# jzhangbs/MVSDF

Measured on AMD Instinct MI355X. Metric: traced rays/sec (fwd+bwd, 10 sphere iters, 4 src views), higher is better.
Workload: dtype f32x3

## Files before the change

include/mvsdf_hip.h:

```cpp
#ifndef MVSDF_HIP_H
#define MVSDF_HIP_H
#include <stddef.h>
#include <stdint.h>

#ifdef __cplusplus
extern "C" {
#endif

#define MVSDF_MAX_LAYERS 12

typedef struct {
    int n_layers;
    int K[MVSDF_MAX_LAYERS];
    int N[MVSDF_MAX_LAYERS];
    const float* wp[MVSDF_MAX_LAYERS];
    const float* bias[MVSDF_MAX_LAYERS];
    const float* w[MVSDF_MAX_LAYERS];
    int skip_layer;
    int multires;
    const void* wp16[MVSDF_MAX_LAYERS];
    int trace_dtype;
    unsigned skip_mask;
    const void* wx3[MVSDF_MAX_LAYERS];
} MvsdfNetDesc;

typedef struct {
    float r;
    float thr;
    float line_search_step;
    int line_step_iters;
    int st_iters;
    int n_steps;
    int n_secant;
    float dist_clip;
} MvsdfTraceParams;

enum {
    MVSDF_CNT_ROWS_SPHERE = 0,
    MVSDF_CNT_ROWS_SAMPLER = 1,
    MVSDF_CNT_ROWS_SECANT = 2,
    MVSDF_CNT_ROWS_MINSDF = 3,
    MVSDF_CNT_N_SECANT = 4,
    MVSDF_CNT_N_SAMPLER = 5,
    MVSDF_CNT_N_MINSDF = 6,
    MVSDF_CNT_N_SAMPLER_REST = 7,
    MVSDF_CNT_ROWS_SAMPLER_EVAL = 8,
    MVSDF_CNT_TAIL_NEXT = 9,
    MVSDF_CNT_TAIL_READY = 10,
    MVSDF_CNT_TAIL_WGS = 11,
    MVSDF_CNT_TAIL_ROWS = 12
};

int mvsdf_version(void);
int mvsdf_abi_struct_sizes(size_t* out);
const char* mvsdf_last_error(void);

size_t mvsdf_packed_floats(int N, int K);

int mvsdf_fold_pack(const float* v, const float* g, int N, int K, float* w, float* wp, float* wpT, void* stream);
int mvsdf_fold_pack_net(int n_layers, const float* const* v, const float* const* g, const int* N, const int* K, float* const* w,
                        float* const* wp, float* const* wpT, void* stream);
int mvsdf_fold_backward_net(int n_layers, const float* const* v, const float* const* g, const float* const* dW, const float* const* db,
                            const int* N, const int* K, float* const* dv, float* const* dg, float* const* dbias, int accumulate,
                            void* stream);
int mvsdf_fold_backward(const float* v, const float* g, const float* dW, int N, int K, float* dv, float* dg, void* stream);

size_t mvsdf_packed_bf16_bytes(int N, int K, int nsplit);
int mvsdf_pack_bf16w_net(int n_layers, const float* const* w, const int* N, const int* K, float* const* wp_rounded, void* stream);
int mvsdf_pack_bf16s_net(int n_layers, const float* const* w, const int* N, const int* K, void* const* wp16, void* stream);
int mvsdf_pack_bf16x3_net(int n_layers, const float* const* w, const int* N, const int* K, void* const* wp16, void* stream);
int mvsdf_pack_bf16x3t_net(int n_layers, const float* const* w, const int* N, const int* K, void* const* wx3t, void* stream);

int mvsdf_sdf_col0(const MvsdfNetDesc* net, const float* x, int n, float* y, int mt, void* stream);

int mvsdf_camera_rays(const float* uv, const float* pose, const float* intrinsics, int B, int P, float* ray_dirs, float* cam_loc,
                      void* stream);

int mvsdf_sphere_intersection(const float* cam_loc, const float* ray_dirs, int B, int P, float r, float* t, uint8_t* mask, void* stream);

size_t mvsdf_trace_workspace_bytes(int R);
size_t mvsdf_trace_workspace_bytes_n(int R, int n_steps);
int mvsdf_trace(const MvsdfNetDesc* net, const MvsdfTraceParams* tp, const float* cam_loc, const float* ray_dirs,
                const uint8_t* object_mask, int B, int P, int training, const float* intervals, const float* minsdf_steps,
                float* points, uint8_t* mask, float* dists, unsigned long long* counters, void* workspace,
                size_t workspace_bytes, int mt, int mt_samples, void* stream);
int mvsdf_trace_stage(int stage, const MvsdfNetDesc* net, const MvsdfTraceParams* tp, const float* cam_loc, const float* ray_dirs,
                      const uint8_t* object_mask, int B, int P, int training, const float* intervals, const float* minsdf_steps,
                      float* points, uint8_t* mask, float* dists, unsigned long long* counters, void* workspace,
                      size_t workspace_bytes, int mt, int mt_samples, void* stream);

size_t mvsdf_tracegen_state_bytes(int R);
int mvsdf_tracegen_init(const MvsdfTraceParams* tp, const float* cam_loc, const float* ray_dirs, const uint8_t* object_mask, int B, int P,
                        void* state, uint8_t* req, float* pts, unsigned long long* counters, void* stream);
int mvsdf_tracegen_step(const MvsdfTraceParams* tp, const float* cam_loc, const float* ray_dirs, int B, int P, void* state, const float* vals,
                        uint8_t* req, float* pts, unsigned long long* counters, void* stream);
int mvsdf_tracegen_finish(const MvsdfTraceParams* tp, const float* cam_loc, const float* ray_dirs, int B, int P, int training, const void* state,
                          float* points, uint8_t* mask, float* dists, unsigned long long* counters, void* workspace, size_t workspace_bytes,
                          void* stream);
int mvsdf_tracegen_rows(const MvsdfTraceParams* tp, int kind, const float* cam_loc, const float* ray_dirs, int B, int P, const float* zs, int n_list,
                        void* workspace, float* out_pts, void* stream);
int mvsdf_tracegen_reduce(const MvsdfTraceParams* tp, int kind, const float* cam_loc, const float* ray_dirs, int B, int P, int training,
                          const float* intervals, const float* minsdf_steps, const float* sv, float* points, uint8_t* mask, float* dists,
                          unsigned long long* counters, void* workspace, uint8_t* marks, void* stream);
int mvsdf_tracegen_secant(const MvsdfTraceParams* tp, int op, const float* cam_loc, const float* ray_dirs, int B, int P, int n_sec, const float* vals,
                          float* pts_out, float* points, float* dists, unsigned long long* counters, void* workspace, void* stream);

size_t mvsdf_sdf_ctx_floats(const MvsdfNetDesc* net, int M, int Mg);
int mvsdf_sdf_forward(const MvsdfNetDesc* net, const MvsdfNetDesc* netT, const float* x, int M, int Mg, float* y, float* nrm, float* ctx,
                      void* stream);
size_t mvsdf_sdf_bwd_ws_floats(const MvsdfNetDesc* net, int Mb);
int mvsdf_sdf_backward(const MvsdfNetDesc* net, const MvsdfNetDesc* netT, const float* x, int M, int Mg, int row0, int Mb, const float* dy,
                       const float* dn, const float* ctx, float* dW_cat, float* db_cat, float* dx, float* ws, void* stream);

int mvsdf_sdf_backward_pair(const MvsdfNetDesc* net, const MvsdfNetDesc* netT, int M, int Mg, int MbA, const float* dyA, const float* dnA, float* wsA,
                            int row0X, int MbX, const float* dyX, const float* dnX, float* wsX, float* dx, const float* ctx, void* stream);
int mvsdf_sdf_backward_finish(const MvsdfNetDesc* net, const MvsdfNetDesc* netT, int M, int Mg, int Mb, const float* dy, const float* ctx, float* ws,
                              int row0D, int MbD, const float* fbar, float* dW_cat, float* db_cat, void* stream);

size_t mvsdf_render_ctx_floats(const MvsdfNetDesc* net, int N);
size_t mvsdf_render_bwd_ws_floats(const MvsdfNetDesc* net, int N);
int mvsdf_render_forward(const MvsdfNetDesc* net, const float* points, const float* view, const float* normals, const float* feat,
                         int ldfeat, int N, int multires_view, float* rgb, float* ctx, void* stream);
int mvsdf_render_backward(const MvsdfNetDesc* net, const MvsdfNetDesc* netT, int N, int Nctx, const float* drgb, const float* ctx,
                          float* dW_cat, float* db_cat, float* din, float* ws, void* stream);

int mvsdf_feat_corr(const float* pts, int N, const int* view_start, int B, int V, int C, int H, int W, const float* feat,
                    const long long* feat_strides, const float* feat_src, const long long* src_strides, const float* cam,
                    const float* src_cams, const float* size, const float* center, float* loss_pp, float* dpts, void* stream);

int mvsdf_depth_carve(const float* pts, int pts_ld, int M, const float* depths, int B, int h, int w, const float* cams, const float* size,
                      const float* center, float out_thresh_perc, float far_thresh, float far_att, float near_thresh, float near_att, int use_invalid,
                      float* dist_r, float* weight, float* pts_world, void* stream);

int mvsdf_loss_terms(const float* rgb, const float* rgb_gt, const uint8_t* rgb_mask, int R, const float* grad_theta, int n_eik,
                     const float* eik_out, const float* dist_r, const float* dweight, int n_depth, const float* surf, int n_surf,
                     const long long* n_pos, const float* feat_pp, int n_feat, float w_rgb, float w_eik, float w_surf, float w_feat,
                     float w_depth, float smooth, int surf_on, int feat_on, const float* inv_counts, float* out, float* d_rgb, float* d_grad,
                     float* d_eik_out, float* d_surf, void* stream);

int mvsdf_partition_rays(const uint8_t* net_mask, const uint8_t* object_mask, const uint8_t* true_mask, const float* ray_dirs, int R,
                         long long* perm, long long* inv, long long* true_rows, long long* counts, float* view_sorted, void* stream);
int mvsdf_step_outputs(int R, int n_eik, int n_ds, int Nout, const long long* counts, const float* x_eval, const float* y_eval,
                       const float* n_eval, const long long* inv, const long long* true_rows, const float* rgb_sorted, int d_mask,
                       int e_mask, float* rgb_values, float* sdf_output, float* diff_pts, float* eik_out, float* points_hom, float* grad_theta,
                       float* surf, void* stream);
int mvsdf_step_backward_inputs(int stage, int n_eik, int n_ds, int N, int Nout, int n_true, const float* din, int din_ld, int din_feat0,
                               int din_nrm0, int use_geo, const float* d_diff, const float* dx, const float* view_sorted, const float* n_eval,
                               const long long* true_rows, const float* d_eo, const float* d_gth, const float* d_si, int d_mask, int e_mask,
                               float* dy, float* dn, void* stream);
int mvsdf_step_backward_fbar(int n_eik, int n_ds, int N, int Nout, const float* din, int din_ld, int use_geo, const float* d_diff, const float* dx,
                             const float* view_sorted, const float* n_eval, float* dy, float* fbar, void* stream);

int mvsdf_dsurf_select(const float* depths, const float* kinv, const float* einv, int N, int H, int W, const float* size, const float* center,
                       float bb, float jitter_rad, unsigned long long seed, int n, long long* idx, long long* counts, void* stream);
int mvsdf_dsurf_points(const float* depths, const float* kinv, const float* einv, int N, int H, int W, const float* size, const float* center,
                       float bb, float jitter_rad, unsigned long long seed, int n, const long long* idx_sorted, const long long* counts,
                       float* pts_on, float* pts_jit, void* stream);

size_t mvsdf_adam_ws_floats(void);
int mvsdf_adam_step(float* p, float* g, float* m, float* v, size_t n, float lr, double beta1, double beta2, float eps, int step, float max_norm,
                    float* norm_out, float* ws, void* stream);
int mvsdf_adam_step_scaled(float* p, float* g, float* m, float* v, size_t n, float lr, double beta1, double beta2, float eps, int step,
                           float max_norm, float grad_scale, float* norm_out, float* ws, void* stream);
int mvsdf_adam_step_fused(float* p, float* g, float* m, float* v, size_t n, float lr, double beta1, double beta2, float eps, int step,
                          float max_norm, float grad_scale, int zero_grad, float* norm_out, float* ws, void* stream);

int mvsdf_loss_prep(const uint8_t* net_mask, const uint8_t* obj_mask, const uint8_t* true_mask, int R, int B, uint8_t* hit, int* view_start,
                    long long* n_pos, void* stream);
int mvsdf_loss_scale(const float* const* g, float w_rgb, float w_eik, float w_surf, float w_feat, float w_depth, const float* d_rgb, float* g_rgb,
                     int n_rgb, const float* d_grad, float* g_grad, int n_grad, const float* d_eo, float* g_eo, int n_eo, const float* d_sf,
                     float* g_sf, int n_sf, float* coef_feat, void* stream);

int mvsdf_det_math(int op, const float* x, int n, float* y0, float* y1, void* stream);

#define MVSDF_STEP_MAX_LAYERS 24

typedef struct {
    int B, P;
    int n_eik;
    int n_ds;
    int n_sdf, n_render;
    int N[MVSDF_STEP_MAX_LAYERS];
    int K[MVSDF_STEP_MAX_LAYERS];
    unsigned skip_mask;
    int multires;
    int view_spec;
    int trace_dtype;
    int use_object_mask;
    MvsdfTraceParams tp;
    int mt, mt_samples;
} MvsdfStepDesc;

typedef struct {
    const float* v[MVSDF_STEP_MAX_LAYERS];
    const float* g[MVSDF_STEP_MAX_LAYERS];
    const float* b[MVSDF_STEP_MAX_LAYERS];
} MvsdfStepParams;

typedef struct {
    const float* uv; const float* pose; const float* intrinsics;
    const uint8_t* object_mask;
    const uint8_t* object_mask_true;
    const float* intervals;
    const float* minsdf_steps;
    const float* eik_points;
    const float* ds_on; const float* ds_jit;
    const long long* ds_counts;
    const float* host_stage;
} MvsdfStepInputs;

typedef struct {
    size_t fwd_bytes, bwd_bytes;
    size_t ray_dirs, cam_loc;
    size_t points, mask, dists, counters;
    size_t object_mask_out;
    size_t rgb_values, sdf_output, diff_pts, eik_out, points_hom, grad_theta, surf;
    size_t perm;
    size_t dflat;
    size_t dflat_floats;
} MvsdfStepLayout;

int mvsdf_step_create(const MvsdfStepDesc* desc, MvsdfStepLayout* layout, void** step);
void mvsdf_step_destroy(void* step);
#define MVSDF_STEP_UNHIT_DEFER 0
#define MVSDF_STEP_UNHIT_EAGER 1
int mvsdf_step_forward(void* step, const MvsdfStepParams* prm, const MvsdfStepInputs* in, int d_mask, int e_mask, int mode, void* fwd, void* stream);
int mvsdf_step_resolve_unhit(void* step, void* fwd, void* stream);
int mvsdf_step_can_defer_unhit(void* step);
int mvsdf_step_last_tracer_grid(void* step, int out[2]);
int mvsdf_step_wait_counts(void* step, long long counts[4]);
#define MVSDF_STEP_COUNT_RING 64
long long mvsdf_step_seq(void* step);
size_t mvsdf_step_counts_offset(void* step);
int mvsdf_step_wait_counts_seq(void* step, long long seq, long long counts[4]);
long long mvsdf_step_done_seq(void* step, long long counts[4]);
int mvsdf_step_can_defer(void* step);
int mvsdf_step_saved_offsets(void* step, size_t out[6]);
int mvsdf_step_backward(void* step, const MvsdfStepParams* prm, int N, int n_true, int d_mask, int e_mask, int use_geo, const float* d_diff,
                        const float* d_rgb, const float* d_gth, const float* d_eo, const float* d_si, const void* fwd, void* bwd,
                        float* const* dv, float* const* dg, float* const* db, int accumulate, void* stream);
int mvsdf_step_set_timing(void* step, int enable);
int mvsdf_step_trace_times(void* step, float ms[3]);
int mvsdf_step_times(void* step, float ms[6]);

typedef struct {
    int R, B;
    int N, n_grad, n_depth, n_surf;
    const uint8_t* net_mask; const uint8_t* obj_mask; const uint8_t* true_mask;
    const float* rgb; const float* rgb_gt;
    const float* grad_theta; const float* eik_out; const float* surf; const float* diff_pts;
    float* points_hom;
    int feat_on, surf_on;
    int V, C, H, W;
    const float* feat; long long feat_strides[4]; const float* feat_src; long long src_strides[5];
    const float* cam; const float* src_cams; const float* size; const float* center;
    const float* depths; int dB, dh, dw; const float* depth_cams;
    float out_thresh_perc, far_thresh, far_att, near_thresh, near_att;
    float w_rgb, w_eik, w_surf, w_feat, w_depth;
    int use_invalid;
    float smooth;
    const float* inv_counts;
    const long long* counts_dev;
    int n_eik, n_ds, d_mask, e_mask;
} MvsdfLossArgs;
typedef struct {
    size_t bytes, out, hit, view_start, n_pos, loss_pp, dpts, dist_r, weight, d_rgb, d_grad, d_eo, d_sf;
    size_t s_rgb, s_grad, s_eo, s_sf, s_diff;
} MvsdfLossLayout;
int mvsdf_loss_layout(const MvsdfLossArgs* a, MvsdfLossLayout* lo);
int mvsdf_loss_forward(const MvsdfLossArgs* a, void* blk, void* stream);
int mvsdf_loss_backward(const MvsdfLossArgs* a, const void* blk, const float* const* g, float* g_rgb, float* g_grad, float* g_eo, float* g_sf,
                        float* g_diff, void* stream);

size_t mvsdf_mc_workspace_bytes(int64_t nx, int64_t ny, int64_t nz);
int mvsdf_mc_count(const float* vol, const int64_t* shape, const int64_t* strides, float level, void* ws, size_t ws_bytes, void* stream);
int mvsdf_mc_emit(const float* vol, const int64_t* shape, const int64_t* strides, float level, const float* spacing, const float* origin, void* ws,
                  size_t ws_bytes, float* verts, float* normals, int32_t* faces, int64_t nv_cap, int64_t nf_cap, void* stream);
size_t mvsdf_mesh_cc_workspace_bytes(int64_t nv, int64_t nf);
int mvsdf_mesh_components(const float* verts, const int32_t* faces, int64_t nv, int64_t nf, void* ws, size_t ws_bytes, int32_t* vert_label,
                          int32_t* face_label, void* stream);
int mvsdf_mesh_select(const int32_t* vert_label, const int32_t* face_label, int64_t nv, int64_t nf, int32_t label, const float* verts, const float* normals,
                      const float* colors, const int32_t* faces, void* ws, size_t ws_bytes, float* out_verts, float* out_normals, float* out_colors,
                      int32_t* out_faces, int64_t nv_cap, int64_t nf_cap, void* stream);

size_t mvsdf_smc_workspace_bytes(int64_t n, int64_t block);
size_t mvsdf_smc_emit_workspace_bytes(int64_t n, int64_t block, int64_t nactive);
int mvsdf_smc_coarse_points(const float* axis, int64_t n, int64_t block, int64_t start, int64_t count, float* pts, void* stream);
int mvsdf_smc_seed(const float* coarse, int64_t n, int64_t block, float level, float tol, void* ws, size_t ws_bytes, void* stream);
int mvsdf_smc_brick_points(const float* axis, int64_t n, int64_t block, const void* ws, size_t ws_bytes, int64_t start, int64_t count, float* pts,
                           void* stream);
int mvsdf_smc_closure(const float* values, int64_t n, int64_t block, float level, int64_t slot0, int64_t count, void* ws, size_t ws_bytes, void* stream);
int mvsdf_smc_count(const float* values, int64_t n, int64_t block, float level, int64_t nactive, void* ws, size_t ws_bytes, void* ews, size_t ews_bytes,
                    void* stream);
int mvsdf_smc_emit(const float* values, int64_t n, int64_t block, float level, const float* spacing, const float* origin, int64_t nactive, void* ws,
                   size_t ws_bytes, void* ews, size_t ews_bytes, float* verts, float* normals, int32_t* faces, int64_t nv_cap, int64_t nf_cap, void* stream);

size_t mvsdf_mesh_cut_workspace_bytes(int64_t nv, int64_t nf);
int mvsdf_mesh_cut(const float* colors, const int32_t* faces, int64_t nv, int64_t nf, int32_t thresh, int32_t smooth, void* ws, size_t ws_bytes,
                   uint8_t* removed, void* stream);
int mvsdf_mesh_trim(const float* verts, const float* normals, const float* colors, const int32_t* faces, int64_t nv, int64_t nf, void* ws, size_t ws_bytes,
                    float* out_verts, float* out_normals, float* out_colors, int32_t* out_faces, int64_t nv_cap, int64_t nf_cap, void* stream);

size_t mvsdf_mesh_simplify_workspace_bytes(int64_t nv, int64_t nf);
int mvsdf_mesh_simplify(const float* verts, const float* normals, const float* colors, const int32_t* faces, int64_t nv, int64_t nf, double cell,
                        const double* origin, int32_t quadric, int32_t counts_only, void* ws, size_t ws_bytes, void* stream);
int mvsdf_mesh_simplify_emit(const int32_t* faces, int64_t nv, int64_t nf, void* ws, size_t ws_bytes, float* out_verts, float* out_normals,
                             float* out_colors, int32_t* out_faces, int64_t nv_cap, int64_t nf_cap, void* stream);

uint64_t mvsdf_chamfer_key(uint64_t seed, int64_t i);
size_t mvsdf_chamfer_sample_workspace_bytes(int64_t nv, int64_t nf);
int mvsdf_chamfer_sample_count(const float* verts, const int32_t* faces, int64_t nv, int64_t nf, double density, int64_t max_points, void* ws, size_t ws_bytes,
// ... 133 lines not shown
```

mvsdf_amd/_lib.py:

```python
import ctypes as C
import os
import struct

_HERE = os.path.dirname(os.path.abspath(__file__))
SO_PATH = os.environ.get('MVSDF_LIB') or os.path.join(_HERE, 'libmvsdf_hip.so')
MAX_LAYERS = 12
_lib = None


class NetDesc(C.Structure):
    _fields_ = [('n_layers', C.c_int), ('K', C.c_int * MAX_LAYERS), ('N', C.c_int * MAX_LAYERS),
                ('wp', C.c_void_p * MAX_LAYERS), ('bias', C.c_void_p * MAX_LAYERS), ('w', C.c_void_p * MAX_LAYERS),
                ('skip_layer', C.c_int), ('multires', C.c_int), ('wp16', C.c_void_p * MAX_LAYERS), ('trace_dtype', C.c_int), ('skip_mask', C.c_uint), ('wx3', C.c_void_p * MAX_LAYERS)]


class TraceParams(C.Structure):
    _fields_ = [('r', C.c_float), ('thr', C.c_float), ('line_search_step', C.c_float), ('line_step_iters', C.c_int),
                ('st_iters', C.c_int), ('n_steps', C.c_int), ('n_secant', C.c_int), ('dist_clip', C.c_float)]


class MvsdfError(RuntimeError):
    pass


def lib():
    global _lib
    if _lib is None:
        if not os.path.exists(SO_PATH):
            raise MvsdfError('libmvsdf_hip.so not found at %s -- run `python -c "import __graft_entry__ as g; g.build()"` '
                             '(hipcc --offload-arch=gfx950); there is no CPU/PyTorch fallback for the hot path' % SO_PATH)
        import torch
        L = C.CDLL(SO_PATH)
        L.mvsdf_last_error.restype = C.c_char_p
        L.mvsdf_packed_floats.restype = C.c_size_t
        L.mvsdf_packed_floats.argtypes = [C.c_int, C.c_int]
        L.mvsdf_trace_workspace_bytes.restype = C.c_size_t
        L.mvsdf_trace_workspace_bytes.argtypes = [C.c_int]
        L.mvsdf_trace_workspace_bytes_n.restype = C.c_size_t
        L.mvsdf_trace_workspace_bytes_n.argtypes = [C.c_int, C.c_int]
        for fn in ('mvsdf_sdf_ctx_floats', 'mvsdf_sdf_bwd_ws_floats', 'mvsdf_render_ctx_floats', 'mvsdf_render_bwd_ws_floats'):
            getattr(L, fn).restype = C.c_size_t
        L.mvsdf_adam_ws_floats.restype = C.c_size_t
        L.mvsdf_packed_bf16_bytes.restype = C.c_size_t
        L.mvsdf_packed_bf16_bytes.argtypes = [C.c_int, C.c_int, C.c_int]
        L.mvsdf_tracegen_state_bytes.restype = C.c_size_t
        L.mvsdf_adam_step.argtypes = [C.c_void_p] * 4 + [C.c_size_t] + [C.c_float, C.c_double, C.c_double, C.c_float] + [C.c_int, C.c_float, C.c_void_p, C.c_void_p, C.c_void_p]
        L.mvsdf_adam_step_scaled.argtypes = [C.c_void_p] * 4 + [C.c_size_t] + [C.c_float, C.c_double, C.c_double, C.c_float] + [C.c_int, C.c_float, C.c_float, C.c_void_p, C.c_void_p, C.c_void_p]
        L.mvsdf_adam_step_fused.argtypes = [C.c_void_p] * 4 + [C.c_size_t] + [C.c_float, C.c_double, C.c_double, C.c_float] + [C.c_int, C.c_float, C.c_float, C.c_int, C.c_void_p, C.c_void_p, C.c_void_p]
        L.mvsdf_loss_scale.argtypes = [C.c_void_p] + [C.c_float] * 5 + [C.c_void_p, C.c_void_p, C.c_int] * 4 + [C.c_void_p, C.c_void_p]
        i64, vp, f32 = C.c_int64, C.c_void_p, C.c_float
        L.mvsdf_mc_workspace_bytes.restype = C.c_size_t
        L.mvsdf_mc_workspace_bytes.argtypes = [i64] * 3
        L.mvsdf_mc_count.argtypes = [vp, vp, vp, f32, vp, C.c_size_t, vp]
        L.mvsdf_mc_emit.argtypes = [vp, vp, vp, f32, vp, vp, vp, C.c_size_t, vp, vp, vp, i64, i64, vp]
        L.mvsdf_mesh_cc_workspace_bytes.restype = C.c_size_t
        L.mvsdf_mesh_cc_workspace_bytes.argtypes = [i64, i64]
        L.mvsdf_mesh_components.argtypes = [vp, vp, i64, i64, vp, C.c_size_t, vp, vp, vp]
        L.mvsdf_mesh_select.argtypes = [vp, vp, i64, i64, C.c_int32] + [vp] * 5 + [C.c_size_t] + [vp] * 4 + [i64, i64, vp]
        L.mvsdf_smc_workspace_bytes.restype = C.c_size_t
        L.mvsdf_smc_workspace_bytes.argtypes = [i64, i64]
        L.mvsdf_smc_emit_workspace_bytes.restype = C.c_size_t
        L.mvsdf_smc_emit_workspace_bytes.argtypes = [i64, i64, i64]
        L.mvsdf_smc_coarse_points.argtypes = [vp, i64, i64, i64, i64, vp, vp]
        L.mvsdf_smc_seed.argtypes = [vp, i64, i64, f32, f32, vp, C.c_size_t, vp]
        L.mvsdf_smc_brick_points.argtypes = [vp, i64, i64, vp, C.c_size_t, i64, i64, vp, vp]
        L.mvsdf_smc_closure.argtypes = [vp, i64, i64, f32, i64, i64, vp, C.c_size_t, vp]
        L.mvsdf_smc_count.argtypes = [vp, i64, i64, f32, i64, vp, C.c_size_t, vp, C.c_size_t, vp]
        L.mvsdf_smc_emit.argtypes = [vp, i64, i64, f32, vp, vp, i64, vp, C.c_size_t, vp, C.c_size_t, vp, vp, vp, i64, i64, vp]
        L.mvsdf_mesh_cut_workspace_bytes.restype = C.c_size_t
        L.mvsdf_mesh_cut_workspace_bytes.argtypes = [i64, i64]
        L.mvsdf_mesh_cut.argtypes = [vp, vp, i64, i64, C.c_int32, C.c_int32, vp, C.c_size_t, vp, vp]
        L.mvsdf_mesh_trim.argtypes = [vp] * 4 + [i64, i64, vp, C.c_size_t] + [vp] * 4 + [i64, i64, vp]
        f64, u64, sz = C.c_double, C.c_uint64, C.c_size_t
        L.mvsdf_mesh_simplify_workspace_bytes.restype = sz
        L.mvsdf_mesh_simplify_workspace_bytes.argtypes = [i64, i64]
        L.mvsdf_mesh_simplify.argtypes = [vp] * 4 + [i64, i64, f64, vp, C.c_int32, C.c_int32, vp, sz, vp]
        L.mvsdf_mesh_simplify_emit.argtypes = [vp, i64, i64, vp, sz] + [vp] * 4 + [i64, i64, vp]
        L.mvsdf_chamfer_key.restype = u64
        L.mvsdf_chamfer_key.argtypes = [u64, i64]
        for fn in ('mvsdf_chamfer_sample_workspace_bytes', 'mvsdf_chamfer_mask_workspace_bytes', 'mvsdf_chamfer_nearest_workspace_bytes'):
            getattr(L, fn).restype = sz
            getattr(L, fn).argtypes = [i64, i64]
        L.mvsdf_chamfer_downsample_workspace_bytes.restype = sz
        L.mvsdf_chamfer_downsample_workspace_bytes.argtypes = [i64]
        L.mvsdf_chamfer_sample_count.argtypes = [vp, vp, i64, i64, f64, i64, vp, sz, vp]
        L.mvsdf_chamfer_sample_emit.argtypes = [vp, vp, i64, i64, f64, vp, sz, vp, i64, vp]
        L.mvsdf_chamfer_downsample.argtypes = [vp, i64, f64, u64, i64, vp, sz, vp, vp]
        L.mvsdf_chamfer_mask.argtypes = [vp, vp, i64, vp, i64, vp, f64, vp, vp, vp, vp, sz, vp, vp, vp, vp]
        L.mvsdf_chamfer_nearest.argtypes = [vp, i64, vp, i64, f64, vp, sz, vp, vp]
        i32 = C.c_int32
        L.mvsdf_fusion_workspace_bytes.restype = sz
        L.mvsdf_fusion_workspace_bytes.argtypes = [i64] * 4
        L.mvsdf_fusion_fuse.argtypes = [vp, vp, vp, i64, i64, i64, vp, vp, vp, i32, i32, f64, f64, vp, sz, vp, vp, vp, vp]
        L.mvsdf_fusion_emit.argtypes = [vp, i64, i64, i64, i64, vp, sz, vp, vp, vp, vp, i64, vp]
        L.mvsdf_tsdf_workspace_bytes.restype = sz
        L.mvsdf_tsdf_workspace_bytes.argtypes = [i64] * 4
        L.mvsdf_tsdf_integrate.argtypes = [vp, i64, i64, i64, vp, vp, i64, vp, f64, vp, f64, f64, i32, vp, sz, vp, vp, vp, vp]
        L.mvsdf_mcm_workspace_bytes.restype = sz
        L.mvsdf_mcm_workspace_bytes.argtypes = [i64] * 3
        L.mvsdf_mcm_count.argtypes = [vp, vp, vp, vp, f32, vp, sz, vp]
        L.mvsdf_mcm_emit.argtypes = [vp, vp, vp, vp, f32, vp, vp, vp, sz, vp, vp, vp, i64, i64, vp]
        for fn in ('mvsdf_cloud_clean_workspace_bytes', 'mvsdf_cloud_compact_workspace_bytes'):
            getattr(L, fn).restype = sz
            getattr(L, fn).argtypes = [i64]
        L.mvsdf_cloud_knn.argtypes = [vp, i64, i32, vp, sz, vp, vp]
        L.mvsdf_cloud_components.argtypes = [vp, i64, f64, vp, sz, vp, vp]
        L.mvsdf_cloud_clean.argtypes = [vp, i64, i32, f64, f64, f64, vp, sz, vp, vp, vp, vp]
        L.mvsdf_cloud_compact.argtypes = [vp] * 5 + [i64, vp, sz] + [vp] * 4 + [i64, vp]
        L.mvsdf_raster_workspace_bytes.restype = sz
        L.mvsdf_raster_workspace_bytes.argtypes = [i64] * 5
        L.mvsdf_raster_draw.argtypes = [vp, vp, i64, i64, vp, i64, i64, i64, f64, i64, i32, vp, sz, vp]
        L.mvsdf_raster_resolve.argtypes = [i64, i64, i64, vp, sz, vp, vp, vp]
        L.mvsdf_raster_visibility.argtypes = [vp, i64, vp, i64, i64, i64, f64, vp, vp, f64, vp, sz, vp, vp]
        L.mvsdf_raster_colors.argtypes = [vp, vp, i64, vp, vp, i64, i64, i64, f64, vp, vp, vp, f64, f64, i32, f32, f32, f32, vp, sz, vp, vp, vp]
        for fn in ('mvsdf_featext_raw_floats', 'mvsdf_featext_pack_bytes', 'mvsdf_featext_workspace_bytes', 'mvsdf_featext_layer_workspace_bytes'):
            getattr(L, fn).restype = sz
        L.mvsdf_featext_raw_floats.argtypes = []
        L.mvsdf_featext_pack_bytes.argtypes = []
        L.mvsdf_featext_pack.argtypes = [vp, vp, sz, vp]
        L.mvsdf_featext_workspace_bytes.argtypes = [i64] * 3
        L.mvsdf_featext_forward.argtypes = [vp, vp, i64, i64, i64, vp, sz, vp, vp, vp, C.c_int, C.c_int, vp]
        L.mvsdf_featext_layer_workspace_bytes.argtypes = [C.c_int] * 5
        L.mvsdf_featext_layer.argtypes = [C.c_int, vp, vp, C.c_int, C.c_int, C.c_int, vp, C.c_int, vp, C.c_int, i64, i64, i64, vp, C.c_int, vp, sz, vp, vp]
        for fn in ('mvsdf_stereo_workspace_bytes', 'mvsdf_stereo_volume_offset'):
            getattr(L, fn).restype = sz
            getattr(L, fn).argtypes = [i64] * 4
        L.mvsdf_stereo_normalize.argtypes = [vp, i64, i64, vp, vp, vp]
        L.mvsdf_stereo_patches.argtypes = [vp, i64, i64, i64, i32, vp, vp]
        L.mvsdf_stereo_sweep.argtypes = [vp, i64, i64, i64, i64, i64] + [vp] * 7 + [sz] + [vp] * 5
        L.mvsdf_stereo_sgm_workspace_bytes.restype = sz
        L.mvsdf_stereo_sgm_workspace_bytes.argtypes = [i64] * 3
        L.mvsdf_stereo_regularize.argtypes = [vp, i64, i64, i64, f64, f64, i32, vp, sz, vp, vp]
        L.mvsdf_stereo_sweep_sgm_workspace_bytes.restype = sz
        L.mvsdf_stereo_sweep_sgm_workspace_bytes.argtypes = [i64] * 4
        L.mvsdf_stereo_sweep_sgm.argtypes = [vp, i64, i64, i64, i64, i64] + [vp] * 6 + [f64, f64, i32, vp, sz] + [vp] * 5
        L.mvsdf_stereo_upsample.argtypes = [vp, vp] + [i64] * 5 + [vp, vp]
        L.mvsdf_stereo_band_workspace_bytes.restype = sz
        L.mvsdf_stereo_band_workspace_bytes.argtypes = [i64] * 5
        L.mvsdf_stereo_band.argtypes = [vp, i64, i64, i64, i64, i64] + [vp] * 6 + [i32, vp, sz] + [vp] * 5
        L.mvsdf_viewsel_bits_bytes.restype = sz
        L.mvsdf_viewsel_bits_bytes.argtypes = [i64, i64]
        L.mvsdf_viewsel_workspace_bytes.restype = sz
        L.mvsdf_viewsel_workspace_bytes.argtypes = [i64]
        L.mvsdf_viewsel_pack_dense.argtypes = [vp, i64, i64, vp, vp, vp]
        L.mvsdf_viewsel_pack_tracks.argtypes = [vp, vp, i64, i64, i64, vp, vp, vp]
        L.mvsdf_viewsel_scores.argtypes = [vp, vp, vp, i64, i64, f64, f64, f64, vp, sz, vp, vp, vp, vp]
        L.mvsdf_viewsel_depths.argtypes = [vp, vp, vp, i64, i64, i64, i64, vp, vp, vp]
        L.mvsdf_viewsel_weights_host.argtypes = [vp, vp, i64, f64, f64, f64, vp, vp]
        L.mvsdf_undistort_points.argtypes = [vp, i64, C.c_int, vp, vp, C.c_int, vp, vp, vp]
        L.mvsdf_undistort_images.argtypes = [vp, i64, i64, i64, i64, C.c_int, C.c_int, vp, vp, i64, i64, vp, vp, vp]
        L.mvsdf_undistort_points_host.argtypes = [vp, i64, C.c_int, vp, vp, C.c_int, vp, vp]
        L.mvsdf_undistort_images_host.argtypes = [vp, i64, i64, i64, i64, C.c_int, C.c_int, vp, vp, i64, i64, vp, vp]
        L.mvsdf_batch_args_bytes.restype = sz
        L.mvsdf_batch_args_bytes.argtypes = []
        L.mvsdf_batch_gather.argtypes = [vp, vp]
        for name in EXPORTS:
            getattr(L, name)
        _lib = L
    return _lib


EXPORTS = [
    'mvsdf_version', 'mvsdf_abi_struct_sizes', 'mvsdf_last_error', 'mvsdf_packed_floats', 'mvsdf_fold_pack', 'mvsdf_fold_backward', 'mvsdf_fold_pack_net', 'mvsdf_fold_backward_net', 'mvsdf_packed_bf16_bytes', 'mvsdf_pack_bf16w_net', 'mvsdf_pack_bf16s_net', 'mvsdf_pack_bf16x3_net', 'mvsdf_pack_bf16x3t_net',
    'mvsdf_sdf_col0', 'mvsdf_camera_rays', 'mvsdf_sphere_intersection', 'mvsdf_trace_workspace_bytes', 'mvsdf_trace_workspace_bytes_n', 'mvsdf_trace', 'mvsdf_trace_stage', 'mvsdf_det_math',
    'mvsdf_tracegen_state_bytes', 'mvsdf_tracegen_init', 'mvsdf_tracegen_step', 'mvsdf_tracegen_finish', 'mvsdf_tracegen_rows', 'mvsdf_tracegen_reduce',
    'mvsdf_tracegen_secant',
    'mvsdf_sdf_ctx_floats', 'mvsdf_sdf_forward', 'mvsdf_sdf_bwd_ws_floats', 'mvsdf_sdf_backward', 'mvsdf_sdf_backward_pair', 'mvsdf_sdf_backward_finish',
    'mvsdf_feat_corr', 'mvsdf_depth_carve', 'mvsdf_loss_terms', 'mvsdf_loss_prep', 'mvsdf_loss_scale', 'mvsdf_adam_ws_floats', 'mvsdf_adam_step', 'mvsdf_adam_step_scaled', 'mvsdf_adam_step_fused',
    'mvsdf_partition_rays', 'mvsdf_step_outputs', 'mvsdf_step_backward_inputs', 'mvsdf_step_backward_fbar', 'mvsdf_dsurf_select', 'mvsdf_dsurf_points',
    'mvsdf_render_ctx_floats', 'mvsdf_render_bwd_ws_floats', 'mvsdf_render_forward', 'mvsdf_render_backward',
    'mvsdf_step_create', 'mvsdf_step_destroy', 'mvsdf_step_forward', 'mvsdf_step_resolve_unhit', 'mvsdf_step_can_defer_unhit', 'mvsdf_step_last_tracer_grid', 'mvsdf_step_wait_counts', 'mvsdf_step_backward', 'mvsdf_step_set_timing', 'mvsdf_step_trace_times', 'mvsdf_step_times',
    'mvsdf_step_seq', 'mvsdf_step_counts_offset', 'mvsdf_step_wait_counts_seq', 'mvsdf_step_done_seq', 'mvsdf_step_can_defer', 'mvsdf_step_saved_offsets',
    'mvsdf_loss_layout', 'mvsdf_loss_forward', 'mvsdf_loss_backward',
    'mvsdf_mc_workspace_bytes', 'mvsdf_mc_count', 'mvsdf_mc_emit', 'mvsdf_mesh_cc_workspace_bytes', 'mvsdf_mesh_components', 'mvsdf_mesh_select',
    'mvsdf_smc_workspace_bytes', 'mvsdf_smc_emit_workspace_bytes', 'mvsdf_smc_coarse_points', 'mvsdf_smc_seed', 'mvsdf_smc_brick_points',
    'mvsdf_smc_closure', 'mvsdf_smc_count', 'mvsdf_smc_emit',
    'mvsdf_mesh_cut_workspace_bytes', 'mvsdf_mesh_cut', 'mvsdf_mesh_trim',
    'mvsdf_mesh_simplify_workspace_bytes', 'mvsdf_mesh_simplify', 'mvsdf_mesh_simplify_emit',
    'mvsdf_chamfer_key', 'mvsdf_chamfer_sample_workspace_bytes', 'mvsdf_chamfer_sample_count', 'mvsdf_chamfer_sample_emit',
    'mvsdf_chamfer_downsample_workspace_bytes', 'mvsdf_chamfer_downsample', 'mvsdf_chamfer_mask_workspace_bytes', 'mvsdf_chamfer_mask',
    'mvsdf_chamfer_nearest_workspace_bytes', 'mvsdf_chamfer_nearest',
    'mvsdf_fusion_workspace_bytes', 'mvsdf_fusion_fuse', 'mvsdf_fusion_emit',
    'mvsdf_tsdf_workspace_bytes', 'mvsdf_tsdf_integrate', 'mvsdf_mcm_workspace_bytes', 'mvsdf_mcm_count', 'mvsdf_mcm_emit',
    'mvsdf_cloud_clean_workspace_bytes', 'mvsdf_cloud_compact_workspace_bytes', 'mvsdf_cloud_knn', 'mvsdf_cloud_components', 'mvsdf_cloud_clean',
    'mvsdf_cloud_compact',
    'mvsdf_raster_workspace_bytes', 'mvsdf_raster_draw', 'mvsdf_raster_resolve', 'mvsdf_raster_visibility', 'mvsdf_raster_colors',
    'mvsdf_featext_raw_floats', 'mvsdf_featext_pack_bytes', 'mvsdf_featext_pack', 'mvsdf_featext_workspace_bytes', 'mvsdf_featext_forward',
    'mvsdf_featext_layer_workspace_bytes', 'mvsdf_featext_layer',
    'mvsdf_stereo_workspace_bytes', 'mvsdf_stereo_volume_offset', 'mvsdf_stereo_normalize', 'mvsdf_stereo_patches', 'mvsdf_stereo_sweep',
    'mvsdf_stereo_sgm_workspace_bytes', 'mvsdf_stereo_regularize', 'mvsdf_stereo_sweep_sgm_workspace_bytes', 'mvsdf_stereo_sweep_sgm',
    'mvsdf_stereo_upsample', 'mvsdf_stereo_band_workspace_bytes', 'mvsdf_stereo_band',
    'mvsdf_viewsel_bits_bytes', 'mvsdf_viewsel_workspace_bytes', 'mvsdf_viewsel_pack_dense', 'mvsdf_viewsel_pack_tracks', 'mvsdf_viewsel_scores',
    'mvsdf_viewsel_depths', 'mvsdf_viewsel_weights_host',
    'mvsdf_undistort_points', 'mvsdf_undistort_images', 'mvsdf_undistort_points_host', 'mvsdf_undistort_images_host',
    'mvsdf_batch_args_bytes', 'mvsdf_batch_gather',
]


def check(rc, what=''):
    if rc != 0:
        raise MvsdfError('%s failed (code %d): %s' % (what or 'mvsdf call', rc, lib().mvsdf_last_error().decode()))


def ptr(t):
    if t is None:
        return None
    assert t.is_contiguous(), 'tensor must be contiguous'
    return C.c_void_p(t.data_ptr())


def stream_of(t):
    import torch
    if t.is_cuda:
        return C.c_void_p(torch.cuda.current_stream(t.device).cuda_stream)
    return C.c_void_p(0)


def _vp(t):
    return None if t is None else t.data_ptr()


def _stream(t):
    import torch
    return torch.cuda.current_stream(t.device).cuda_stream


def _header(ws, n):
    import torch
    return [int(x) for x in ws[:8 * n].view(torch.int64).cpu()]


def f64_from_bits(bits):
    return struct.unpack('<d', struct.pack('<q', bits))[0]
```

mvsdf_amd/csrc/step_driver.hip:

```cpp
#include <hip/hip_runtime.h>
#include <stdint.h>
#include <stdlib.h>
#include <string.h>
#include <new>
#include "capi_util.h"
#include "step_internal.h"
#include <sched.h>
#include <time.h>

namespace {

inline size_t al256(size_t x) { return (x + 255) & ~(size_t)255; }

struct FwdOffsets {
    size_t w[MVSDF_STEP_MAX_LAYERS], wp[MVSDF_STEP_MAX_LAYERS], wpT[MVSDF_STEP_MAX_LAYERS], wp16[MVSDF_STEP_MAX_LAYERS];
    size_t wx3[MVSDF_STEP_MAX_LAYERS], wx3T[MVSDF_STEP_MAX_LAYERS];
    int chain_x3;
    size_t trace_ws, trace_ws_bytes;
    size_t inv, true_rows, true_rank, counts, view_sorted;
    size_t bias[MVSDF_STEP_MAX_LAYERS], steps;
    size_t x_eval, y_eval, n_eval, sdf_ctx, rgb_sorted, render_ctx;
};
struct BwdOffsets {
    size_t dy, dn, dy_x, dn_x, din, drgb_sorted, render_ws, wsA, wsX, dx, fbar;
};

struct Step {
    MvsdfStepDesc d;
    MvsdfStepLayout lay;
    FwdOffsets fo;
    BwdOffsets bo;
    int R, E, M, Nout, K0r, nl;
    size_t woff[MVSDF_STEP_MAX_LAYERS], boff[MVSDF_STEP_MAX_LAYERS];
    size_t seg[2][3];
    long long* counts_host;
    long long* counts_host_dev;
    int can_defer;
    hipEvent_t ev_counts;
    bool counts_pending;
    long long counts_seq;
    hipStream_t counts_stream;
    int timing;
    hipEvent_t ev_t[9];
    bool timed, timed_bwd;
    hipStream_t side;
    hipEvent_t ev_fork, ev_join;
    int split_rows;
    int can_lazy;
    int last_grid[2];
};

void make_descs(const Step& st, const MvsdfStepParams* prm, const char* fwd, MvsdfNetDesc* sdf, MvsdfNetDesc* sdfT, MvsdfNetDesc* rnd, MvsdfNetDesc* rndT) {
    const MvsdfStepDesc& d = st.d;
    auto fill = [&](MvsdfNetDesc* o, MvsdfNetDesc* oT, int l0, int n, bool is_sdf) {
        memset(o, 0, sizeof(*o));
        memset(oT, 0, sizeof(*oT));
        o->n_layers = oT->n_layers = n;
        for (int i = 0; i < n; ++i) {
            const int l = l0 + i;
            o->K[i] = d.K[l]; o->N[i] = d.N[l];
            oT->K[i] = d.N[l]; oT->N[i] = d.K[l];
            o->wp[i] = (const float*)(fwd + st.fo.wp[l]);
            oT->wp[i] = (const float*)(fwd + st.fo.wpT[l]);
            o->bias[i] = oT->bias[i] = prm->b[l];
            o->w[i] = oT->w[i] = (const float*)(fwd + st.fo.w[l]);
            if (is_sdf && d.trace_dtype != 0) o->wp16[i] = fwd + st.fo.wp16[l];
            if (is_sdf && st.fo.chain_x3) { o->wx3[i] = fwd + st.fo.wx3[l]; oT->wx3[i] = fwd + st.fo.wx3T[l]; }
        }
        if (is_sdf) {
            const unsigned m = d.skip_mask;
            const int single = (m && !(m & (m - 1))) ? __builtin_ctz(m) : -1;
            o->skip_layer = oT->skip_layer = m ? (single >= 0 ? single : __builtin_ctz(m)) : -1;
            o->skip_mask = (m && single < 0) ? m : 0;
            o->multires = oT->multires = d.multires;
            o->trace_dtype = (d.trace_dtype >= 1 && d.trace_dtype <= 5) ? d.trace_dtype : 0;
        } else {
            o->skip_layer = oT->skip_layer = -1;
        }
    };
    fill(sdf, sdfT, 0, d.n_sdf, true);
    fill(rnd, rndT, d.n_sdf, d.n_render, false);
}

__global__ void k_step_gather_x(const float* __restrict__ eik, int n_eik, const float* __restrict__ ds_on, const float* __restrict__ ds_jit, int n_ds,
                                const float* __restrict__ points, const long long* __restrict__ perm, int R, float* __restrict__ x_eval,
                                uint8_t* __restrict__ ones) {
    const int E = n_eik + 2 * n_ds, total = (E + R) * 3;
    for (int i = blockIdx.x * blockDim.x + threadIdx.x; i < total; i += gridDim.x * blockDim.x) {
        const int row = i / 3, c = i - 3 * row;
        float v;
        if (row < n_eik) v = eik[i];
        else if (row < n_eik + n_ds) v = ds_on[3 * (size_t)(row - n_eik) + c];
        else if (row < E) v = ds_jit[3 * (size_t)(row - n_eik - n_ds) + c];
        else v = points[3 * (size_t)perm[row - E] + c];
        x_eval[i] = v;
        if (ones && i < R) ones[i] = 1;
    }
}

__global__ void k_step_gather_drgb(const float* __restrict__ d_rgb, const long long* __restrict__ perm, int N, float* __restrict__ out) {
    const int i = blockIdx.x * blockDim.x + threadIdx.x;
    if (i >= 3 * N) return;
    const int row = i / 3, c = i - 3 * row;
    out[i] = d_rgb[3 * (size_t)perm[row] + c];
}

#define ST_TRY(expr) do { int rc_ = (expr); if (rc_) return rc_; } while (0)
#define ST_HIP(expr) do { hipError_t e_ = (expr); if (e_ != hipSuccess) return mv_check(e_, #expr); } while (0)

}

extern "C" {

int mvsdf_step_create(const MvsdfStepDesc* desc, MvsdfStepLayout* layout, void** out) {
    if (!desc || !layout || !out) return mv_fail(-1, "mvsdf_step_create: null argument");
    if (desc->trace_dtype == 1) return mv_fail(-2, "mvsdf_step_create: trace_dtype 1 (bf16 weights AND 8-bit activations) was removed in round 5: use 3 (bf16x2)");
    const MvsdfStepDesc& d = *desc;
    const int nl = d.n_sdf + d.n_render;
    if (d.B <= 0 || d.P <= 0 || d.n_eik < 0 || d.n_ds < 0 || d.n_sdf < 2 || d.n_render < 1 || d.n_sdf > MVSDF_MAX_LAYERS || d.n_render > MVSDF_MAX_LAYERS ||
        nl > MVSDF_STEP_MAX_LAYERS || (long long)d.B * d.P > (1ll << 24))
        return mv_fail(-1, "mvsdf_step_create: bad sizes");
    Step* st = new (std::nothrow) Step;
    if (!st) return mv_fail(-1, "mvsdf_step_create: out of host memory");
    memset(st, 0, sizeof(*st));
    st->d = d;
    st->R = d.B * d.P; st->E = d.n_eik + 2 * d.n_ds; st->M = st->R + st->E; st->nl = nl;
    st->Nout = d.N[d.n_sdf - 1]; st->K0r = d.K[d.n_sdf];
    st->split_rows = -1;
    const int R = st->R, M = st->M;
    MvsdfNetDesc sdf, sdfT, rnd, rndT;
    MvsdfStepParams fake;
    memset(&fake, 0, sizeof(fake));
    static const float dummy = 0.f;
    for (int l = 0; l < nl; ++l) fake.b[l] = &dummy;
    MvsdfStepLayout& L = st->lay;
    FwdOffsets& fo = st->fo;
    size_t p = 0;
    auto take = [&](size_t bytes) { const size_t o = p; p += al256(bytes ? bytes : 4); return o; };
    L.ray_dirs = take((size_t)R * 12); L.cam_loc = take((size_t)d.B * 12);
    L.points = take((size_t)R * 12); L.mask = take((size_t)R); L.dists = take((size_t)R * 4); L.counters = take(16 * 8);
    L.object_mask_out = take((size_t)R);
    fo.trace_ws_bytes = mvsdf_trace_workspace_bytes_n(R, d.tp.n_steps);
    fo.trace_ws = take(fo.trace_ws_bytes);
    fo.chain_x3 = mv_dev_switches().chain_x3;
    for (int l = 0; l < nl; ++l) {
        fo.w[l] = take((size_t)d.N[l] * d.K[l] * 4);
        fo.wp[l] = take(mvsdf_packed_floats(d.N[l], d.K[l]) * 4);
        fo.wpT[l] = take(mvsdf_packed_floats(d.K[l], d.N[l]) * 4);
        if (l < d.n_sdf && d.trace_dtype == 2) {
            fo.wp16[l] = take(mvsdf_packed_floats(d.N[l], d.K[l]) * 4);
        } else if (l < d.n_sdf && (d.trace_dtype == 3 || d.trace_dtype == 4)) {
            fo.wp16[l] = take(mvsdf_packed_bf16_bytes(d.N[l], d.K[l], 0));
        } else if (l < d.n_sdf && d.trace_dtype == 5) {
            fo.wp16[l] = take(3 * mvsdf_packed_bf16_bytes(d.N[l], d.K[l], 0));
        }
        if (l < d.n_sdf && fo.chain_x3) {
            fo.wx3[l] = d.trace_dtype == 5 ? fo.wp16[l] : take(3 * mvsdf_packed_bf16_bytes(d.N[l], d.K[l], 0));
            fo.wx3T[l] = take(3 * mvsdf_packed_bf16_bytes(d.K[l], d.N[l], 0));
        }
    }
    L.perm = take((size_t)R * 8); fo.inv = take((size_t)R * 8); fo.true_rows = take((size_t)R * 8); fo.true_rank = take((size_t)R * 4); fo.counts = take(4 * 8 + 4 * 4);
    fo.view_sorted = take((size_t)R * 12);
    for (int l = 0; l < d.n_sdf; ++l) fo.bias[l] = take((size_t)d.N[l] * 4);
    fo.steps = take((size_t)(d.tp.n_steps > 0 ? d.tp.n_steps : 0) * 4);
    fo.x_eval = take((size_t)M * 12); fo.y_eval = take((size_t)M * st->Nout * 4); fo.n_eval = take((size_t)M * 12);
    make_descs(*st, &fake, (const char*)nullptr, &sdf, &sdfT, &rnd, &rndT);
    for (int i = 0; i < d.n_sdf; ++i) { sdf.wp[i] = sdfT.wp[i] = &dummy; sdf.w[i] = &dummy; }
    for (int i = 0; i < d.n_render; ++i) { rnd.wp[i] = rndT.wp[i] = &dummy; }
    const size_t ctx_f = mvsdf_sdf_ctx_floats(&sdf, M, M), rctx_f = mvsdf_render_ctx_floats(&rnd, R);
    if (!ctx_f || !rctx_f) { delete st; return mv_fail(-2, "mvsdf_step_create: network descriptor rejected (layer dims / skip mask)"); }
    st->can_lazy = mv_chain_fwd_covers(&sdf);
    st->can_defer = (d.n_ds == 0 && mv_step_can_defer(&sdf, &sdfT, &rnd, &rndT)) ? 1 : 0;
    fo.sdf_ctx = take(ctx_f * 4);
    fo.rgb_sorted = take((size_t)R * 12);
    fo.render_ctx = take(rctx_f * 4);
    L.rgb_values = take((size_t)R * 12); L.sdf_output = take((size_t)R * 4); L.diff_pts = take((size_t)R * 12);
    L.eik_out = take((size_t)M * 4); L.points_hom = take((size_t)M * 16); L.grad_theta = take((size_t)M * 12);
    L.surf = take((size_t)(R + d.n_eik) * 4);
    L.fwd_bytes = p;
    BwdOffsets& bo = st->bo;
    p = 0;
    bo.dy = take((size_t)M * st->Nout * 4); bo.dn = take((size_t)M * 12);
    bo.dy_x = take((size_t)R * st->Nout * 4); bo.dn_x = take((size_t)R * 12);
    bo.din = take((size_t)R * st->K0r * 4); bo.drgb_sorted = take((size_t)R * 12);
    bo.render_ws = take(mvsdf_render_bwd_ws_floats(&rnd, R) * 4);
    bo.wsA = take(mvsdf_sdf_bwd_ws_floats(&sdf, M) * 4);
    bo.wsX = take(mvsdf_sdf_bwd_ws_floats(&sdf, R) * 4);
    bo.dx = take((size_t)R * 12); bo.fbar = take((size_t)R * 4);
    size_t off = 0;
    int lo = 0;
    const int cuts[2] = {d.n_sdf, nl};
    for (int net = 0; net < 2; ++net) {
        st->seg[net][0] = off;
        for (int l = lo; l < cuts[net]; ++l) { st->woff[l] = off; off += (size_t)d.N[l] * d.K[l]; }
        st->seg[net][1] = off;
        for (int l = lo; l < cuts[net]; ++l) { st->boff[l] = off; off += (size_t)d.N[l]; }
        st->seg[net][2] = off;
        lo = cuts[net];
    }
    L.dflat_floats = off;
    L.dflat = take(off * 4);
    L.bwd_bytes = p;
    *layout = L;
    *out = st;
    return 0;
}

void mvsdf_step_destroy(void* step) {
    Step* st = (Step*)step;
    if (!st) return;
    if (st->timing) for (int i = 0; i < 9; ++i) hipEventDestroy(st->ev_t[i]);
    if (st->counts_host) { hipEventDestroy(st->ev_counts); hipHostFree(st->counts_host); }
    if (st->side) { hipStreamSynchronize(st->side); hipEventDestroy(st->ev_fork); hipEventDestroy(st->ev_join); hipStreamDestroy(st->side); }
    delete st;
}

int mvsdf_step_set_timing(void* step, int enable) {
    Step* st = (Step*)step;
    if (!st) return mv_fail(-1, "mvsdf_step_set_timing: null step");
    if (enable && !st->timing) {
        for (int i = 0; i < 9; ++i) ST_HIP(hipEventCreate(&st->ev_t[i]));
        st->timing = 1;
    } else if (!enable && st->timing) {
        for (int i = 0; i < 9; ++i) hipEventDestroy(st->ev_t[i]);
        st->timing = 0;
    }
    st->timed = false; st->timed_bwd = false;
    return 0;
}

int mvsdf_step_trace_times(void* step, float ms[3]) {
    Step* st = (Step*)step;
    if (!st || !ms || !st->timing || !st->timed) return mv_fail(-1, "mvsdf_step_trace_times: timing is off or no forward has run");
    float a = 0.f, b = 0.f, c = 0.f;
    ST_HIP(hipEventElapsedTime(&a, st->ev_t[0], st->ev_t[1]));
    ST_HIP(hipEventElapsedTime(&b, st->ev_t[1], st->ev_t[2]));
    ST_HIP(hipEventElapsedTime(&c, st->ev_t[3], st->ev_t[4]));
    ms[0] = a; ms[1] = b; ms[2] = c;
    return 0;
}

int mvsdf_step_times(void* step, float ms[6]) {
    Step* st = (Step*)step;
    if (!st || !ms || !st->timing || !st->timed) return mv_fail(-1, "mvsdf_step_times: timing is off or no forward has run");
    if (int rc = mvsdf_step_trace_times(step, ms)) return rc;
    ST_HIP(hipEventElapsedTime(&ms[3], st->ev_t[4], st->ev_t[5]));
    ms[4] = 0.f;
    if (st->timed_bwd) ST_HIP(hipEventElapsedTime(&ms[4], st->ev_t[6], st->ev_t[7]));
    ST_HIP(hipEventElapsedTime(&ms[5], st->ev_t[8], st->ev_t[5]));
    return 0;
}

int mvsdf_step_forward(void* step, const MvsdfStepParams* prm, const MvsdfStepInputs* in, int d_mask, int e_mask, int mode, void* fwd_, void* stream) {
    Step* st = (Step*)step;
    if (!st || !prm || !in || !fwd_) return mv_fail(-1, "mvsdf_step_forward: null argument");
    if (mode != MVSDF_STEP_UNHIT_DEFER && mode != MVSDF_STEP_UNHIT_EAGER) return mv_fail(-1, "mvsdf_step_forward: mode must be MVSDF_STEP_UNHIT_DEFER or MVSDF_STEP_UNHIT_EAGER");
    const bool lazy = mode == MVSDF_STEP_UNHIT_DEFER;
    if (lazy && !st->can_lazy) return mv_fail(-3, "mvsdf_step_forward: MVSDF_STEP_UNHIT_DEFER is not available for this step (mvsdf_step_can_defer_unhit)");
    const MvsdfStepDesc& d = st->d;
    if (!in->uv || !in->pose || !in->intrinsics || !in->object_mask || !in->object_mask_true || !in->intervals || !in->minsdf_steps ||
        (d.n_eik > 0 && !in->eik_points) || (d.n_ds > 0 && (!in->ds_on || !in->ds_jit || !in->ds_counts)))
        return mv_fail(-1, "mvsdf_step_forward: missing input");
    hipStream_t s = (hipStream_t)stream;
    if (!st->counts_host) {
        ST_HIP(hipHostMalloc((void**)&st->counts_host, MVSDF_STEP_COUNT_RING * 8 * sizeof(long long), hipHostMallocMapped | hipHostMallocCoherent));
        memset(st->counts_host, 0, MVSDF_STEP_COUNT_RING * 8 * sizeof(long long));
        if (hipHostGetDevicePointer((void**)&st->counts_host_dev, st->counts_host, 0) != hipSuccess) { (void)hipGetLastError(); st->counts_host_dev = nullptr; }
        if (hipEventCreateWithFlags(&st->ev_counts, hipEventDisableTiming) != hipSuccess) {
            hipHostFree(st->counts_host); st->counts_host = nullptr;
            return mv_fail(-1, "mvsdf_step_forward: hipEventCreate failed");
        }
    }
    char* fwd = (char*)fwd_;
    const MvsdfStepLayout& L = st->lay;
    const FwdOffsets& fo = st->fo;
    const int R = st->R, E = st->E, M = st->M, nl = st->nl;
    if (st->timing) ST_HIP(hipEventRecord(st->ev_t[8], s));
    float* w[MVSDF_STEP_MAX_LAYERS]; float* wp[MVSDF_STEP_MAX_LAYERS]; float* wpT[MVSDF_STEP_MAX_LAYERS];
    for (int l = 0; l < nl; ++l) { w[l] = (float*)(fwd + fo.w[l]); wp[l] = (float*)(fwd + fo.wp[l]); wpT[l] = (float*)(fwd + fo.wpT[l]); }
    float* ray_dirs = (float*)(fwd + L.ray_dirs); float* cam_loc = (float*)(fwd + L.cam_loc);
    {
        void* wp16[MVSDF_STEP_MAX_LAYERS]; int nsplit[MVSDF_STEP_MAX_LAYERS];
        void* wx3[MVSDF_STEP_MAX_LAYERS]; void* wx3T[MVSDF_STEP_MAX_LAYERS];
        for (int l = 0; l < nl; ++l) {
            const bool bf = l < d.n_sdf && d.trace_dtype != 0;
            wp16[l] = bf ? (void*)(fwd + fo.wp16[l]) : nullptr;
            const bool x3 = l < d.n_sdf && fo.chain_x3;
            wx3[l] = (x3 && d.trace_dtype != 5) ? (void*)(fwd + fo.wx3[l]) : nullptr;
            wx3T[l] = x3 ? (void*)(fwd + fo.wx3T[l]) : nullptr;
            nsplit[l] = 0;
        }
        const float* stage_dev = nullptr;
        if (in->host_stage) {
            if (hipHostGetDevicePointer((void**)&stage_dev, (void*)in->host_stage, 0) != hipSuccess || !stage_dev) {
                (void)hipGetLastError();
                return mv_fail(-1, "mvsdf_step_forward: host_stage is not device-visible pinned memory");
            }
        }
        float* bias_copy[MVSDF_STEP_MAX_LAYERS];
        for (int l = 0; l < nl; ++l) bias_copy[l] = (lazy && l < d.n_sdf) ? (float*)(fwd + fo.bias[l]) : nullptr;
        float* steps_copy = lazy ? (float*)(fwd + fo.steps) : nullptr;
        if (lazy && !stage_dev) ST_HIP(hipMemcpyAsync(steps_copy, in->minsdf_steps, (size_t)d.tp.n_steps * 4, hipMemcpyDeviceToDevice, s));
        ST_TRY(mv_step_prologue(nl, prm->v, prm->g, d.N, d.K, w, wp, wpT, wp16, nsplit, d.trace_dtype == 2 ? 1 : (d.trace_dtype == 5 ? 2 : 0), wx3, wx3T, in->uv, in->pose, in->intrinsics, d.B, d.P, ray_dirs, cam_loc,
                                (uint8_t*)(fwd + L.object_mask_out), (unsigned long long*)(fwd + L.counters), stage_dev, (float*)in->minsdf_steps, d.tp.n_steps,
                                (float*)in->eik_points, 3 * d.n_eik, steps_copy, prm->b, bias_copy, stream));
    }
    MvsdfNetDesc sdf, sdfT, rnd, rndT;
    make_descs(*st, prm, fwd, &sdf, &sdfT, &rnd, &rndT);
    float* x_eval = (float*)(fwd + fo.x_eval); float* y_eval = (float*)(fwd + fo.y_eval); float* n_eval = (float*)(fwd + fo.n_eval);
    FwdGather g;
    g.eik = in->eik_points; g.on = in->ds_on; g.jit = in->ds_jit; g.pts = (float*)(fwd + L.points); g.perm = (long long*)(fwd + L.perm);
    g.n_eik = d.n_eik; g.n_ds = d.n_ds; g.x_out = x_eval;
    if (st->split_rows < 0) {
        const char* e = getenv("MVSDF_SPLIT_ROWS");
        st->split_rows = (e && *e) ? (atoi(e) != 0 && E >= 1) : mv_chain_split_pays(&sdf, E, M);
        if (st->split_rows) {
            int prio_least = 0, prio_greatest = 0;
            if (hipDeviceGetStreamPriorityRange(&prio_least, &prio_greatest) != hipSuccess) { (void)hipGetLastError(); prio_least = 0; }
            if (hipStreamCreateWithPriority(&st->side, hipStreamNonBlocking, prio_least) != hipSuccess) { (void)hipGetLastError(); st->side = nullptr; st->split_rows = 0; }
            else if (hipEventCreateWithFlags(&st->ev_fork, hipEventDisableTiming) != hipSuccess ||
                     hipEventCreateWithFlags(&st->ev_join, hipEventDisableTiming) != hipSuccess) {
                (void)hipGetLastError();
                if (st->ev_fork) { (void)hipEventDestroy(st->ev_fork); st->ev_fork = nullptr; }
                if (st->ev_join) { (void)hipEventDestroy(st->ev_join); st->ev_join = nullptr; }
                (void)hipStreamDestroy(st->side);
                st->side = nullptr; st->split_rows = 0;
            }
        }
    }
    bool split = st->split_rows == 1;
    struct SideGuard {
        hipStream_t side; bool armed;
        ~SideGuard() { if (armed && side) (void)hipStreamSynchronize(side); }
    } side_guard{st->side, false};
    if (split) ST_HIP(hipEventRecord(st->ev_fork, s));
    float* points = (float*)(fwd + L.points); uint8_t* mask = (uint8_t*)(fwd + L.mask); float* dists = (float*)(fwd + L.dists);
    unsigned long long* counters = (unsigned long long*)(fwd + L.counters);
    auto stage = [&](int which) {
        if (lazy && which != 3)
            return mv_trace_stage_notail(which, &sdf, &d.tp, cam_loc, ray_dirs, in->object_mask, d.B, d.P, 1, in->intervals, in->minsdf_steps, points, mask, dists,
                                         counters, fwd + fo.trace_ws, fo.trace_ws_bytes, d.mt, d.mt_samples, stream);
        return mvsdf_trace_stage(which, &sdf, &d.tp, cam_loc, ray_dirs, in->object_mask, d.B, d.P, 1, in->intervals, in->minsdf_steps, points, mask, dists,
                                 counters, fwd + fo.trace_ws, fo.trace_ws_bytes, d.mt, d.mt_samples, stream);
    };
    if (st->timing) ST_HIP(hipEventRecord(st->ev_t[0], s));
    if (lazy) ST_TRY(stage(1));
    else ST_TRY(mv_trace_stage1_prezeroed(&sdf, &d.tp, cam_loc, ray_dirs, in->object_mask, d.B, d.P, 1, in->intervals, in->minsdf_steps, points, mask, dists,
                                     counters, fwd + fo.trace_ws, fo.trace_ws_bytes, d.mt, d.mt_samples, stream));
    if (st->timing) ST_HIP(hipEventRecord(st->ev_t[1], s));
    if (split) {
        ST_HIP(hipStreamWaitEvent(st->side, st->ev_fork, 0));
        side_guard.armed = true;
        const int rcs = mv_sdf_forward_gather(&sdf, &sdfT, nullptr, &g, M, M, 0, E, y_eval, n_eval, (float*)(fwd + fo.sdf_ctx), st->side);
        if (rcs == 1) { split = false; side_guard.armed = false; }
        else if (rcs) return rcs;
        else ST_HIP(hipEventRecord(st->ev_join, st->side));
    }
    ST_TRY(stage(3));
    if (st->timing) ST_HIP(hipEventRecord(st->ev_t[2], s));
    long long* perm = (long long*)(fwd + L.perm); long long* inv = (long long*)(fwd + fo.inv); long long* true_rows = (long long*)(fwd + fo.true_rows);
    long long* counts = (long long*)(fwd + fo.counts); float* view_sorted = (float*)(fwd + fo.view_sorted);
    ST_TRY(mv_partition_rays_step(mask, d.use_object_mask ? in->object_mask : nullptr, in->object_mask_true, ray_dirs, R, perm, inv, true_rows, counts,
                                  view_sorted, (int*)(fwd + fo.true_rank), d.n_ds > 0 ? in->ds_counts : nullptr,
                                  st->counts_host_dev ? st->counts_host_dev + 8 * ((st->counts_seq + 1) % MVSDF_STEP_COUNT_RING) : nullptr, st->counts_seq + 1,
                                  (float*)(fwd + fo.counts + 32), d.n_eik, d.n_ds, d_mask, e_mask, stream));
    ++st->counts_seq;
    if (!st->counts_host_dev) {
        ST_HIP(hipMemcpyAsync(st->counts_host, counts, 4 * sizeof(long long), hipMemcpyDeviceToHost, s));
        ST_HIP(hipEventRecord(st->ev_counts, s));
    }
    st->counts_pending = true; st->counts_stream = s;
    if (st->timing) ST_HIP(hipEventRecord(st->ev_t[3], s));
    ST_TRY(stage(lazy ? 7 : 4));
    mv_trace_last_grid(st->last_grid);
    if (st->timing) { ST_HIP(hipEventRecord(st->ev_t[4], s)); st->timed = true; }
    {
        if (split) { ST_HIP(hipStreamWaitEvent(s, st->ev_join, 0)); side_guard.armed = false; }
        int rcf = mv_sdf_forward_gather_cnt(&sdf, &sdfT, nullptr, &g, M, M, split ? E : 0, M, lazy ? counts : nullptr, E, 1, y_eval, n_eval, (float*)(fwd + fo.sdf_ctx), stream);
        if (rcf == 1 && lazy) return mv_fail(-3, "mvsdf_step_forward: the fused forward chain refused a step it was said to cover");
        if (rcf == 1) {
            const int total = M * 3;
            hipLaunchKernelGGL(k_step_gather_x, dim3((total + 255) / 256), dim3(256), 0, s, in->eik_points, d.n_eik, in->ds_on, in->ds_jit, d.n_ds, points, perm,
                               R, x_eval, (uint8_t*)nullptr);
            ST_HIP(hipGetLastError());
            rcf = mvsdf_sdf_forward(&sdf, &sdfT, x_eval, M, M, y_eval, n_eval, (float*)(fwd + fo.sdf_ctx), stream);
        }
        if (rcf) return rcf;
    }
    float* rgb_sorted = (float*)(fwd + fo.rgb_sorted);
    ST_TRY(mvsdf_render_forward(&rnd, x_eval + 3 * (size_t)E, view_sorted, n_eval + 3 * (size_t)E, y_eval + (size_t)E * st->Nout + 2, st->Nout, R,
                                d.view_spec, rgb_sorted, (float*)(fwd + fo.render_ctx), stream));
    ST_TRY((lazy ? mv_step_outputs_hit : mvsdf_step_outputs)(R, d.n_eik, d.n_ds, st->Nout, counts, x_eval, y_eval, n_eval, inv, true_rows, rgb_sorted, d_mask, e_mask,
                              (float*)(fwd + L.rgb_values), (float*)(fwd + L.sdf_output), (float*)(fwd + L.diff_pts), (float*)(fwd + L.eik_out),
                              (float*)(fwd + L.points_hom), (float*)(fwd + L.grad_theta), (float*)(fwd + L.surf), stream));
    if (st->timing) ST_HIP(hipEventRecord(st->ev_t[5], s));
    return 0;
}

int mvsdf_step_resolve_unhit(void* step, void* fwd_, void* stream) {
    Step* st = (Step*)step;
    if (!st || !fwd_) return mv_fail(-1, "mvsdf_step_resolve_unhit: null argument");
    if (!st->can_lazy) return mv_fail(-3, "mvsdf_step_resolve_unhit: not available for this step (mvsdf_step_can_defer_unhit)");
    const MvsdfStepDesc& d = st->d;
    char* fwd = (char*)fwd_;
    const MvsdfStepLayout& L = st->lay;
    const FwdOffsets& fo = st->fo;
    const int R = st->R, E = st->E, M = st->M;
    MvsdfStepParams prm;
    memset(&prm, 0, sizeof(prm));
    for (int l = 0; l < d.n_sdf; ++l) prm.b[l] = (const float*)(fwd + fo.bias[l]);
    MvsdfNetDesc sdf, sdfT, rnd, rndT;
    make_descs(*st, &prm, fwd, &sdf, &sdfT, &rnd, &rndT);
    float* points = (float*)(fwd + L.points); uint8_t* mask = (uint8_t*)(fwd + L.mask); float* dists = (float*)(fwd + L.dists);
    const float* steps = (const float*)(fwd + fo.steps);
    ST_TRY(mv_trace_stage_notail(5, &sdf, &d.tp, (const float*)(fwd + L.cam_loc), (const float*)(fwd + L.ray_dirs), (const uint8_t*)(fwd + L.object_mask_out), d.B, d.P, 1,
                                 steps, steps, points, mask, dists, (unsigned long long*)(fwd + L.counters), fwd + fo.trace_ws, fo.trace_ws_bytes, d.mt, d.mt_samples, stream));
    FwdGather g;
    memset(&g, 0, sizeof(g));
    g.pts = points; g.perm = (long long*)(fwd + L.perm); g.n_eik = d.n_eik; g.n_ds = d.n_ds; g.x_out = (float*)(fwd + fo.x_eval);
    const long long* counts = (const long long*)(fwd + fo.counts);
    float* y_eval = (float*)(fwd + fo.y_eval);
    const int rcf = mv_sdf_forward_gather_cnt(&sdf, &sdfT, nullptr, &g, M, M, E, M, counts, E, 2, y_eval, (float*)(fwd + fo.n_eval), (float*)(fwd + fo.sdf_ctx), stream);
    if (rcf) return rcf == 1 ? mv_fail(-3, "mvsdf_step_resolve_unhit: the fused forward chain refused a step it was said to cover") : rcf;
    return mv_step_unhit_scatter(R, E, st->Nout, counts, y_eval, g.perm, (float*)(fwd + L.sdf_output), stream);
}
int mvsdf_step_can_defer_unhit(void* step) { Step* st = (Step*)step; return (st && st->can_lazy) ? 1 : 0; }
int mvsdf_step_last_tracer_grid(void* step, int out[2]) {
    Step* st = (Step*)step;
    if (!st || !out) return mv_fail(-1, "mvsdf_step_last_tracer_grid: null argument");
    out[0] = st->last_grid[0]; out[1] = st->last_grid[1];
    return 0;
}

static int step_wait_seq(Step* st, long long seq, long long counts[4]) {
    long long* slot = st->counts_host + 8 * (seq % MVSDF_STEP_COUNT_RING);
    for (unsigned long long it = 1;; ++it) {
        const long long have = __atomic_load_n(&slot[4], __ATOMIC_ACQUIRE);
        if (have == seq) break;
        if (have > seq) return mv_fail(-4, "mvsdf_step_wait_counts_seq: the record of that forward was overwritten (read the counts from its forward block)");
        if (it < 5000) { __builtin_ia32_pause(); continue; }
        struct timespec ts = {0, 20000};
// ... 194 lines not shown
```

mvsdf_amd/csrc/step_internal.h:

```cpp
#pragma once
#include <stdint.h>
#include "../../include/mvsdf_hip.h"
#include "diff_route.h"

struct FwdGather { const float* eik; const float* on; const float* jit; const float* pts; const long long* perm; int n_eik, n_ds; float* x_out; };

int mv_partition_rays_step(const uint8_t* net_mask, const uint8_t* object_mask, const uint8_t* true_mask, const float* ray_dirs, int R, long long* perm,
                           long long* inv, long long* true_rows, long long* counts, float* view_sorted, int* true_rank, const long long* extra_counts,
                           long long* counts_host, long long counts_seq, float* term_rows, int n_eik, int n_ds, int d_mask, int e_mask,
                           void* stream);
int mv_step_backward_assemble(int n_eik, int n_ds, int N, int Nout, int n_true, const float* din, int din_ld, int din_feat0, int din_nrm0, int use_geo,
                              const int* true_rank, const float* d_eo, const float* d_gth, const float* d_si, int d_mask, int e_mask, float* dy,
                              float* dn, float* dy_x, float* dn_x, const long long* cnt, void* stream);

int mv_sdf_backward_pair_cnt(const MvsdfNetDesc* d, const MvsdfNetDesc* dT, int M, int Mg, int MbA, const float* dyA, const float* dnA, float* wsA,
                             int row0X, int MbX, const float* dyX, const float* dnX, float* wsX, float* dx, const float* ctx, const long long* cnt, int n_hint,
                             void* stream);
int mv_step_can_defer(const MvsdfNetDesc* sdf, const MvsdfNetDesc* sdfT, const MvsdfNetDesc* rnd, const MvsdfNetDesc* rndT);

int mv_sdf_forward_gather(const MvsdfNetDesc* d, const MvsdfNetDesc* dT, const float* x, const void* gather, int M, int Mg, int r_begin, int r_end,
                          float* y, float* nrm, float* ctx, void* stream);
int mv_sdf_forward_gather_cnt(const MvsdfNetDesc* d, const MvsdfNetDesc* dT, const float* x, const void* gather, int M, int Mg, int r_begin, int r_end,
                              const long long* cnt, int cnt_base, int cnt_mode, float* y, float* nrm, float* ctx, void* stream);
int mv_step_outputs_hit(int R, int n_eik, int n_ds, int Nout, const long long* counts, const float* x_eval, const float* y_eval, const float* n_eval,
                        const long long* inv, const long long* true_rows, const float* rgb_sorted, int d_mask, int e_mask, float* rgb_values, float* sdf_output,
                        float* diff_pts, float* eik_out, float* points_hom, float* grad_theta, float* surf, void* stream);
int mv_step_unhit_scatter(int R, int E, int Nout, const long long* counts, const float* y_eval, const long long* perm, float* sdf_output, void* stream);
int mv_chain_fwd_covers(const MvsdfNetDesc* d);
int mv_chain_split_pays(const MvsdfNetDesc* d, int E, int M);

int mv_render_backward_chain(const MvsdfNetDesc* d, const MvsdfNetDesc* dT, int N, int Nctx, const float* drgb, const long long* drgb_rows, const float* ctx,
                             float* din, float* ws, const long long* cnt, void* stream);
int mv_sdf_backward_delta_fbar(const MvsdfNetDesc* d, int M, int Mg, int Mb, const float* ctx, float* ws, int row0D, int MbD, int Nout, const float* din,
                               int din_ld, int use_geo, const float* d_diff, const float* dx, const float* view_sorted, const float* n_eval, float* dy,
                               float* fbar, const long long* cnt, void* stream);
int mv_sdf_backward_delta(const MvsdfNetDesc* d, const MvsdfNetDesc* dT, int M, int Mg, int Mb, const float* ctx, float* ws, int row0D, int MbD,
                          const float* fbar, void* stream);
int mv_step_wgrad(const MvsdfNetDesc* sd, const MvsdfNetDesc* rd, int M, int Mg, int Mb, const float* dy, const float* ctx, float* wsA, int N, int Nctx,
                  const float* rctx, float* rws, float* dW_s, float* db_s, float* dW_r, float* db_r, const long long* cnt, int cnt_base, void* stream);

int mv_step_prologue(int n_layers, const float* const* v, const float* const* g, const int* N, const int* K, float* const* w, float* const* wp,
                     float* const* wpT, void* const* wp16, const int* nsplit, int wp16_mode, void* const* wx3, void* const* wx3T, const float* uv, const float* pose,
                     const float* intrinsics, int B, int P,
                     float* ray_dirs, float* cam_loc, uint8_t* ones, unsigned long long* counters, const float* stage_src, float* stage_a, int stage_na,
                     float* stage_b, int stage_nb, float* stage_a2, const float* const* bias, float* const* bias_copy,
                     void* stream);
const MvDevSwitches& mv_dev_switches();
extern "C" int mv_trace_stage1_prezeroed(const MvsdfNetDesc* desc, const MvsdfTraceParams* tp, const float* cam_loc, const float* ray_dirs, const uint8_t* object_mask,
                              int B, int P, int training, const float* intervals, const float* minsdf_steps, float* points, uint8_t* mask, float* dists,
                              unsigned long long* counters, void* workspace, size_t workspace_bytes, int mt, int mt_samples, void* stream);
extern "C" int mv_trace_stage_notail(int stage, const MvsdfNetDesc* desc, const MvsdfTraceParams* tp, const float* cam_loc, const float* ray_dirs, const uint8_t* object_mask,
                              int B, int P, int training, const float* intervals, const float* minsdf_steps, float* points, uint8_t* mask, float* dists,
                              unsigned long long* counters, void* workspace, size_t workspace_bytes, int mt, int mt_samples, void* stream);
void mv_trace_last_grid(int out[2]);
```

mvsdf_amd/csrc/trace.hip:

```cpp
#include <stdlib.h>
#include <type_traits>
#include "tile_engine.h"
#include "tile_engine_bf16.h"
#include "tile_engine_bf16s.h"
#include "trace_params.h"
#include "capi_util.h"

struct RayCommon {
    float c[3], d[3];
};

__device__ __forceinline__ float mv_clamp(float v, float lo, float hi) { return v < lo ? lo : (v > hi ? hi : v); }

__device__ __forceinline__ bool mv_sphere_isect(const float* c, const float* d, float r, float& t0, float& t1) {
    const float dot = fmaf(d[2], c[2], fmaf(d[1], c[1], d[0] * c[0]));
    const float nrm = sqrtf(c[0] * c[0] + c[1] * c[1] + c[2] * c[2]);
    const float under = dot * dot - (nrm * nrm - r * r);
    const bool hit = under > 0.0f;
    float a = 0.0f, b = 0.0f;
    if (hit) {
        const float s = sqrtf(under);
        a = s * -1.0f - dot;
        b = s * 1.0f - dot;
    }
    t0 = a < 0.0f ? 0.0f : a;
    t1 = b < 0.0f ? 0.0f : b;
    return hit;
}

template <int MT, int NTW, int NW, class NET, bool XR = false>
__device__ __forceinline__ void mv_eval_dispatch(const NET& net, int ntiles, float* act, float* pe, const float* pts, float* out, int tid) {
    if constexpr (std::is_same<NET, MvNet>::value) {
        if (MT >= 4 && ntiles == 4) mv_sdf_eval_col0<(MT >= 4 ? 4 : MT), NTW, NW>(net, act, pe, pts, out, tid);
        else if (MT >= 3 && ntiles == 3) mv_sdf_eval_col0<(MT >= 3 ? 3 : MT), NTW, NW>(net, act, pe, pts, out, tid);
        else if (MT >= 2 && ntiles == 2) mv_sdf_eval_col0<(MT >= 2 ? 2 : MT), NTW, NW>(net, act, pe, pts, out, tid);
        else if constexpr (XR) mv_sdf_eval_col0<1, NTW, NW, true>(net, act, pe, pts, out, tid);
        else mv_sdf_eval_col0<1, NTW, NW>(net, act, pe, pts, out, tid);
    } else {
        if (MT >= 4 && ntiles == 4) mv_sdf_eval_col0<(MT >= 4 ? 4 : MT), NTW, NW, false>(net, act, pe, pts, out, tid);
        else if (MT >= 3 && ntiles == 3) mv_sdf_eval_col0<(MT >= 3 ? 3 : MT), NTW, NW, false>(net, act, pe, pts, out, tid);
        else if (MT >= 2 && ntiles == 2) {
            if constexpr (XR && MT == 2 && NTW < 4 && mv_bs_pp<NET>::v) mv_sdf_eval_col0_pp<2, NTW, NW, (XR && NTW < 4)>(net, act, pe, pts, out, tid);
            else mv_sdf_eval_col0<(MT >= 2 ? 2 : MT), NTW, NW, (XR && NTW < 4)>(net, act, pe, pts, out, tid);
        }
        else if constexpr (mv_bs_pp<NET>::v) mv_sdf_eval_col0_pp<1, NTW, NW, (XR && NTW < 4)>(net, act, pe, pts, out, tid);
        else mv_sdf_eval_col0<1, NTW, NW, (XR && NTW < 4)>(net, act, pe, pts, out, tid);
    }
}

struct TraceLds {
    float* act; float* pe; float* pts; float* sdfv; float* sv; int* misc;
};
template <class NET> __host__ __device__ constexpr int mv_act_rows(int rows, bool sphere = false) {
    return !mv_bs_pp<NET>::v ? rows : (rows < 32 ? 32 : ((sphere && rows == 32) ? 64 : rows));
}
template <class NET, bool SPHERE = false>
__device__ __forceinline__ TraceLds mv_carve(float* base, int rows, int S, int d0, int sv_floats) {
    TraceLds l;
    l.act = base;
    l.pe = l.act + mv_act_rows<NET>(rows, SPHERE) * S;
    l.pts = l.pe + ((rows * d0 + 3) & ~3);
    l.sdfv = l.pts + rows * 4;
    l.sv = l.sdfv + rows;
    l.misc = (int*)(l.sv + sv_floats);
    return l;
}

struct TailCtx {
    const float* steps;
    float* sv;
    int unit_rows;
    int enable, spin;
    int stop_left;
    unsigned* probe;
};
#define MV_SPHERE_FINALIZE \
    if (tid == 0 && nrows_total) atomicAdd(&counters[MV_CNT_ROWS_SPHERE], nrows_total); \
    if (valid) { \
        bool net_mask = acc_s < acc_e; \
        const bool sampler = unf_s; \
        float dist = acc_s; \
        bool listed = false; \
        float zmin = acc_s, zmax = acc_e; \
        int kind = 0; \
        if (sampler) { listed = true; kind = MV_ITEM_SAMPLER | (om ? MV_ITEM_OM : 0); } \
        else if (training) { \
            const bool in_mask = !net_mask && om; \
            const bool out_mask = !om; \
            if (in_mask || out_mask) { \
                if (!isect) { \
                    const float dot = (d[0] * c[0] + d[1] * c[1]) + d[2] * c[2]; \
                    dist = -dot; \
                } else { \
                    listed = true; kind = MV_ITEM_MINSDF; \
                    zmin = (net_mask && out_mask) ? acc_s : t0; \
                    zmax = t1; \
                } \
            } \
        } \
        o_mask[gid] = net_mask ? 1 : 0; \
        o_dists[gid] = dist; \
        o_points[3 * (size_t)gid + 0] = c[0] + dist * d[0]; \
        o_points[3 * (size_t)gid + 1] = c[1] + dist * d[1]; \
        o_points[3 * (size_t)gid + 2] = c[2] + dist * d[2]; \
        if (listed) { \
            const bool smp = kind & MV_ITEM_SAMPLER; \
            w_zmin[gid] = zmin; \
            w_zmax[gid] = zmax; \
            const unsigned long long idx = atomicAdd(&counters[smp ? MV_CNT_N_SAMPLER : MV_CNT_N_MINSDF], 1ull); \
            (smp ? w_list : w_list_min)[idx] = gid | (kind << 28); \
            if (!smp) n_pub = 1; \
        } \
    }

template <int MT, int NTW, int NW, class NET>
__global__ __launch_bounds__(64 * NW) void k_sphere_trace(NET net, MvTraceParams tp, const float* __restrict__ cam_loc,
                                                            const float* __restrict__ dirs, const uint8_t* __restrict__ object_mask,
                                                            int R, int P, int training, float* __restrict__ o_points,
                                                            uint8_t* __restrict__ o_mask, float* __restrict__ o_dists,
                                                            float* __restrict__ w_zmin, float* __restrict__ w_zmax, int* __restrict__ w_list,
                                                            int* __restrict__ w_list_min, unsigned long long* __restrict__ counters, TailCtx tail) {
    extern __shared__ __attribute__((aligned(16))) float smem[];
    constexpr int ROWS = 16 * MT, NR = 8 * MT;
    const long long clk0 = tail.probe ? (long long)wall_clock64() : 0;
    unsigned n_rounds = 0;
    const int tid = threadIdx.x, lane = tid & 63, w = __builtin_amdgcn_readfirstlane(tid >> 6);
    TraceLds lds = mv_carve<NET, (NTW < 4)>(smem, ROWS, net.S, 3 + 6 * net.multires, 0);
    int* s_n = lds.misc;

    const int gid = blockIdx.x * NR + tid;
    const bool valid = (tid < NR) && (gid < R);
    float c[3] = {0, 0, 0}, d[3] = {0, 0, 0};
    float t0 = 0.f, t1 = 0.f;
    bool isect = false, om = false;
    if (valid) {
        const int b = gid / P;
        for (int i = 0; i < 3; ++i) { c[i] = cam_loc[3 * b + i]; d[i] = dirs[3 * (size_t)gid + i]; }
        isect = mv_sphere_isect(c, d, tp.r, t0, t1);
        om = object_mask[gid] != 0;
    }
    bool unf_s = isect, unf_e = isect;
    float acc_s = isect ? t0 : 0.f, acc_e = isect ? t1 : 0.f;
    float next_s = 0.f, next_e = 0.f, curr_s = 0.f, curr_e = 0.f;
    int iters = 0, k = 0, phase = isect ? 0 : 3;
    bool req_s = isect, req_e = isect;
    float ts = acc_s, te = acc_e;
    unsigned long long nrows_total = 0;

    bool hard_s = false, hard_e = false, bo_s = false, bo_e = false;
    const float lss1 = 1.0f - tp.line_search_step;
    bool helping = false;
    int n_pub = 0;
    int h_chunk = 0, h_left = 0, h_items = 0, h_nr = 0;
    long long h_svi = 0;
    unsigned h_units = 0;
    long long clk1 = 0;
    for (;;) {
        int row_s = 0, row_e = 0;
        int sr_s[3] = {-1, -1, -1}, sr_e[3] = {-1, -1, -1};
        int lvl0 = 0;
        if (!helping && w == 0) {
            const unsigned long long ms = __ballot(req_s), me = __ballot(req_e);
            const unsigned long long lt = (1ull << lane) - 1ull;
            const int ns = __popcll(ms), ne = __popcll(me), n = ns + ne;
            row_s = __popcll(ms & lt);
            row_e = ns + __popcll(me & lt);
            if (req_s) { float* p = lds.pts + row_s * 3; p[0] = c[0] + ts * d[0]; p[1] = c[1] + ts * d[1]; p[2] = c[2] + ts * d[2]; }
            if (req_e) { float* p = lds.pts + row_e * 3; p[0] = c[0] + te * d[0]; p[1] = c[1] + te * d[1]; p[2] = c[2] + te * d[2]; }
            int base = n, left = ((n + 15) & ~15) - n;
            lvl0 = (phase == 2) ? k + 1 : 0;
            const bool can = (phase == 1 || phase == 2);
            if (left > 0 && tp.line_step_iters > 0) {
#pragma unroll
                for (int pass = 0; pass < 2; ++pass) {
#pragma unroll
                    for (int dd = 0; dd < 3; ++dd) {
                        const bool lv_ok = can && (lvl0 + dd + 1 <= tp.line_step_iters);
                        const bool cs = lv_ok && req_s && (pass == 0 ? hard_s : !hard_s);
                        const bool ce = lv_ok && req_e && (pass == 0 ? hard_e : !hard_e);
                        const unsigned long long bs = __ballot(cs), be = __ballot(ce);
                        int cnt = __popcll(bs), take = cnt < left ? cnt : left;
                        if (cs && __popcll(bs & lt) < take) sr_s[dd] = base + __popcll(bs & lt);
                        base += take; left -= take;
                        cnt = __popcll(be); take = cnt < left ? cnt : left;
                        if (ce && __popcll(be & lt) < take) sr_e[dd] = base + __popcll(be & lt);
                        base += take; left -= take;
                    }
                }
                float z = ts;
#pragma unroll
                for (int dd = 0; dd < 3; ++dd) {
                    z = z - (lss1 / (float)(1 << (lvl0 + dd))) * curr_s;
                    if (sr_s[dd] >= 0) { float* p = lds.pts + sr_s[dd] * 3; p[0] = c[0] + z * d[0]; p[1] = c[1] + z * d[1]; p[2] = c[2] + z * d[2]; }
                }
                z = te;
#pragma unroll
                for (int dd = 0; dd < 3; ++dd) {
                    z = z + (lss1 / (float)(1 << (lvl0 + dd))) * curr_e;
                    if (sr_e[dd] >= 0) { float* p = lds.pts + sr_e[dd] * 3; p[0] = c[0] + z * d[0]; p[1] = c[1] + z * d[1]; p[2] = c[2] + z * d[2]; }
                }
            }
            if (lane == 0) { s_n[0] = base; s_n[1] = n; }
        }
        int n = 0;
        if (!helping) {
            __syncthreads();
            n = s_n[0];
            if (n == 0) {
                MV_SPHERE_FINALIZE
                if (!tail.enable) break;
                const int pub = (w == 0) ? __popcll(__ballot(n_pub != 0)) : 0;
                __syncthreads();
                if (tid == 0) {
                    __hip_atomic_fetch_add(&counters[MV_CNT_TAIL_READY], (unsigned long long)pub, __ATOMIC_RELEASE, __HIP_MEMORY_SCOPE_AGENT);
                    __hip_atomic_fetch_add(&counters[MV_CNT_TAIL_WGS], 1ull, __ATOMIC_RELAXED, __HIP_MEMORY_SCOPE_AGENT);
                }
                clk1 = tail.probe ? (long long)wall_clock64() : 0;
                helping = true;
            } else {
                ++n_rounds;
                if (tid == 0) nrows_total += (unsigned long long)s_n[1];
            }
        }
        if (helping) {
            if (h_left == 0) {
                if (tid == 0) {
                    long long take = -1;
                    int n_items = 0;
                    for (int tries = 0; tries < 64; ++tries) {
                        if (__hip_atomic_load(&counters[MV_CNT_TAIL_WGS], __ATOMIC_RELAXED, __HIP_MEMORY_SCOPE_AGENT) + (unsigned long long)tail.stop_left >= (unsigned long long)gridDim.x) break;
                        const long long head = (long long)__hip_atomic_load(&counters[MV_CNT_TAIL_NEXT], __ATOMIC_RELAXED, __HIP_MEMORY_SCOPE_AGENT);
                        const unsigned long long res0 = __hip_atomic_load(&counters[MV_CNT_N_MINSDF], __ATOMIC_RELAXED, __HIP_MEMORY_SCOPE_AGENT);
                        asm volatile("" ::: "memory");
                        const unsigned long long rdy = __hip_atomic_load(&counters[MV_CNT_TAIL_READY], __ATOMIC_RELAXED, __HIP_MEMORY_SCOPE_AGENT);
                        asm volatile("" ::: "memory");
                        const unsigned long long res = __hip_atomic_load(&counters[MV_CNT_N_MINSDF], __ATOMIC_RELAXED, __HIP_MEMORY_SCOPE_AGENT);
                        long long rows = (long long)res * tp.n_steps;
                        if (res0 == res && rdy == res && head + ((long long)gridDim.x + 1) * ROWS <= rows) {
                            take = (long long)__hip_atomic_fetch_add(&counters[MV_CNT_TAIL_NEXT], (unsigned long long)ROWS, __ATOMIC_RELAXED, __HIP_MEMORY_SCOPE_AGENT);
                            n_items = (int)res;
                            while (take + ROWS > rows) {
                                const unsigned long long wgs = __hip_atomic_load(&counters[MV_CNT_TAIL_WGS], __ATOMIC_RELAXED, __HIP_MEMORY_SCOPE_AGENT);
                                asm volatile("" ::: "memory");
                                const unsigned long long a0 = __hip_atomic_load(&counters[MV_CNT_N_MINSDF], __ATOMIC_RELAXED, __HIP_MEMORY_SCOPE_AGENT);
                                asm volatile("" ::: "memory");
                                const unsigned long long r1 = __hip_atomic_load(&counters[MV_CNT_TAIL_READY], __ATOMIC_RELAXED, __HIP_MEMORY_SCOPE_AGENT);
                                asm volatile("" ::: "memory");
                                const unsigned long long a1 = __hip_atomic_load(&counters[MV_CNT_N_MINSDF], __ATOMIC_RELAXED, __HIP_MEMORY_SCOPE_AGENT);
                                if (a0 == a1 && r1 == a1) {
                                    rows = (long long)a1 * tp.n_steps;
                                    n_items = (int)a1;
                                    if (wgs >= (unsigned long long)gridDim.x) break;
                                }
                                __builtin_amdgcn_s_sleep(127);
                            }
                            if (take >= rows) take = -1;
                            break;
                        }
                        if (!tail.spin) break;
                        __builtin_amdgcn_s_sleep(127); __builtin_amdgcn_s_sleep(127); __builtin_amdgcn_s_sleep(127); __builtin_amdgcn_s_sleep(127);
                    }
                    s_n[0] = (int)take; s_n[1] = n_items;
                }
                __syncthreads();
                const int take = s_n[0];
                if (take < 0) break;
                h_items = s_n[1];
                h_left = 1;
                h_chunk = take;
                ++h_units;
            }
            {
                const long long total = (long long)h_items * tp.n_steps, q0 = (long long)h_chunk;
                h_nr = (int)min((long long)ROWS, total - q0);
                if (tid < ROWS) {
                    float* p = lds.pts + tid * 3;
                    if (tid < h_nr) {
                        const long long q = q0 + tid;
                        const int it = (int)(q / tp.n_steps), i = (int)(q - (long long)it * tp.n_steps);
                        const int g2 = __hip_atomic_load(&w_list_min[it], __ATOMIC_RELAXED, __HIP_MEMORY_SCOPE_AGENT) & 0x0fffffff;
                        const float* cc = cam_loc + 3 * (g2 / P);
                        const float* dd = dirs + 3 * (size_t)g2;
                        const float zmin = __hip_atomic_load(&w_zmin[g2], __ATOMIC_RELAXED, __HIP_MEMORY_SCOPE_AGENT);
                        const float zmax = __hip_atomic_load(&w_zmax[g2], __ATOMIC_RELAXED, __HIP_MEMORY_SCOPE_AGENT);
                        const float z = tail.steps[i] * (zmax - zmin) + zmin;
                        p[0] = cc[0] + z * dd[0]; p[1] = cc[1] + z * dd[1]; p[2] = cc[2] + z * dd[2];
                        h_svi = (long long)it * tp.n_steps + i;
                    } else { p[0] = 0.f; p[1] = 0.f; p[2] = 0.f; }
                }
                n = h_nr;
                --h_left;
            }
            __syncthreads();
        }
        mv_eval_dispatch<MT, NTW, NW, NET, (MT == 1 || (MT <= 2 && !std::is_same<NET, MvNet>::value))>(net, (n + 15) >> 4, lds.act, lds.pe, lds.pts, lds.sdfv, tid);
        if (helping) {
            if (tid < h_nr) tail.sv[h_svi] = lds.sdfv[tid];
            __syncthreads();
            continue;
        }
        if (w == 0) {
            int used = 0;
            if (phase != 3) {
                const float vs = req_s ? mv_clamp(lds.sdfv[row_s], -tp.dist_clip, tp.dist_clip) : 0.f;
                const float ve = req_e ? mv_clamp(lds.sdfv[row_e], -tp.dist_clip, tp.dist_clip) : 0.f;
                const bool had_s = req_s, had_e = req_e;
                bool end_iter = false;
                if (phase == 0) { next_s = vs; next_e = ve; }
                else {
                    if (phase == 1) { next_s = vs; next_e = ve; k = 0; bo_s = false; bo_e = false; }
                    else { if (req_s) next_s = vs; if (req_e) next_e = ve; k++; }
                    for (;;) {
                        const bool np_s = next_s < 0.f, np_e = next_e < 0.f;
                        if (!(k < tp.line_step_iters && (np_s || np_e))) { end_iter = true; break; }
                        const float coef = lss1 / (float)(1 << k);
                        if (np_s) { acc_s -= coef * curr_s; ts = acc_s; bo_s = true; }
                        if (np_e) { acc_e += coef * curr_e; te = acc_e; bo_e = true; }
                        const int dd = k - lvl0;
                        const int rs = (np_s && had_s && dd >= 0 && dd < 3) ? (dd == 0 ? sr_s[0] : (dd == 1 ? sr_s[1] : sr_s[2])) : -1;
                        const int re = (np_e && had_e && dd >= 0 && dd < 3) ? (dd == 0 ? sr_e[0] : (dd == 1 ? sr_e[1] : sr_e[2])) : -1;
                        if (rs >= 0) { next_s = mv_clamp(lds.sdfv[rs], -tp.dist_clip, tp.dist_clip); used++; }
                        if (re >= 0) { next_e = mv_clamp(lds.sdfv[re], -tp.dist_clip, tp.dist_clip); used++; }
                        req_s = np_s && rs < 0; req_e = np_e && re < 0;
                        if (req_s || req_e) { phase = 2; break; }
                        k++;
                    }
                    if (end_iter) {
                        unf_s = unf_s && (acc_s < acc_e);
                        unf_e = unf_e && (acc_s < acc_e);
                        hard_s = bo_s; hard_e = bo_e;
                    }
                }
                if (phase == 0 || end_iter) {
                    curr_s = unf_s ? next_s : 0.f;
                    curr_e = unf_e ? next_e : 0.f;
                    if (curr_s <= tp.thr) curr_s = 0.f;
                    if (curr_e <= tp.thr) curr_e = 0.f;
                    unf_s = unf_s && (curr_s > tp.thr);
                    unf_e = unf_e && (curr_e > tp.thr);
                    if ((!unf_s && !unf_e) || iters == tp.st_iters) {
                        phase = 3; req_s = false; req_e = false;
                    } else {
                        iters++;
                        acc_s = acc_s + curr_s;
                        acc_e = acc_e - curr_e;
                        req_s = unf_s; req_e = unf_e; ts = acc_s; te = acc_e;
                        phase = 1;
                    }
                }
            }
            for (int o = 32; o > 0; o >>= 1) used += __shfl_xor(used, o);
            if (lane == 0) nrows_total += (unsigned long long)used;
        }
    }

    if (tail.enable) {
        if (tid == 0 && h_units) atomicAdd(&counters[MV_CNT_TAIL_ROWS], (unsigned long long)h_units * (unsigned long long)ROWS);
        if (tail.probe && tid == 0) {
            unsigned* pr = tail.probe + 4 * blockIdx.x;
            pr[0] = n_rounds; pr[1] = h_units; pr[2] = (unsigned)(clk1 - clk0); pr[3] = (unsigned)((long long)wall_clock64() - clk1);
        }
    }
}

struct SampleCtx {
    const float* cam_loc; const float* dirs; int R, P, training;
    const float* intervals; const float* steps;
    float* o_points; uint8_t* o_mask; float* o_dists;
    const float* w_zmin; const float* w_zmax;
    float* sec_state;
    int* sec_list;
    float* sv;
    int* list_rest; int* src_rest;
    int n_first;
    unsigned long long* counters;
};

struct RowSeg { const int* list; const int* src; int cnt_index, i0, ni, blocks; int unit_rows; };

template <int MT, int NTW, int NW, class NET>
__device__ void mv_eval_rows(const NET& net, const MvTraceParams& tp, const SampleCtx& c, const RowSeg& sg, long long q0, float* smem, int n_list) {
    constexpr int ROWS = 16 * MT;
    const int tid = threadIdx.x;
    const int n_steps = tp.n_steps, ni = sg.ni;
    const long long total = (long long)n_list * ni;
    if (q0 >= total) return;
    const int nr = (int)min((long long)ROWS, total - q0);
    TraceLds lds = mv_carve<NET>(smem, ROWS, net.S, 3 + 6 * net.multires, 0);
    long long svi = 0;
    if (tid < ROWS) {
        float* p = lds.pts + tid * 3;
        if (tid < nr) {
            const long long q = q0 + tid;
            const int it = (int)(q / ni), i = sg.i0 + (int)(q - (long long)it * ni);
            const int e = sg.list[it];
            const int gid = e & 0x0fffffff;
            const bool samp = (e >> 28) & MV_ITEM_SAMPLER;
            const float* cc = c.cam_loc + 3 * (gid / c.P);
            const float* d = c.dirs + 3 * (size_t)gid;
            const float zmin = c.w_zmin[gid], zmax = c.w_zmax[gid];
            const float z = samp ? (zmin + c.intervals[i] * (zmax - zmin))
                                 : (c.steps[i] * (zmax - zmin) + zmin);
            p[0] = cc[0] + z * d[0]; p[1] = cc[1] + z * d[1]; p[2] = cc[2] + z * d[2];
            svi = (long long)(sg.src ? sg.src[it] : it) * n_steps + i;
        } else { p[0] = 0.f; p[1] = 0.f; p[2] = 0.f; }
    }
    __syncthreads();
    mv_eval_dispatch<MT, NTW, NW>(net, (nr + 15) >> 4, lds.act, lds.pe, lds.pts, lds.sdfv, tid);
    if (tid < nr) c.sv[svi] = lds.sdfv[tid];
}

__device__ __forceinline__ int mv_first_where(const float* __restrict__ sv, int n, int lane, int what) {
    for (int base = 0; base < n; base += 64) {
        const int i = base + lane;
        const float v = i < n ? sv[i] : 1.0f;
        const unsigned long long m = __ballot(what == 0 ? (v < 0.f) : (!(v > 0.f) && !(v < 0.f)));
        if (m) return base + __builtin_ctzll(m);
    }
    return -1;
}
__device__ __forceinline__ int mv_first_argmin(const float* __restrict__ sv, int n, int lane) {
    float bv = INFINITY; int bi = 0x7fffffff;
    for (int i = lane; i < n; i += 64) { const float v = sv[i]; if (v < bv) { bv = v; bi = i; } }
    for (int o = 32; o > 0; o >>= 1) {
        const float ov = __shfl_xor(bv, o); const int oi = __shfl_xor(bi, o);
        if (ov < bv || (ov == bv && oi < bi)) { bv = ov; bi = oi; }
    }
    return bi == 0x7fffffff ? 0 : bi;
}

#define MV_RED_WAVES 16
__global__ __launch_bounds__(64 * MV_RED_WAVES) void k_reduce_items(MvTraceParams tp, SampleCtx c, const int* __restrict__ list, const int* __restrict__ src,
                                                                  int cnt_index, int mode) {
    __shared__ int s_cat[MV_RED_WAVES];
    __shared__ unsigned long long s_base[2];
    const int n_list = (int)c.counters[cnt_index];
    const int lane = threadIdx.x & 63, w = threadIdx.x >> 6;
    const int it = blockIdx.x * MV_RED_WAVES + w;
// ... 99 lines not shown
    if (r0 >= n_list) return;
    const int n = min(ROWS, n_list - r0);
    TraceLds lds = mv_carve<NET, (SPHERE && NTW < 4)>(smem, ROWS, net.S, 3 + 6 * net.multires, 0);
    const bool mine = tid < n;
    int gid = 0;
    float cc[3] = {0, 0, 0}, d[3] = {0, 0, 0}, z_low = 0, z_high = 0, sdf_low = 0, sdf_high = 1, z_pred = 0;
    if (mine) {
        gid = c.sec_list[r0 + tid];
        const int b = gid / c.P;
        for (int i = 0; i < 3; ++i) { cc[i] = c.cam_loc[3 * b + i]; d[i] = c.dirs[3 * (size_t)gid + i]; }
        z_low = c.sec_state[gid]; z_high = c.sec_state[(size_t)c.R + gid];
        sdf_low = c.sec_state[2 * (size_t)c.R + gid]; sdf_high = c.sec_state[3 * (size_t)c.R + gid];
        z_pred = -sdf_low * (z_high - z_low) / (sdf_high - sdf_low) + z_low;
    }
    for (int it = 0; it < tp.n_secant; ++it) {
        if (tid < ROWS) { float* p = lds.pts + tid * 3; p[0] = cc[0] + z_pred * d[0]; p[1] = cc[1] + z_pred * d[1]; p[2] = cc[2] + z_pred * d[2]; }
        __syncthreads();
        mv_eval_dispatch<MT, NTW, NW, NET, SPHERE>(net, (n + 15) >> 4, lds.act, lds.pe, lds.pts, lds.sdfv, tid);
        if (mine) {
            const float sm = lds.sdfv[tid];
            if (sm > 0.f) { z_low = z_pred; sdf_low = sm; }
            if (sm < 0.f) { z_high = z_pred; sdf_high = sm; }
            z_pred = -sdf_low * (z_high - z_low) / (sdf_high - sdf_low) + z_low;
        }
    }
    if (mine) {
        c.o_dists[gid] = z_pred;
        c.o_points[3 * (size_t)gid + 0] = cc[0] + z_pred * d[0];
        c.o_points[3 * (size_t)gid + 1] = cc[1] + z_pred * d[1];
        c.o_points[3 * (size_t)gid + 2] = cc[2] + z_pred * d[2];
    }
    if (tid == 0) atomicAdd(&c.counters[MV_CNT_ROWS_SECANT], (unsigned long long)n * (unsigned long long)tp.n_secant);
}

template <class NET> struct mv_net_wt { static constexpr int v = 1; };
template <int NS, int WT> struct mv_net_wt<MvNetBs<NS, WT>> { static constexpr int v = WT; };
template <int MT, int NTW, int NW, class NET>
__global__ __launch_bounds__(64 * NW, (mv_net_wt<NET>::v == 3 && NTW == 2 && MT <= 2 && NW == 8) ? 4 : NW / 4) void k_ray_samples(NET net, MvTraceParams tp, SampleCtx c, RowSeg s0, RowSeg s1, int sec_blocks) {
    extern __shared__ __attribute__((aligned(16))) float smem[];
    int b = blockIdx.x;
    if (b < sec_blocks) {
        mv_secant_rays<(MT > 1 ? 1 : MT), NTW, NW, NET>(net, tp, c, (int)c.counters[MV_CNT_N_SECANT], b, smem);
        return;
    }
    b -= sec_blocks;
    const bool first = b < s0.blocks;
    if (!first && b - s0.blocks >= s1.blocks) return;
    const RowSeg sg = first ? s0 : s1;
    long long q0 = (long long)(first ? b : b - s0.blocks) * (16 * MT);
    const int n_list = (int)c.counters[sg.cnt_index];
    if (sg.unit_rows > 0) {
        if (q0 >= (long long)n_list * sg.ni + 16 * MT) return;
        __shared__ long long s_q0;
        if (threadIdx.x == 0) s_q0 = (long long)atomicAdd(&c.counters[MV_CNT_TAIL_NEXT], (unsigned long long)(16 * MT));
        __syncthreads();
        q0 = s_q0;
    }
    mv_eval_rows<MT, NTW, NW, NET>(net, tp, c, sg, q0, smem, n_list);
}
template <int MT, int NTW, int NW, class NET>
__global__ __launch_bounds__(64 * NW) void k_secant_chains(NET net, MvTraceParams tp, SampleCtx c) {
    extern __shared__ __attribute__((aligned(16))) float smem[];
    mv_secant_rays<MT, NTW, NW, NET, true>(net, tp, c, (int)c.counters[MV_CNT_N_SECANT], blockIdx.x, smem);
}
const MvTraceSwitches& mv_trace_switches() {
    static const MvTraceSwitches sw = mv_trace_switches_from_env([](const char* name) -> const char* { return getenv(name); }, mv_dev_env);
    return sw;
}
static unsigned* g_tail_probe = nullptr;
extern "C" void mv_trace_set_tail_probe(unsigned* buf) { g_tail_probe = buf; }
static int mv_cu_count() {
    static int n = 0;
    if (n == 0) {
        int dev = 0, v = 0;
        if (hipGetDevice(&dev) != hipSuccess || hipDeviceGetAttribute(&v, hipDeviceAttributeMultiprocessorCount, dev) != hipSuccess || v <= 0) { (void)hipGetLastError(); v = 1; }
        n = v;
    }
    return n;
}

struct TraceCall {
    int engine, R, P, training;
    bool tail, no_tail;
    const MvTraceParams* tp;
    const float *cam_loc, *dirs, *intervals, *steps;
    const uint8_t* om;
    float *points, *dists;
    uint8_t* mask;
    void* ws; unsigned long long* counters; hipStream_t stream;
};

static thread_local int g_last_grid[2] = {0, 0};
void mv_trace_last_grid(int out[2]) { out[0] = g_last_grid[0]; out[1] = g_last_grid[1]; }

template <int MT, int NTW, int NW, class NET>
static hipError_t launch_stage1(const NET& net, const TraceCall& t) {
    const MvTraceWs w = mv_trace_ws(t.R, t.tp->n_steps);
    TailCtx tail = {};
    if (t.tail) tail = {t.steps, mv_ws_at<float>(t.ws, w.sv_min), 16 * MT, 1, 1, mv_tail_stop_left(t.R, MT, mv_trace_switches()), g_tail_probe};
    const size_t lds1 = mv_trace_lds_bytes(net.S, net.multires, MT, mv_act_rows<NET>(16 * MT, NTW < 4));
    static size_t set1 = 0;
    if (lds1 > set1) {
        hipError_t e = hipFuncSetAttribute((const void*)k_sphere_trace<MT, NTW, NW, NET>, hipFuncAttributeMaxDynamicSharedMemorySize, (int)lds1);
        if (e != hipSuccess) return e;
        set1 = lds1;
    }
    hipLaunchKernelGGL((k_sphere_trace<MT, NTW, NW, NET>), dim3(mv_sphere_grid(t.R, MT)), dim3(64 * NW), lds1, t.stream, net, *t.tp, t.cam_loc, t.dirs, t.om, t.R, t.P,
                       t.training, t.points, t.mask, t.dists, mv_ws_at<float>(t.ws, w.w_zmin), mv_ws_at<float>(t.ws, w.w_zmax), mv_ws_at<int>(t.ws, w.w_list),
                       mv_ws_at<int>(t.ws, w.w_list_min), t.counters, tail);
    return hipGetLastError();
}

template <int MT, int NTW, int NW, class NET>
static hipError_t launch_stage2(const NET& net, const TraceCall& t, int part) {
    const MvTraceParams& tp = *t.tp;
    const MvTraceWs w = mv_trace_ws(t.R, tp.n_steps);
    const size_t lds2 = mv_trace_lds_bytes(net.S, net.multires, MT, mv_act_rows<NET>(16 * MT));
    static size_t set2 = 0;
    if (lds2 > set2) {
        hipError_t e = hipFuncSetAttribute((const void*)k_ray_samples<MT, NTW, NW, NET>, hipFuncAttributeMaxDynamicSharedMemorySize, (int)lds2);
        if (e != hipSuccess) return e;
        set2 = lds2;
    }
    const int n = tp.n_steps, nf = mv_first_window(n, mv_trace_switches());
    const MvSampleGrids g = mv_sample_grids(t.R, n, nf, MT, t.training, t.tail, MV_RED_WAVES);
    int *w_list = mv_ws_at<int>(t.ws, w.w_list), *w_list_min = mv_ws_at<int>(t.ws, w.w_list_min);
    SampleCtx c;
    c.cam_loc = t.cam_loc; c.dirs = t.dirs; c.R = t.R; c.P = t.P; c.training = t.training; c.intervals = t.intervals; c.steps = t.steps;
    c.o_points = t.points; c.o_mask = t.mask; c.o_dists = t.dists; c.w_zmin = mv_ws_at<float>(t.ws, w.w_zmin); c.w_zmax = mv_ws_at<float>(t.ws, w.w_zmax);
    c.sec_state = mv_ws_at<float>(t.ws, w.sec_state); c.sec_list = mv_ws_at<int>(t.ws, w.sec_list); c.sv = mv_ws_at<float>(t.ws, w.sv); c.counters = t.counters;
    c.list_rest = mv_ws_at<int>(t.ws, w.list_rest); c.src_rest = mv_ws_at<int>(t.ws, w.src_rest); c.n_first = nf;
    const RowSeg none = {nullptr, nullptr, 0, 0, 1, 0, 0};
    const dim3 wg(64 * NW), red_wg(64 * MV_RED_WAVES);
    if (part == 1) {
        const RowSeg first = {w_list, nullptr, (int)MV_CNT_N_SAMPLER, 0, nf, g.first, 0};
        hipLaunchKernelGGL((k_ray_samples<MT, NTW, NW, NET>), dim3(g.first), wg, lds2, t.stream, net, tp, c, first, none, 0);
        hipLaunchKernelGGL(k_reduce_items, dim3(g.red), red_wg, 0, t.stream, tp, c, w_list, (const int*)nullptr, (int)MV_CNT_N_SAMPLER, 0);
        if (nf < n) {
            const RowSeg rest = {c.list_rest, c.src_rest, (int)MV_CNT_N_SAMPLER_REST, nf, n - nf, g.rest, 0};
            hipLaunchKernelGGL((k_ray_samples<MT, NTW, NW, NET>), dim3(g.rest), wg, lds2, t.stream, net, tp, c, rest, none, 0);
            hipLaunchKernelGGL(k_reduce_items, dim3(g.red), red_wg, 0, t.stream, tp, c, c.list_rest, c.src_rest, (int)MV_CNT_N_SAMPLER_REST, 1);
        }
    } else if (part == 8) {
        hipLaunchKernelGGL((k_ray_samples<MT, NTW, NW, NET>), dim3(g.sec), wg, lds2, t.stream, net, tp, c, none, none, g.sec);
        g_last_grid[0] = g.sec; g_last_grid[1] = 0;
    } else if (part == 2 || t.training) {
        if (part == 4 || t.tail) c.sv = mv_ws_at<float>(t.ws, w.sv_min);
        const int sec = part == 2 ? g.sec : 0;
        const RowSeg minsdf = {w_list_min, nullptr, (int)MV_CNT_N_MINSDF, 0, n, g.minsdf, t.tail ? 1 : 0};
        hipLaunchKernelGGL((k_ray_samples<MT, NTW, NW, NET>), dim3(sec + g.minsdf), wg, lds2, t.stream, net, tp, c, minsdf, none, sec);
        g_last_grid[0] = sec; g_last_grid[1] = g.minsdf;
        if (t.training) hipLaunchKernelGGL(k_reduce_items, dim3(g.red), red_wg, 0, t.stream, tp, c, w_list_min, (const int*)nullptr, (int)MV_CNT_N_MINSDF, 2);
    }
    return hipGetLastError();
}

template <int MT, int NTW, int NW, class NET>
static hipError_t launch_secant(const NET& net, const TraceCall& t) {
    const MvTraceParams& tp = *t.tp;
    const MvTraceWs w = mv_trace_ws(t.R, tp.n_steps);
    const size_t lds = mv_trace_lds_bytes(net.S, net.multires, MT, mv_act_rows<NET>(16 * MT, NTW < 4));
    static size_t set = 0;
    if (lds > set) {
        hipError_t e = hipFuncSetAttribute((const void*)k_secant_chains<MT, NTW, NW, NET>, hipFuncAttributeMaxDynamicSharedMemorySize, (int)lds);
        if (e != hipSuccess) return e;
        set = lds;
    }
    SampleCtx c = {};
    c.cam_loc = t.cam_loc; c.dirs = t.dirs; c.R = t.R; c.P = t.P; c.training = t.training; c.intervals = t.intervals; c.steps = t.steps;
    c.o_points = t.points; c.o_mask = t.mask; c.o_dists = t.dists; c.w_zmin = mv_ws_at<float>(t.ws, w.w_zmin); c.w_zmax = mv_ws_at<float>(t.ws, w.w_zmax);
    c.sec_state = mv_ws_at<float>(t.ws, w.sec_state); c.sec_list = mv_ws_at<int>(t.ws, w.sec_list); c.sv = mv_ws_at<float>(t.ws, w.sv); c.counters = t.counters;
    c.list_rest = mv_ws_at<int>(t.ws, w.list_rest); c.src_rest = mv_ws_at<int>(t.ws, w.src_rest); c.n_first = tp.n_steps;
    const int sec = (t.R + 16 * MT - 1) / (16 * MT);
    hipLaunchKernelGGL((k_secant_chains<MT, NTW, NW, NET>), dim3(sec), dim3(64 * NW), lds, t.stream, net, tp, c);
    g_last_grid[0] = sec; g_last_grid[1] = 0;
    return hipGetLastError();
}

#define MV_S1(ON_, MT_, NTW_, NW_) case mv_inst_key(MT_, NTW_, NW_): if constexpr (ON_) return launch_stage1<MT_, NTW_, NW_>(net, t); break
#define MV_S2(ON_, MT_, NTW_, NW_) case mv_inst_key(MT_, NTW_, NW_): if constexpr (ON_) return launch_stage2<MT_, NTW_, NW_>(net, t, part); break
template <class NET>
static hipError_t mv_launch_inst(const MvInst& r, const NET& net, const TraceCall& t, int part) {
    constexpr bool f32 = std::is_same<NET, MvNet>::value, nw16 = MV_SPHERE_NW16 != 0 && mv_net_wt<NET>::v == 3;
    if (r.rc) return hipErrorInvalidValue;
    if (part == 16) {
        if (r.nw == 16) { if constexpr (nw16) { if (r.mt == 1 && r.ntw == 1) return launch_secant<1, 1, 16>(net, t); } return hipErrorInvalidValue; }
        part = 8;
    }
    if (part == 0) switch (mv_inst_key(r.mt, r.ntw, r.nw)) {
        MV_S1(nw16, 1, 1, 16); MV_S1(!nw16, 1, 2, 8); MV_S1(true, 2, 2, 8); MV_S1(true, 4, 2, 8); MV_S1(true, 1, 4, 8); MV_S1(true, 2, 4, 8);
        MV_S1(f32, 1, 4, 4); MV_S1(f32, 2, 4, 4); MV_S1(f32, 4, 4, 4);
    } else switch (mv_inst_key(r.mt, r.ntw, r.nw)) {
        MV_S2(true, 1, 2, 8); MV_S2(true, 2, 2, 8); MV_S2(true, 4, 2, 8); MV_S2(true, 1, 4, 8); MV_S2(true, 2, 4, 8);
        MV_S2(f32, 1, 4, 4); MV_S2(f32, 2, 4, 4); MV_S2(f32, 4, 4, 4);
    }
    return hipErrorInvalidValue;
}
#undef MV_S1
#undef MV_S2

template <class NET>
static hipError_t mv_trace_launch(int stages, const NET& net, TraceCall t, int mt, int mt_samples) {
    const MvTraceSwitches& sw = mv_trace_switches();
    const int maxnt = mv_hidden_nt(net);
    const MvInst s1 = mv_route_sphere(t.engine, maxnt, mt);
    if (s1.rc) return hipErrorInvalidValue;
    t.tail = !t.no_tail && mv_tail_on(t.engine, t.training, t.steps != nullptr, t.R, s1.mt, mv_cu_count(), sw);
    hipError_t e = (stages & 1) ? mv_launch_inst(s1, net, t, 0) : hipSuccess;
    for (int part = 1; part <= 16 && e == hipSuccess; part <<= 1)
        if ((stages >> 1) & part)
            e = mv_launch_inst(part == 16 ? mv_route_secant(t.engine, maxnt, mt_samples, t.R, sw) : mv_route_samples(t.engine, maxnt, mt_samples, t.R, part, sw), net, t, part);
    return e;
}

struct GenRay {
    float acc_s, acc_e, next_s, next_e, curr_s, curr_e, t0, t1, ts, te;
    int iters, k, phase, flags, pad0, pad1;
};

__device__ __forceinline__ void mv_gen_emit(const GenRay& g, const float* c, const float* d, uint8_t* req, float* pts) {
    const bool rs = g.flags & 4, re = g.flags & 8;
    req[0] = rs ? 1 : 0; req[1] = re ? 1 : 0;
    pts[0] = c[0] + g.ts * d[0]; pts[1] = c[1] + g.ts * d[1]; pts[2] = c[2] + g.ts * d[2];
    pts[3] = c[0] + g.te * d[0]; pts[4] = c[1] + g.te * d[1]; pts[5] = c[2] + g.te * d[2];
}

__global__ void k_gen_init(MvTraceParams tp, const float* __restrict__ cam_loc, const float* __restrict__ dirs, const uint8_t* __restrict__ om,
                           int R, int P, GenRay* __restrict__ state, uint8_t* __restrict__ req, float* __restrict__ pts) {
    const int gid = blockIdx.x * blockDim.x + threadIdx.x;
    if (gid >= R) return;
    float c[3], d[3];
    for (int i = 0; i < 3; ++i) { c[i] = cam_loc[3 * (gid / P) + i]; d[i] = dirs[3 * (size_t)gid + i]; }
    GenRay g;
    const bool isect = mv_sphere_isect(c, d, tp.r, g.t0, g.t1);
    g.acc_s = isect ? g.t0 : 0.f; g.acc_e = isect ? g.t1 : 0.f;
    g.next_s = g.next_e = g.curr_s = g.curr_e = 0.f;
    g.ts = g.acc_s; g.te = g.acc_e;
    g.iters = 0; g.k = 0; g.phase = isect ? 0 : 3;
    g.flags = (isect ? (1 | 2 | 4 | 8 | 16) : 0) | (om[gid] ? 32 : 0);
    g.pad0 = g.pad1 = 0;
    state[gid] = g;
    mv_gen_emit(g, c, d, req + 2 * (size_t)gid, pts + 6 * (size_t)gid);
}

__global__ void k_gen_step(MvTraceParams tp, const float* __restrict__ cam_loc, const float* __restrict__ dirs, int R, int P,
                           GenRay* __restrict__ state, const float* __restrict__ vals, uint8_t* __restrict__ req, float* __restrict__ pts,
                           unsigned long long* __restrict__ counters) {
    const int gid = blockIdx.x * blockDim.x + threadIdx.x;
    int nreq = 0;
    if (gid < R) {
        GenRay g = state[gid];
        if (g.phase != 3) {
            bool unf_s = g.flags & 1, unf_e = g.flags & 2;
            const bool req_s = g.flags & 4, req_e = g.flags & 8;
            nreq = (req_s ? 1 : 0) + (req_e ? 1 : 0);
            const float vs = req_s ? mv_clamp(vals[2 * (size_t)gid], -tp.dist_clip, tp.dist_clip) : 0.f;
            const float ve = req_e ? mv_clamp(vals[2 * (size_t)gid + 1], -tp.dist_clip, tp.dist_clip) : 0.f;
            bool nreq_s = false, nreq_e = false, end_iter = false;
            if (g.phase == 0) { g.next_s = vs; g.next_e = ve; }
            else if (g.phase == 1) { g.next_s = vs; g.next_e = ve; g.k = 0; }
            else { if (req_s) g.next_s = vs; if (req_e) g.next_e = ve; g.k++; }
            if (g.phase != 0) {
                const bool np_s = g.next_s < 0.f, np_e = g.next_e < 0.f;
                if (g.k < tp.line_step_iters && (np_s || np_e)) {
                    const float coef = (1.0f - tp.line_search_step) / (float)(1 << g.k);
                    nreq_s = np_s; nreq_e = np_e;
                    if (np_s) { g.acc_s -= coef * g.curr_s; g.ts = g.acc_s; }
                    if (np_e) { g.acc_e += coef * g.curr_e; g.te = g.acc_e; }
                    g.phase = 2;
                } else {
                    end_iter = true;
                    unf_s = unf_s && (g.acc_s < g.acc_e);
                    unf_e = unf_e && (g.acc_s < g.acc_e);
                }
            }
            if (g.phase == 0 || end_iter) {
                g.curr_s = unf_s ? g.next_s : 0.f;
                g.curr_e = unf_e ? g.next_e : 0.f;
                if (g.curr_s <= tp.thr) g.curr_s = 0.f;
                if (g.curr_e <= tp.thr) g.curr_e = 0.f;
                unf_s = unf_s && (g.curr_s > tp.thr);
                unf_e = unf_e && (g.curr_e > tp.thr);
                if ((!unf_s && !unf_e) || g.iters == tp.st_iters) {
                    g.phase = 3; nreq_s = false; nreq_e = false;
                } else {
                    g.iters++;
                    g.acc_s = g.acc_s + g.curr_s;
                    g.acc_e = g.acc_e - g.curr_e;
                    nreq_s = unf_s; nreq_e = unf_e; g.ts = g.acc_s; g.te = g.acc_e;
                    g.phase = 1;
                }
            }
            g.flags = (g.flags & (16 | 32)) | (unf_s ? 1 : 0) | (unf_e ? 2 : 0) | (nreq_s ? 4 : 0) | (nreq_e ? 8 : 0);
            state[gid] = g;
// ... 53 lines not shown
    __shared__ int base[2];
    const int tid = threadIdx.x, lane = tid & 63, w = tid >> 6;
    if (tid < 2) base[tid] = 0;
    __syncthreads();
    for (int r0 = 0; r0 < R; r0 += 1024) {
        const int gid = r0 + tid;
        const int e = gid < R ? scratch[gid] : -1;
        const bool smp = e >= 0 && ((e >> 28) & MV_ITEM_SAMPLER), mn = e >= 0 && ((e >> 28) & MV_ITEM_MINSDF);
        const unsigned long long bs = __ballot(smp), bm = __ballot(mn), lt = (1ull << lane) - 1ull;
        if (lane == 0) { wsum[0][w] = __popcll(bs); wsum[1][w] = __popcll(bm); }
        __syncthreads();
        int os = base[0], omn = base[1];
        for (int j = 0; j < w; ++j) { os += wsum[0][j]; omn += wsum[1][j]; }
        if (smp) w_list[os + __popcll(bs & lt)] = e;
        if (mn) w_list_min[omn + __popcll(bm & lt)] = e;
        __syncthreads();
        if (tid == 0) { for (int j = 0; j < 16; ++j) { base[0] += wsum[0][j]; base[1] += wsum[1][j]; } }
        __syncthreads();
    }
    if (tid == 0) { counters[MV_CNT_N_SAMPLER] = (unsigned long long)base[0]; counters[MV_CNT_N_MINSDF] = (unsigned long long)base[1]; }
}

__global__ void k_gen_rows(int n_list, int n_steps, const int* __restrict__ list, const float* __restrict__ cam_loc, const float* __restrict__ dirs,
                           int P, const float* __restrict__ zs , int is_sampler, const float* __restrict__ w_zmin,
                           const float* __restrict__ w_zmax, float* __restrict__ out) {
    const long long q = (long long)blockIdx.x * blockDim.x + threadIdx.x;
    if (q >= (long long)n_list * n_steps) return;
    const int it = (int)(q / n_steps), i = (int)(q - (long long)it * n_steps);
    const int gid = list[it] & 0x0fffffff;
    const float* cc = cam_loc + 3 * (gid / P);
    const float* d = dirs + 3 * (size_t)gid;
    const float zmin = w_zmin[gid], zmax = w_zmax[gid];
    const float z = is_sampler ? (zmin + zs[i] * (zmax - zmin)) : (zs[i] * (zmax - zmin) + zmin);
    out[3 * q + 0] = cc[0] + z * d[0]; out[3 * q + 1] = cc[1] + z * d[1]; out[3 * q + 2] = cc[2] + z * d[2];
}

__global__ void k_gen_secant(int op, int n_sec, int R, int P, const int* __restrict__ sec_list, float* __restrict__ sec_state,
                             const float* __restrict__ cam_loc, const float* __restrict__ dirs, const float* __restrict__ vals,
                             float* __restrict__ pts_out, float* __restrict__ o_points, float* __restrict__ o_dists) {
    const int i = blockIdx.x * blockDim.x + threadIdx.x;
    if (i >= n_sec) return;
    const int gid = sec_list[i];
    float z_low = sec_state[gid], z_high = sec_state[(size_t)R + gid], sdf_low = sec_state[2 * (size_t)R + gid], sdf_high = sec_state[3 * (size_t)R + gid];
    float z_pred = -sdf_low * (z_high - z_low) / (sdf_high - sdf_low) + z_low;
    const float* cc = cam_loc + 3 * (gid / P);
    const float* d = dirs + 3 * (size_t)gid;
    if (op == 1) {
        const float sm = vals[i];
        if (sm > 0.f) { sec_state[gid] = z_pred; sec_state[2 * (size_t)R + gid] = sm; }
        if (sm < 0.f) { sec_state[(size_t)R + gid] = z_pred; sec_state[3 * (size_t)R + gid] = sm; }
        return;
    }
    float* o = op == 0 ? pts_out + 3 * (size_t)i : o_points + 3 * (size_t)gid;
    o[0] = cc[0] + z_pred * d[0]; o[1] = cc[1] + z_pred * d[1]; o[2] = cc[2] + z_pred * d[2];
    if (op == 2) o_dists[gid] = z_pred;
}

__global__ __launch_bounds__(1024) void k_gen_sort_list(int* __restrict__ list, const unsigned long long* __restrict__ counters, int cnt_index,
                                                        uint8_t* __restrict__ marks, int R) {
    __shared__ int wsum[16];
    __shared__ int base;
    const int n = (int)counters[cnt_index], tid = threadIdx.x, lane = tid & 63, w = tid >> 6;
    for (int i = tid; i < n; i += 1024) marks[list[i]] = 1;
    if (tid == 0) base = 0;
    __syncthreads();
    for (int r0 = 0; r0 < R; r0 += 1024) {
        const int gid = r0 + tid;
        const bool m = gid < R && marks[gid];
        const unsigned long long b = __ballot(m), lt = (1ull << lane) - 1ull;
        if (lane == 0) wsum[w] = __popcll(b);
        __syncthreads();
        int o = base;
        for (int j = 0; j < w; ++j) o += wsum[j];
        if (m) list[o + __popcll(b & lt)] = gid;
        __syncthreads();
        if (tid == 0) for (int j = 0; j < 16; ++j) base += wsum[j];
        __syncthreads();
    }
}

extern "C" {

size_t mvsdf_trace_workspace_bytes_n(int R, int n_steps) { return mv_trace_ws(R, n_steps).total; }
size_t mvsdf_trace_workspace_bytes(int R) { return mvsdf_trace_workspace_bytes_n(R, 128); }

static int trace_impl(int stages, const MvsdfNetDesc* desc, const MvsdfTraceParams* tp, const float* cam_loc, const float* ray_dirs,
                      const uint8_t* object_mask, int B, int P, int training, const float* intervals, const float* minsdf_steps,
                      float* points, uint8_t* mask, float* dists, unsigned long long* counters, void* workspace,
                      size_t workspace_bytes, int mt, int mt_samples, void* stream) {
    const MvEngineClass ec = mv_trace_engine(desc ? desc->trace_dtype : 0, false);
    if (ec.rc) return mv_fail(ec.rc, ec.why);
    return mv_with_trace_net(desc, ec.engine, [&](const auto& net) {
        if (!tp || !cam_loc || !ray_dirs || !object_mask || !intervals || !points || !mask || !dists || !counters || !workspace)
            return mv_fail(-1, "mvsdf_trace: null argument");
        if (B <= 0 || P <= 0 || (long long)B * P >= (1 << 28)) return mv_fail(-1, "mvsdf_trace: B*P out of range");
        if (training && !minsdf_steps) return mv_fail(-1, "mvsdf_trace: training needs minsdf_steps");
        if (tp->n_steps < 2 || tp->n_steps > 1024 || tp->line_step_iters < 0 || tp->line_step_iters > 30)
            return mv_fail(-1, "mvsdf_trace: tracer parameters out of range");
        const int R = B * P;
        if (workspace_bytes < mvsdf_trace_workspace_bytes_n(R, tp->n_steps)) return mv_fail(-1, "mvsdf_trace: workspace too small");
        hipStream_t s = (hipStream_t)stream;
        hipError_t e = hipSuccess;
        if ((stages & 1) && !(stages & 0x100)) e = hipMemsetAsync(counters, 0, 16 * sizeof(unsigned long long), s);
        if (e != hipSuccess) return mv_check(e, "mvsdf_trace: memset");
        const TraceCall t = {ec.engine, R, P, training, false, (stages & 0x200) != 0, tp, cam_loc, ray_dirs, intervals, minsdf_steps ? minsdf_steps : intervals, object_mask,
                             points, dists, mask, workspace, counters, s};
        return mv_check(mv_trace_launch(stages, net, t, mt, mt_samples), "mvsdf_trace");
    });
}

int mvsdf_trace(const MvsdfNetDesc* desc, const MvsdfTraceParams* tp, const float* cam_loc, const float* ray_dirs,
                const uint8_t* object_mask, int B, int P, int training, const float* intervals, const float* minsdf_steps,
                float* points, uint8_t* mask, float* dists, unsigned long long* counters, void* workspace,
                size_t workspace_bytes, int mt, int mt_samples, void* stream) {
    return trace_impl(7, desc, tp, cam_loc, ray_dirs, object_mask, B, P, training, intervals, minsdf_steps, points, mask, dists, counters,
                      workspace, workspace_bytes, mt, mt_samples, stream);
}

int mvsdf_trace_stage(int stage, const MvsdfNetDesc* desc, const MvsdfTraceParams* tp, const float* cam_loc, const float* ray_dirs,
                      const uint8_t* object_mask, int B, int P, int training, const float* intervals, const float* minsdf_steps,
                      float* points, uint8_t* mask, float* dists, unsigned long long* counters, void* workspace,
                      size_t workspace_bytes, int mt, int mt_samples, void* stream) {
    if (stage < 1 || stage > 7) return mv_fail(-1, "mvsdf_trace_stage: stage must be 1..7");
    static const int bits[8] = {0, 1, 6, 2, 4, 8, 16, 32};
    return trace_impl(bits[stage], desc, tp, cam_loc, ray_dirs, object_mask, B, P, training, intervals, minsdf_steps, points, mask, dists, counters,
                      workspace, workspace_bytes, mt, mt_samples, stream);
}

int mv_trace_stage1_prezeroed(const MvsdfNetDesc* desc, const MvsdfTraceParams* tp, const float* cam_loc, const float* ray_dirs, const uint8_t* object_mask,
                              int B, int P, int training, const float* intervals, const float* minsdf_steps, float* points, uint8_t* mask, float* dists,
                              unsigned long long* counters, void* workspace, size_t workspace_bytes, int mt, int mt_samples, void* stream) {
    return trace_impl(1 | 0x100, desc, tp, cam_loc, ray_dirs, object_mask, B, P, training, intervals, minsdf_steps, points, mask, dists, counters,
                      workspace, workspace_bytes, mt, mt_samples, stream);
}
int mv_trace_stage_notail(int stage, const MvsdfNetDesc* desc, const MvsdfTraceParams* tp, const float* cam_loc, const float* ray_dirs, const uint8_t* object_mask,
                          int B, int P, int training, const float* intervals, const float* minsdf_steps, float* points, uint8_t* mask, float* dists,
                          unsigned long long* counters, void* workspace, size_t workspace_bytes, int mt, int mt_samples, void* stream) {
    static const int bits[8] = {0, 1 | 0x100, 0, 0, 0, 8, 16, 32};
    if (stage < 1 || stage > 7 || !bits[stage]) return mv_fail(-1, "mv_trace_stage_notail: stage must be 1, 5, 6 or 7");
    return trace_impl(bits[stage] | 0x200, desc, tp, cam_loc, ray_dirs, object_mask, B, P, training, intervals, minsdf_steps, points, mask, dists, counters,
                      workspace, workspace_bytes, mt, mt_samples, stream);
}

size_t mvsdf_tracegen_state_bytes(int R) { return (size_t)(R > 0 ? R : 0) * sizeof(GenRay); }

static int tracegen_check(const MvsdfTraceParams* tp, int B, int P) {
    if (!tp || B <= 0 || P <= 0 || (long long)B * P >= (1 << 28)) return mv_fail(-1, "mvsdf_tracegen: bad sizes");
    if (tp->n_steps < 2 || tp->n_steps > 1024 || tp->line_step_iters < 0 || tp->line_step_iters > 30) return mv_fail(-1, "mvsdf_tracegen: tracer parameters out of range");
    return 0;
}

int mvsdf_tracegen_init(const MvsdfTraceParams* tp, const float* cam_loc, const float* ray_dirs, const uint8_t* object_mask, int B, int P,
                        void* state, uint8_t* req, float* pts, unsigned long long* counters, void* stream) {
    int rc = tracegen_check(tp, B, P);
    if (rc) return rc;
    if (!cam_loc || !ray_dirs || !object_mask || !state || !req || !pts || !counters) return mv_fail(-1, "mvsdf_tracegen_init: null argument");
    const int R = B * P;
    hipStream_t s = (hipStream_t)stream;
    hipError_t e = hipMemsetAsync(counters, 0, 16 * sizeof(unsigned long long), s);
    if (e != hipSuccess) return mv_check(e, "mvsdf_tracegen_init: memset");
    hipLaunchKernelGGL(k_gen_init, dim3((R + 255) / 256), dim3(256), 0, s, *tp, cam_loc, ray_dirs, object_mask, R, P, (GenRay*)state, req, pts);
    return mv_check(hipGetLastError(), "mvsdf_tracegen_init");
}

int mvsdf_tracegen_step(const MvsdfTraceParams* tp, const float* cam_loc, const float* ray_dirs, int B, int P, void* state, const float* vals,
                        uint8_t* req, float* pts, unsigned long long* counters, void* stream) {
    int rc = tracegen_check(tp, B, P);
    if (rc) return rc;
    if (!cam_loc || !ray_dirs || !state || !vals || !req || !pts || !counters) return mv_fail(-1, "mvsdf_tracegen_step: null argument");
    const int R = B * P;
    hipLaunchKernelGGL(k_gen_step, dim3((R + 255) / 256), dim3(256), 0, (hipStream_t)stream, *tp, cam_loc, ray_dirs, R, P, (GenRay*)state, vals, req, pts, counters);
    return mv_check(hipGetLastError(), "mvsdf_tracegen_step");
}

int mvsdf_tracegen_finish(const MvsdfTraceParams* tp, const float* cam_loc, const float* ray_dirs, int B, int P, int training, const void* state,
                          float* points, uint8_t* mask, float* dists, unsigned long long* counters, void* workspace, size_t workspace_bytes,
                          void* stream) {
    int rc = tracegen_check(tp, B, P);
    if (rc) return rc;
    const int R = B * P;
    if (!cam_loc || !ray_dirs || !state || !points || !mask || !dists || !counters || !workspace) return mv_fail(-1, "mvsdf_tracegen_finish: null argument");
    if (workspace_bytes < mvsdf_trace_workspace_bytes_n(R, tp->n_steps)) return mv_fail(-1, "mvsdf_tracegen_finish: workspace too small");
    const MvTraceWs w = mv_trace_ws(R, tp->n_steps);
    hipStream_t s = (hipStream_t)stream;
    int* scratch = mv_ws_at<int>(workspace, w.sec_list);
    int* w_list_min = mv_ws_at<int>(workspace, w.w_list_min);
    hipLaunchKernelGGL(k_gen_finish, dim3((R + 255) / 256), dim3(256), 0, s, *tp, cam_loc, ray_dirs, R, P, training, (const GenRay*)state, points, mask,
                       dists, mv_ws_at<float>(workspace, w.w_zmin), mv_ws_at<float>(workspace, w.w_zmax), scratch, w_list_min, counters);
    hipLaunchKernelGGL(k_gen_lists, dim3(1), dim3(1024), 0, s, R, mv_ws_at<int>(workspace, w.w_list), w_list_min, scratch, counters);
    return mv_check(hipGetLastError(), "mvsdf_tracegen_finish");
}

int mvsdf_tracegen_rows(const MvsdfTraceParams* tp, int kind, const float* cam_loc, const float* ray_dirs, int B, int P, const float* zs, int n_list,
                        void* workspace, float* out_pts, void* stream) {
    int rc = tracegen_check(tp, B, P);
    if (rc) return rc;
    if (!cam_loc || !ray_dirs || !zs || !workspace || !out_pts || n_list <= 0 || n_list > B * P || kind < 0 || kind > 1)
        return mv_fail(-1, "mvsdf_tracegen_rows: bad arguments");
    const MvTraceWs w = mv_trace_ws(B * P, tp->n_steps);
    const long long total = (long long)n_list * tp->n_steps;
    hipLaunchKernelGGL(k_gen_rows, dim3((unsigned)((total + 255) / 256)), dim3(256), 0, (hipStream_t)stream, n_list, tp->n_steps,
                       mv_ws_at<int>(workspace, kind == 0 ? w.w_list : w.w_list_min), cam_loc, ray_dirs, P, zs, kind == 0 ? 1 : 0,
                       mv_ws_at<float>(workspace, w.w_zmin), mv_ws_at<float>(workspace, w.w_zmax), out_pts);
    return mv_check(hipGetLastError(), "mvsdf_tracegen_rows");
}

int mvsdf_tracegen_reduce(const MvsdfTraceParams* tp, int kind, const float* cam_loc, const float* ray_dirs, int B, int P, int training,
                          const float* intervals, const float* minsdf_steps, const float* sv, float* points, uint8_t* mask, float* dists,
                          unsigned long long* counters, void* workspace, uint8_t* marks, void* stream) {
    int rc = tracegen_check(tp, B, P);
    if (rc) return rc;
    const int R = B * P;
    if (!cam_loc || !ray_dirs || !intervals || !sv || !points || !mask || !dists || !counters || !workspace || kind < 0 || kind > 1 || (kind == 0 && !marks))
        return mv_fail(-1, "mvsdf_tracegen_reduce: bad arguments");
    const MvTraceWs w = mv_trace_ws(R, tp->n_steps);
    int* w_list = mv_ws_at<int>(workspace, w.w_list);
    int* w_list_min = mv_ws_at<int>(workspace, w.w_list_min);
    SampleCtx c;
    c.cam_loc = cam_loc; c.dirs = ray_dirs; c.R = R; c.P = P; c.training = training; c.intervals = intervals;
    c.steps = minsdf_steps ? minsdf_steps : intervals;
    c.o_points = points; c.o_mask = mask; c.o_dists = dists; c.w_zmin = mv_ws_at<float>(workspace, w.w_zmin); c.w_zmax = mv_ws_at<float>(workspace, w.w_zmax);
    c.sec_state = mv_ws_at<float>(workspace, w.sec_state); c.sec_list = mv_ws_at<int>(workspace, w.sec_list); c.sv = (float*)sv; c.counters = counters;
    c.list_rest = mv_ws_at<int>(workspace, w.list_rest); c.src_rest = mv_ws_at<int>(workspace, w.src_rest); c.n_first = tp->n_steps;
    hipStream_t s = (hipStream_t)stream;
// ... 28 lines not shown
```

mvsdf_amd/csrc/trace_params.h:

```cpp
#pragma once
#include "../../include/mvsdf_hip.h"
typedef MvsdfTraceParams MvTraceParams;
#define MV_CNT_ROWS_SPHERE MVSDF_CNT_ROWS_SPHERE
#define MV_CNT_ROWS_SAMPLER MVSDF_CNT_ROWS_SAMPLER
#define MV_CNT_ROWS_SECANT MVSDF_CNT_ROWS_SECANT
#define MV_CNT_ROWS_MINSDF MVSDF_CNT_ROWS_MINSDF
#define MV_CNT_N_SECANT MVSDF_CNT_N_SECANT
#define MV_CNT_N_SAMPLER MVSDF_CNT_N_SAMPLER
#define MV_CNT_N_MINSDF MVSDF_CNT_N_MINSDF
#define MV_CNT_N_SAMPLER_REST MVSDF_CNT_N_SAMPLER_REST
#define MV_CNT_ROWS_SAMPLER_EVAL MVSDF_CNT_ROWS_SAMPLER_EVAL
#define MV_CNT_TAIL_NEXT MVSDF_CNT_TAIL_NEXT
#define MV_CNT_TAIL_READY MVSDF_CNT_TAIL_READY
#define MV_CNT_TAIL_WGS MVSDF_CNT_TAIL_WGS
#define MV_CNT_TAIL_ROWS MVSDF_CNT_TAIL_ROWS
#define MV_ITEM_SAMPLER 1
#define MV_ITEM_MINSDF 2
#define MV_ITEM_OM 4
```

mvsdf_amd/csrc/trace_route.h:

```cpp
#pragma once
#include <stddef.h>
#include <stdlib.h>

struct MvTraceSwitches {
    int tail = 1;
    int tail_stop = -1;
    int nfirst = 12;
    int mt_first = 0;
    int bf_carry = 0;
};
inline MvTraceSwitches mv_trace_switches_from_env(const char* (*product_env)(const char*), const char* (*dev_env)(const char*)) {
    MvTraceSwitches v;
    const char* e;
    if ((e = product_env("MVSDF_TAIL"))) v.tail = atoi(e);
    if ((e = dev_env("MVSDF_TAIL_STOP"))) v.tail_stop = atoi(e);
    if ((e = dev_env("MVSDF_NFIRST"))) v.nfirst = atoi(e);
    if (v.nfirst < 2) v.nfirst = 2;
    if ((e = dev_env("MVSDF_MT_FIRST"))) v.mt_first = atoi(e);
    if ((e = dev_env("MVSDF_BF_CARRY"))) v.bf_carry = atoi(e) != 0;
    return v;
}

enum MvTraceEngine {
    MV_ENG_F32 = 0,
// ... 9 lines not shown
        case 1: return {-2, 0, col0 ? "mvsdf_sdf_col0: " MV_DTYPE1_GONE : "mvsdf_trace: " MV_DTYPE1_GONE};
        case 3: return {0, MV_ENG_BS2, nullptr};
        case 4: return {0, MV_ENG_BS3, nullptr};
        case 5: return {0, MV_ENG_X3, nullptr};
        default: return {0, MV_ENG_F32, nullptr};
    }
}

struct MvInst { int rc, mt, ntw, nw, xr; const char* why; };
inline MvInst mv_inst_refuse(int rc, const char* why) { return {rc, 0, 0, 0, 0, why}; }
constexpr int mv_inst_key(int mt, int ntw, int nw) { return (mt * 100 + ntw) * 100 + nw * 2; }
inline MvInst mv_inst_ladder(int engine, int maxnt, int mt) {
    if (maxnt > 16) return {0, mt >= 2 ? 2 : 1, 4, 8, 0, nullptr};
    const int m = mt >= 4 ? 4 : (mt >= 2 ? 2 : 1);
    return (engine != MV_ENG_F32 || maxnt >= 16) ? MvInst{0, m, 2, 8, 0, nullptr} : MvInst{0, m, 4, 4, 0, nullptr};
}
#ifndef MV_SPHERE_NW16
#define MV_SPHERE_NW16 1
#endif
inline MvInst mv_route_sphere(int engine, int maxnt, int mt) {
    if (maxnt > 32) return mv_inst_refuse(1, "network too wide");
    const MvInst r = mv_inst_ladder(engine, maxnt, mt);
    if (MV_SPHERE_NW16 != 0 && engine == MV_ENG_X3 && r.mt == 1 && r.ntw == 2) return {0, 1, 1, 16, 0, nullptr};
    return r;
}
inline MvInst mv_route_samples(int engine, int maxnt, int mt_samples, int R, int part, const MvTraceSwitches& sw) {
    if (maxnt > 32) return mv_inst_refuse(1, "network too wide");
    int mt = mt_samples;
    if (part == 1) mt = sw.mt_first > 0 ? sw.mt_first : (engine == MV_ENG_X3 ? (mt_samples > 2 ? 2 : mt_samples) : (R <= 4096 ? 1 : mt_samples));
    return mv_inst_ladder(engine, maxnt, mt);
}
#ifndef MV_SECANT_NW16
#define MV_SECANT_NW16 1
#endif
inline MvInst mv_route_secant(int engine, int maxnt, int mt_samples, int R, const MvTraceSwitches& sw) {
    const MvInst s = mv_route_sphere(engine, maxnt, 1);
    if (MV_SECANT_NW16 != 0 && s.rc == 0 && s.mt == 1 && s.ntw == 1 && s.nw == 16) return s;
    return mv_route_samples(engine, maxnt, mt_samples, R, 8, sw);
}
inline MvInst mv_route_col0(int engine, int maxnt, int mt, const MvTraceSwitches& sw) {
    if (engine != MV_ENG_F32) {
        if (maxnt > 32) return mv_inst_refuse(-1, "mvsdf_sdf_col0: network too wide");
        MvInst r = mv_inst_ladder(engine, maxnt, mt);
        r.xr = sw.bf_carry != 0;
        return r;
    }
    if (mt != 1 && mt != 2 && mt != 4 && mt != 49) return mv_inst_refuse(-1, "mvsdf_sdf_col0: mt must be 1, 2, 4 (row tiles per workgroup) or 49 (the sphere tracer's carried-ring engine)");
    if (mt != 49) return mv_inst_ladder(engine, maxnt, mt);
    if (maxnt > 16) return mv_inst_refuse(-1, "mvsdf_sdf_col0: mt = 49 needs a hidden width <= 256");
    return {0, 1, 2, 8, 1, nullptr};
}

inline int mv_sphere_grid(int R, int mt1) { return (R + 8 * mt1 - 1) / (8 * mt1); }
inline bool mv_tail_on(int engine, int training, bool steps_given, int R, int mt1, int cus, const MvTraceSwitches& sw) {
    const int need = engine == MV_ENG_F32 ? 1 : ((engine == MV_ENG_X3 && R > 2048) ? 1 : 2);
    return training && steps_given && sw.tail >= need && mv_sphere_grid(R, mt1) <= cus;
}
inline int mv_tail_stop_left(int R, int mt1, const MvTraceSwitches& sw) { return sw.tail_stop >= 0 ? sw.tail_stop : mv_sphere_grid(R, mt1) / 4; }
inline int mv_first_window(int n_steps, const MvTraceSwitches& sw) { return sw.nfirst < n_steps ? sw.nfirst : n_steps; }
struct MvSampleGrids { int first, rest, minsdf, sec, red; };
inline int mv_row_blocks(int R, int per_item, int mt) { return (int)(((long long)R * per_item + 16 * mt - 1) / (16 * mt)); }
inline MvSampleGrids mv_sample_grids(int R, int n_steps, int nf, int mt, int training, bool tail, int red_waves) {
    return {mv_row_blocks(R, nf, mt), nf < n_steps ? mv_row_blocks(R, n_steps - nf, mt) : 0, training ? mv_row_blocks(R, n_steps, mt) + (tail ? 1 : 0) : 0,
            (R + 15) / 16, (R + red_waves - 1) / red_waves};
}
inline size_t mv_tile_lds_floats(int S, int multires, int mt, int act_rows) { return (size_t)act_rows * S + ((16 * mt * (3 + 6 * multires) + 3) & ~3) + 16 * mt * 4 + 16 * mt; }
inline size_t mv_trace_lds_bytes(int S, int multires, int mt, int act_rows) { return mv_tile_lds_floats(S, multires, mt, act_rows) * 4 + 32; }
inline size_t mv_col0_lds_bytes(int S, int multires, int mt) { return mv_tile_lds_floats(S, multires, mt, 16 * mt) * 4; }

struct MvTraceWs {
    size_t w_zmin, w_zmax;
    size_t sec_state;
    size_t w_list, w_list_min;
    size_t sec_list;
    size_t sv;
    size_t list_rest, src_rest;
    size_t sv_min;
    size_t total;
};
inline MvTraceWs mv_trace_ws(int R, int n_steps) {
    const size_t r = 4 * (size_t)(R > 0 ? R : 0), n = n_steps > 0 ? n_steps : 0;
    return {0, r, 2 * r, 6 * r, 7 * r, 8 * r, 9 * r, (9 + n) * r, (10 + n) * r, (11 + n) * r, (11 + 2 * n) * r + 256};
}
template <class T> inline T* mv_ws_at(void* ws, size_t offset) { return (T*)((char*)ws + offset); }
```

mvsdf_amd/model/implicit_differentiable_renderer.py:

```python
import importlib
import os
import weakref

import numpy as np
import torch
import torch.nn as nn

from .. import functional as Fn
from .. import native_step as NS
from ..utils.general import PinnedUniform
from .. import ops
from ..utils import rend_util
from . import conf as _default_conf
from .ray_tracing import NativeSDF, RayTracing
from .sample_network import SampleNetwork

conf = _default_conf
if os.environ.get('IDR_USE_ENV', '0') == '1' and os.environ.get('IDR_CONF', '') != '':
    print('override conf: ', os.environ.get('IDR_CONF'))
    conf = importlib.import_module(os.environ.get('IDR_CONF'))

DEFAULT_TRACE_DTYPE = 'f32x3'


# ... 208 lines not shown

    def __ior__(self, other):
        self._need()
        return super().__ior__(other)

    def __copy__(self):
        return self.copy()

    def __deepcopy__(self, memo):
        import copy as _copy
        return _copy.deepcopy(self.copy(), memo)

    def __reduce__(self):
        return (dict, (self.copy(),))


class PendingOutputs(LazyOutputs):
    _LAZY = ('diff_surf_pts', 'rgb_values', 'grad_theta', 'eikonal_points_hom', 'eikonal_output', 'surf_indicator_output')

    def __init__(self, data, fill, rec, late=None):
        super().__init__(data, fill, late)
        self._mv_rec = rec

    def _materialize(self):
        if self._pending is not None:
            self._pending(self)
            self._pending = None

    def pending_rec(self):
        return self._mv_rec if self._pending is not None else None

    def raw(self, k):
        if self._late is not None and k in self._LATE:
            self._need(k)
        return dict.__getitem__(self, k)


class StepOutputs(LazyOutputs):
    _LAZY = ()

    def __init__(self, data, late):
        super().__init__(data, None, late)


class _StepStats(dict):

    def __init__(self, rec, **kw):
        super().__init__(**kw)
        self._rec = rec

    def __getitem__(self, k):
        if k == 'N' and not dict.__contains__(self, 'N'):
            dict.__setitem__(self, 'N', self._rec.resolve()[0])
        return dict.__getitem__(self, k)

    def get(self, k, default=None):
        return self[k] if (k == 'N' or k in self) else default


class IDRNetwork(nn.Module):
    HOST_STAGE = True
    DEFERRED_STEP = os.environ.get('MVSDF_DEFERRED_STEP', '1') != '0'

    def __init__(self, conf):
        super().__init__()
        self.feature_vector_size = conf.get_int('feature_vector_size')
        self.implicit_network = ImplicitNetwork(self.feature_vector_size, **conf.get_config('implicit_network'))
        self.rendering_network = RenderingNetwork(self.feature_vector_size, **conf.get_config('rendering_network'))
        self.ray_tracer = RayTracing(**conf.get_config('ray_tracer'))
        self.sample_network = SampleNetwork()
        self.object_bounding_sphere = conf.get_float('ray_tracer.object_bounding_sphere')
        self.last_stats = {}
        self.set_trace_dtype(DEFAULT_TRACE_DTYPE)
        self._counts_host = None
        self._counts_event = None
        self._draw = PinnedUniform()
        self._fold_cache = {}
        self._lazy_prev = None
        self.lazy_unused_outputs = False
        self.native_step = os.environ.get('MVSDF_NATIVE_STEP', '1') != '0'
        self.host_stage = type(self).HOST_STAGE
        self.deferred_step = type(self).DEFERRED_STEP
        self.eager_unhit_rows = os.environ.get('MVSDF_EAGER_UNHIT', '0') not in ('', '0')
        self._steps = {}
        self._ones = None

    def set_trace_dtype(self, dtype):
        if dtype not in ops.TRACE_DTYPES:
            raise ValueError('IDRNetwork.set_trace_dtype(%r): expected one of %s' % (dtype, ', '.join(sorted(ops.TRACE_DTYPES))))
        self.trace_dtype = dtype
        self.implicit_network.trace_dtype = dtype
        return self

    def _dsurf_samples(self, input, n_dsurf_points, bb):
        depths, depth_cams = input['depths'], input['depth_cams']
        depths_pack = depths.reshape(-1, depths.shape[-2], depths.shape[-1])
        cams_pack = depth_cams.reshape(-1, 2, 4, 4)
        seed = int(torch.randint(0, 2 ** 62, (1,)).item())
        jitter_rad = 0.1
        on, jit, counts, _ = ops.dsurf_samples(depths_pack, cams_pack, input['size'][:1], input['center'][:1], bb, jitter_rad, seed, n_dsurf_points)
        return on, jit, counts

    def forward(self, input, train_progress=None):
        intrinsics, uv, pose = input['intrinsics'], input['uv'], input['pose']
        object_mask_true = input['object_mask'].reshape(-1)
        prev = self._lazy_prev() if self._lazy_prev is not None else None
        if prev is not None:
            prev._expire()
        self._lazy_prev = None
        if self.training:
            self._check_point_groups(train_progress)
        if self.training and self.native_step and not self.lazy_unused_outputs and self.ray_tracer.events is None and not ops._MINSDF_SIDE_STREAM:
            out = self._forward_native(input, train_progress, object_mask_true)
            if out is not None:
                return out
        object_mask = object_mask_true if conf.use_mask else torch.ones_like(object_mask_true)

        ray_dirs, cam_loc = rend_util.get_camera_params(uv, pose, intrinsics)
        batch_size, num_pixels, _ = ray_dirs.shape
        R = batch_size * num_pixels
        dev = ray_dirs.device

        flat = None
        if self.training:
            flat, plan, (net, rnet) = Fn.fold_networks_flat([self.implicit_network.fold_spec(), self.rendering_network.fold_spec()], self._fold_cache)
            ws = bs = rws = rbs = None
        else:
            (net, ws, bs), (rnet, rws, rbs) = Fn.fold_networks([self.implicit_network.fold_spec(), self.rendering_network.fold_spec()])
        ops.pack_trace_net(net, self.trace_dtype)
        n_dsurf_points, dsurf = 0, None
        if self.training:
            assert train_progress is not None
            if any([conf.d_use_dsurf_on(train_progress), conf.d_use_dsurf_jitter(train_progress),
                    conf.eik_use_dsurf_on(train_progress), conf.eik_use_dsurf_jitter(train_progress)]):
                n_dsurf_points = R // 2
                dsurf = self._dsurf_samples(input, n_dsurf_points, self.object_bounding_sphere)
        sync = {}

        def on_mask(net_mask):
            sync['part'] = ops.partition_rays(net_mask, object_mask if conf.use_mask else None, object_mask_true, ray_dirs)
            if self._counts_host is None:
                self._counts_host = torch.empty(4, dtype=torch.int64).pin_memory()
                self._counts_event = torch.cuda.Event()
            if dsurf is None:
                self._counts_host[:2].copy_(sync['part'][3], non_blocking=True)
            else:
                self._counts_host.copy_(torch.cat([sync['part'][3], dsurf[2]]), non_blocking=True)
            self._counts_event.record()

        deferred = [] if (self.training and self.lazy_unused_outputs) else None
        with torch.no_grad():
            points, network_object_mask, dists = self.ray_tracer(sdf=NativeSDF(net), cam_loc=cam_loc, object_mask=object_mask,
                                                                 ray_directions=ray_dirs, mask_ready=on_mask if self.training else None,
                                                                 defer_minsdf=deferred)
        ray_dirs = ray_dirs.reshape(-1, 3)

        if self.training:
            perm, inv, true_rows, _, view_sorted = sync['part']
        else:
            surface_mask = network_object_mask
            perm = torch.sort((~surface_mask).to(torch.int8), stable=True).indices
            n_hit_dev = surface_mask.sum()
            inv = torch.empty_like(perm)
            inv[perm] = torch.arange(R, device=dev)
        pts_sorted = points[perm]

# ... 89 lines not shown
        key = (B, P, n_ds, str(dev), self.trace_dtype, mt, mt_samples, tpv, bool(conf.use_mask))
        st = self._steps.get(key)
        if st is None:
            vs, gs, bs, skips, multires = inet.fold_spec()
            rvs, rgs, rbs, _, _ = rnet.fold_spec()
            if len(vs) + len(rvs) > NS.STEP_MAX_LAYERS or max(v.shape[0] for v in vs[:-1]) > 512:
                self._steps[key] = False
                return None
            d = NS.StepDesc()
            d.B, d.P, d.n_eik, d.n_ds = B, P, R // 2, n_ds
            d.n_sdf, d.n_render = len(vs), len(rvs)
            for l, v in enumerate(list(vs) + list(rvs)):
                d.N[l], d.K[l] = v.shape
            skips = skips if isinstance(skips, (tuple, list)) else ((skips,) if skips >= 0 else ())
            d.skip_mask = sum(1 << int(sk) for sk in skips)
            d.multires, d.view_spec = multires, rnet.view_spec
            d.trace_dtype = ops.TRACE_DTYPES[self.trace_dtype]
            d.use_object_mask = 1 if conf.use_mask else 0
            d.tp = NS.TraceParams(*tpv)
            d.mt, d.mt_samples = mt, mt_samples
            st = self._steps[key] = NS.NativeStep(d, dev)
        return st or None

    def _forward_native(self, input, train_progress, object_mask_true):
        assert train_progress is not None
        uv, pose, intrinsics = input['uv'], input['pose'], input['intrinsics']
        dev = uv.device
        if not (uv.is_cuda and uv.dtype == torch.float32 and pose.dtype == torch.float32 and intrinsics.dtype == torch.float32 and pose.shape[1:] == (4, 4)):
            return None
        B, P = uv.shape[0], uv.shape[1]
        R = B * P
        use_ds = any([conf.d_use_dsurf_on(train_progress), conf.d_use_dsurf_jitter(train_progress),
                      conf.eik_use_dsurf_on(train_progress), conf.eik_use_dsurf_jitter(train_progress)])
        n_ds = R // 2 if use_ds else 0
        st = self._native_step_for(B, P, n_ds, dev)
        if st is None:
            return None
        rt = self.ray_tracer
        vs, gs, bs, params, live = self._step_params()
        dsurf = self._dsurf_samples(input, n_ds, self.object_bounding_sphere) if use_ds else None
        bb = self.object_bounding_sphere
        n_eik = R // 2
        stage_slot = None
        if isinstance(self._draw, PinnedUniform) and isinstance(rt._draw, PinnedUniform):
            if self.host_stage:
                minsdf_steps, eik, stage, stage_slot = self._draw.pair_staged((rt.n_steps,), 0.0, 1.0, (n_eik, 3), -bb, bb, dev)
            else:
                (minsdf_steps, eik), stage = self._draw.pair((rt.n_steps,), 0.0, 1.0, (n_eik, 3), -bb, bb, dev), None
        else:
            minsdf_steps = rt._draw((rt.n_steps,), 0.0, 1.0, dev)
            eik = self._draw((n_eik, 3), -bb, bb, dev)
            minsdf_steps, eik = minsdf_steps.float().contiguous(), eik.float().contiguous()
            stage = None
        true_u8 = object_mask_true if object_mask_true.dtype == torch.uint8 else (
            object_mask_true.view(torch.uint8) if object_mask_true.dtype == torch.bool else object_mask_true.to(torch.uint8))
        if not true_u8.is_contiguous():
            true_u8 = true_u8.contiguous()
        if conf.use_mask:
            om_u8 = true_u8
        else:
            if self._ones is None or self._ones.numel() != R or self._ones.device != dev:
                self._ones = torch.ones(R, dtype=torch.uint8, device=dev)
            om_u8 = self._ones
        iv = rt.intervals(dev)
        i = st.inputs
        uv_c, pose_c, intr_c = (uv if uv.is_contiguous() else uv.contiguous()), (pose if pose.is_contiguous() else pose.contiguous()), (
            intrinsics if intrinsics.is_contiguous() else intrinsics.contiguous())
        keep = (uv_c, pose_c, intr_c, true_u8, om_u8, iv, minsdf_steps, eik, dsurf)
        i.uv, i.pose, i.intrinsics = uv_c.data_ptr(), pose_c.data_ptr(), intr_c.data_ptr()
        i.object_mask, i.object_mask_true = om_u8.data_ptr(), true_u8.data_ptr()
        i.intervals, i.minsdf_steps, i.eik_points = iv.data_ptr(), minsdf_steps.data_ptr(), eik.data_ptr()
        i.host_stage = stage.data_ptr() if stage is not None else None
        if dsurf is not None:
            i.ds_on, i.ds_jit, i.ds_counts = dsurf[0].data_ptr(), dsurf[1].data_ptr(), dsurf[2].data_ptr()
        else:
            i.ds_on = i.ds_jit = i.ds_counts = None
        rec = NS.StepRecord()
        rec.step, rec.vs, rec.gs, rec.bs, rec.params, rec.live = st, vs, gs, bs, params, live
        rec.prm = st.params(vs, gs, bs)
        rec.d_mask, rec.e_mask = self._group_masks(train_progress, n_eik, n_ds)
        rec.use_geo = not bool(train_progress < conf.phase[0] or conf.disable_rgb_grad)
        rec.inputs_keep = keep
        rec.eager_unhit = bool(self.eager_unhit_rows) or not st.can_defer_unhit
        NS.enqueue_forward(rec)
        if stage_slot is not None:
            stage_slot[2] = (st, rec.seq)
        L, f = st.layout, rec.fwd
        counters = f.b(L.counters, (128,)).view(torch.int64)
        rt.last_counters = counters
        d_ = self.__dict__
        d_['_last_step'] = st
        d_['_last_rec'] = weakref.ref(rec)
        eager = {
            'points': f.f(L.points, (R, 3)),
            'diff_surf_pts': None,
            'rgb_values': None,
            'sdf_output': f.f(L.sdf_output, (R, 1)),
            'network_object_mask': f.b(L.mask, (R,)).view(torch.bool),
            'object_mask': object_mask_true if conf.use_mask else f.b(L.object_mask_out, (R,)).view(torch.bool),
            'object_mask_true': object_mask_true,
            'grad_theta': None,
            'eikonal_points_hom': None,
            'eikonal_output': None,
            'surf_indicator_output': None,
        }

        def materialize(target):
            diff_pts, rgb_values, grad_theta, eik_out, surf = NS.run_step(rec)
            if dsurf is not None and min(int(rec.counts[2]), int(rec.counts[3])) < n_ds:
                raise ValueError("Cannot take a larger sample than population when 'replace=False'")
            nd, _ = rec.keep
            dict.update(target, {'diff_surf_pts': diff_pts, 'rgb_values': rgb_values, 'grad_theta': grad_theta,
                                 'eikonal_points_hom': f.f(L.points_hom, (1, nd, 4, 1)), 'eikonal_output': eik_out, 'surf_indicator_output': surf})

        late = rec.resolve_unhit if rec.unhit_pending else None
        if self.deferred_step and st.can_defer and dsurf is None and torch.is_grad_enabled():
            out = PendingOutputs(eager, materialize, rec, late)
            d_['last_stats'] = _StepStats(rec, R=R, E=st.E, counters=counters)
            return out
        materialize(eager)
        d_['last_stats'] = {'R': R, 'N': rec.N, 'E': st.E, 'counters': counters}
        return StepOutputs(eager, late) if late is not None else eager

    def _step_params(self):
        c = getattr(self, '_param_cache', None)
        inet, rnet = self.implicit_network, self.rendering_network
        if c is not None:
            lins, objs = c[0], c[1]
            if all(m._parameters.get(n) is o for (m, n), o in zip(lins, objs)):
                return c[2]
        vs, gs, bs, _, _ = inet.fold_spec()
        rvs, rgs, rbs, _, _ = rnet.fold_spec()
        vs, gs, bs = list(vs) + list(rvs), list(gs) + list(rgs), list(bs) + list(rbs)
        lins, objs = [], []
        mods = inet._lins() + [getattr(rnet, 'lin' + str(l)) for l in range(rnet.num_layers - 1)]
        for m in mods:
            for n, o in m._parameters.items():
                lins.append((m, n)); objs.append(o)
        params = tuple(vs) + tuple(gs) + tuple(bs)
        res = (vs, gs, bs, params, [p for p in params if p is not None])
        self._param_cache = (lins, objs, res)
        return res

    @staticmethod
    def _check_point_groups(train_progress):
        for term, flags in (('depth', ('d_use_rt_surf', 'd_use_eik', 'd_use_dsurf_on', 'd_use_dsurf_jitter')),
                            ('eikonal', ('eik_use_rt_surf', 'eik_use_eik', 'eik_use_dsurf_on', 'eik_use_dsurf_jitter'))):
            if not any(getattr(conf, f)(train_progress) for f in flags):
                raise ValueError('IDRNetwork.forward: every point group of the %s term is switched off at train_progress %g (conf.%s): '
                                 'the reference fails here (torch.cat of an empty list, idr.py:258-286)' % (term, train_progress, ' / '.join(flags)))

    def _group_masks(self, train_progress, n_eik, n_ds):
        d_flags = (conf.d_use_rt_surf, conf.d_use_eik, conf.d_use_dsurf_on, conf.d_use_dsurf_jitter)
        e_flags = (conf.eik_use_rt_surf, conf.eik_use_eik, conf.eik_use_dsurf_on, conf.eik_use_dsurf_jitter)
        has = (True, n_eik > 0, n_ds > 0, n_ds > 0)
        return (sum(1 << g for g in range(4) if has[g] and d_flags[g](train_progress)),
                sum(1 << g for g in range(4) if has[g] and e_flags[g](train_progress)))

    def _rgb_from_shared(self, shared, ws, bs, points, view_dirs, N, train_progress, row0=0, folded=None):
        defer = self.training and points.requires_grad and points.grad_fn is not None
        y2, normals = Fn.sdf_reuse(shared, ws, bs, points, N, defer_dw=defer, row0=row0)
        feature_vectors = y2[:, 2:]
        if (train_progress is not None and train_progress < conf.phase[0]) or conf.disable_rgb_grad:
            points, normals, view_dirs = [a.detach() for a in (points, normals, view_dirs)]
        return self.rendering_network(points, normals, view_dirs, feature_vectors, folded=folded)

# ... 9 lines not shown
```

mvsdf_amd/native_step.py:

```python
import ctypes as C
import operator

import torch

from ._lib import TraceParams, check, lib

STEP_MAX_LAYERS = 24
_DATA_PTR = torch.Tensor.data_ptr
_VERSION_OF = operator.attrgetter('_version')


class StepDesc(C.Structure):
    _fields_ = [('B', C.c_int), ('P', C.c_int), ('n_eik', C.c_int), ('n_ds', C.c_int), ('n_sdf', C.c_int), ('n_render', C.c_int),
                ('N', C.c_int * STEP_MAX_LAYERS), ('K', C.c_int * STEP_MAX_LAYERS), ('skip_mask', C.c_uint), ('multires', C.c_int),
                ('view_spec', C.c_int), ('trace_dtype', C.c_int), ('use_object_mask', C.c_int), ('tp', TraceParams), ('mt', C.c_int),
                ('mt_samples', C.c_int)]


class StepParams(C.Structure):
    _fields_ = [('v', C.c_void_p * STEP_MAX_LAYERS), ('g', C.c_void_p * STEP_MAX_LAYERS), ('b', C.c_void_p * STEP_MAX_LAYERS)]


class StepInputs(C.Structure):
    _fields_ = [(n, C.c_void_p) for n in ('uv', 'pose', 'intrinsics', 'object_mask', 'object_mask_true', 'intervals', 'minsdf_steps', 'eik_points',
                                          'ds_on', 'ds_jit', 'ds_counts', 'host_stage')]


class StepLayout(C.Structure):
    _fields_ = [(n, C.c_size_t) for n in ('fwd_bytes', 'bwd_bytes', 'ray_dirs', 'cam_loc', 'points', 'mask', 'dists', 'counters', 'object_mask_out',
                                          'rgb_values', 'sdf_output', 'diff_pts', 'eik_out', 'points_hom', 'grad_theta', 'surf', 'perm', 'dflat',
                                          'dflat_floats')]


class LossArgs(C.Structure):
    _fields_ = [('R', C.c_int), ('B', C.c_int), ('N', C.c_int), ('n_grad', C.c_int), ('n_depth', C.c_int), ('n_surf', C.c_int),
                ('net_mask', C.c_void_p), ('obj_mask', C.c_void_p), ('true_mask', C.c_void_p), ('rgb', C.c_void_p), ('rgb_gt', C.c_void_p),
                ('grad_theta', C.c_void_p), ('eik_out', C.c_void_p), ('surf', C.c_void_p), ('diff_pts', C.c_void_p), ('points_hom', C.c_void_p),
                ('feat_on', C.c_int), ('surf_on', C.c_int), ('V', C.c_int), ('C', C.c_int), ('H', C.c_int), ('W', C.c_int),
                ('feat', C.c_void_p), ('feat_strides', C.c_longlong * 4), ('feat_src', C.c_void_p), ('src_strides', C.c_longlong * 5),
                ('cam', C.c_void_p), ('src_cams', C.c_void_p), ('size', C.c_void_p), ('center', C.c_void_p),
                ('depths', C.c_void_p), ('dB', C.c_int), ('dh', C.c_int), ('dw', C.c_int), ('depth_cams', C.c_void_p),
                ('out_thresh_perc', C.c_float), ('far_thresh', C.c_float), ('far_att', C.c_float), ('near_thresh', C.c_float), ('near_att', C.c_float),
                ('w_rgb', C.c_float), ('w_eik', C.c_float), ('w_surf', C.c_float), ('w_feat', C.c_float), ('w_depth', C.c_float),
                ('use_invalid', C.c_int), ('smooth', C.c_float), ('inv_counts', C.c_void_p),
                ('counts_dev', C.c_void_p), ('n_eik', C.c_int), ('n_ds', C.c_int), ('d_mask', C.c_int), ('e_mask', C.c_int)]


class LossLayout(C.Structure):
    _fields_ = [(n, C.c_size_t) for n in ('bytes', 'out', 'hit', 'view_start', 'n_pos', 'loss_pp', 'dpts', 'dist_r', 'weight', 'd_rgb', 'd_grad',
                                          'd_eo', 'd_sf', 's_rgb', 's_grad', 's_eo', 's_sf', 's_diff')]


_bound = False


def _bind():
    global _bound
    L = lib()
    if not _bound:
        L.mvsdf_step_create.argtypes = [C.c_void_p, C.c_void_p, C.POINTER(C.c_void_p)]
        L.mvsdf_step_destroy.argtypes = [C.c_void_p]
        L.mvsdf_step_destroy.restype = None
        L.mvsdf_step_forward.argtypes = [C.c_void_p, C.c_void_p, C.c_void_p, C.c_int, C.c_int, C.c_int, C.c_void_p, C.c_void_p]
        L.mvsdf_step_resolve_unhit.argtypes = [C.c_void_p, C.c_void_p, C.c_void_p]
        L.mvsdf_step_can_defer_unhit.argtypes = [C.c_void_p]
        L.mvsdf_step_last_tracer_grid.argtypes = [C.c_void_p, C.c_void_p]
        L.mvsdf_step_wait_counts.argtypes = [C.c_void_p, C.c_void_p]
        L.mvsdf_step_seq.argtypes = [C.c_void_p]
        L.mvsdf_step_seq.restype = C.c_longlong
        L.mvsdf_step_counts_offset.argtypes = [C.c_void_p]
        L.mvsdf_step_counts_offset.restype = C.c_size_t
        L.mvsdf_step_wait_counts_seq.argtypes = [C.c_void_p, C.c_longlong, C.c_void_p]
        L.mvsdf_step_done_seq.argtypes = [C.c_void_p, C.c_void_p]
        L.mvsdf_step_done_seq.restype = C.c_longlong
        L.mvsdf_step_can_defer.argtypes = [C.c_void_p]
        L.mvsdf_step_saved_offsets.argtypes = [C.c_void_p, C.c_void_p]
        L.mvsdf_step_backward.argtypes = [C.c_void_p, C.c_void_p] + [C.c_int] * 5 + [C.c_void_p] * 10 + [C.c_int, C.c_void_p]
        L.mvsdf_step_set_timing.argtypes = [C.c_void_p, C.c_int]
        L.mvsdf_step_trace_times.argtypes = [C.c_void_p, C.c_void_p]
        L.mvsdf_step_times.argtypes = [C.c_void_p, C.c_void_p]
        L.mvsdf_loss_layout.argtypes = [C.c_void_p, C.c_void_p]
        L.mvsdf_loss_forward.argtypes = [C.c_void_p, C.c_void_p, C.c_void_p]
        L.mvsdf_loss_backward.argtypes = [C.c_void_p] * 9
        _bound = True
    return L


loss_timing = None


def _timed_loss_forward(L, args, blk, dev):
    if loss_timing is None:
        check(L.mvsdf_loss_forward(C.byref(args), blk.data_ptr(), _stream(dev)), 'mvsdf_loss_forward')
        return
    ev = (torch.cuda.Event(enable_timing=True), torch.cuda.Event(enable_timing=True))
    ev[0].record()
    check(L.mvsdf_loss_forward(C.byref(args), blk.data_ptr(), _stream(dev)), 'mvsdf_loss_forward')
    ev[1].record()
    loss_timing.append(ev)


def _region(block, off, nbytes, dtype, shape):
    return block[off:off + nbytes].view(dtype).view(shape)


def _strides(shape):
    st, acc = [], 1
    for n in reversed(shape):
        st.append(acc)
        acc *= max(int(n), 1)
    return tuple(reversed(st))


class Block:
    __slots__ = ('u8', 'f32')

    def __init__(self, nbytes, device):
        self.u8 = torch.empty((nbytes + 3) // 4 * 4, dtype=torch.uint8, device=device)
        self.f32 = self.u8.view(torch.float32)

    def f(self, off, shape):
        return torch.as_strided(self.f32, shape, _strides(shape), off >> 2)

    def b(self, off, shape):
        return torch.as_strided(self.u8, shape, _strides(shape), off)

    def data_ptr(self):
        return self.u8.data_ptr()


def _stream(dev):
    return C.c_void_p(torch._C._cuda_getCurrentRawStream(dev.index if dev.index is not None else torch.cuda.current_device()))


class NativeStep:

    def __init__(self, desc, device):
        L = _bind()
        self.desc, self.device = desc, device
        self.layout = StepLayout()
        h = C.c_void_p()
        check(L.mvsdf_step_create(C.byref(desc), C.byref(self.layout), C.byref(h)), 'mvsdf_step_create')
        self._h = h
        self.R, self.E = desc.B * desc.P, desc.n_eik + 2 * desc.n_ds
        self.Nout = desc.N[desc.n_sdf - 1]
        self.nl = desc.n_sdf + desc.n_render
        self._bwd = None
        self._prm_key, self._prm, self._prm_list, self._prm_src = None, None, None, None
        self._grad_key, self._grad_arrays = None, None
        self._counts = (C.c_longlong * 4)()
        self._counts_peek = (C.c_longlong * 4)()
        self.inputs = StepInputs()
        self.timing = False
        self.can_defer = bool(L.mvsdf_step_can_defer(h))
        self.counts_off = int(L.mvsdf_step_counts_offset(h))
        self.can_defer_unhit = bool(L.mvsdf_step_can_defer_unhit(h))

    def __del__(self):
        h, self._h = getattr(self, '_h', None), None
        if h:
            try:
                lib().mvsdf_step_destroy(h)
            except Exception:
                pass

    def _track(self, vs, gs, bs):
        src = self._prm_src
        if src is None or src[0] is not vs or src[1] is not gs or src[2] is not bs:
            self._prm_src = (vs, gs, bs)
            self._prm_list = list(vs) + [g for g in gs if g is not None] + list(bs)
            self._prm_key = self._grad_key = None

    def params(self, vs, gs, bs):
        self._track(vs, gs, bs)
        key = tuple(map(_DATA_PTR, self._prm_list))
        if key != self._prm_key:
            for p in list(vs) + [g for g in gs if g is not None] + list(bs):
                assert p.is_cuda and p.dtype == torch.float32 and p.is_contiguous(), 'float32 contiguous parameters on the GPU expected'
            prm = StepParams()
            for l, (v, g, b) in enumerate(zip(vs, gs, bs)):
                prm.v[l], prm.g[l], prm.b[l] = v.data_ptr(), (g.data_ptr() if g is not None else None), b.data_ptr()
            self._prm_key, self._prm = key, prm
        return self._prm

    def grad_arrays(self, vs, gs, bs):
        self._track(vs, gs, bs)
        ps = self._prm_list
        grads = [p.grad for p in ps]
        for g_ in grads:
            if g_ is None:
                return None
        key = tuple(map(_DATA_PTR, grads))
        if key != self._grad_key:
            if not all(p.grad.is_cuda and p.grad.dtype == torch.float32 and p.grad.is_contiguous() for p in ps):
                return None
            n = STEP_MAX_LAYERS
            dv, dg, db = (C.c_void_p * n)(), (C.c_void_p * n)(), (C.c_void_p * n)()
            for l, (v, g, b) in enumerate(zip(vs, gs, bs)):
                dv[l], dg[l], db[l] = v.grad.data_ptr(), (g.grad.data_ptr() if g is not None else None), b.grad.data_ptr()
            self._grad_key, self._grad_arrays = key, (dv, dg, db)
        return self._grad_arrays

    def forward(self, prm, d_mask, e_mask, eager_unhit=True):
        fwd = Block(self.layout.fwd_bytes, self.device)
        check(lib().mvsdf_step_forward(self._h, C.byref(prm), C.byref(self.inputs), d_mask, e_mask, 1 if eager_unhit else 0, fwd.data_ptr(),
                                       _stream(self.device)), 'mvsdf_step_forward')
        return fwd

    def resolve_unhit(self, fwd):
        check(lib().mvsdf_step_resolve_unhit(self._h, fwd.data_ptr(), _stream(self.device)), 'mvsdf_step_resolve_unhit')

    def last_tracer_grid(self):
        out = (C.c_int * 2)()
        check(lib().mvsdf_step_last_tracer_grid(self._h, out), 'mvsdf_step_last_tracer_grid')
        return int(out[0]), int(out[1])

    def wait_counts(self):
        check(lib().mvsdf_step_wait_counts(self._h, self._counts), 'mvsdf_step_wait_counts')
        return tuple(self._counts)

    def seq(self):
        return int(lib().mvsdf_step_seq(self._h))

    def wait_counts_seq(self, seq, fwd):
        rc = lib().mvsdf_step_wait_counts_seq(self._h, seq, self._counts)
        if rc == -4:
            torch.cuda.current_stream(self.device).synchronize()
            return tuple(int(v) for v in fwd.u8[self.counts_off:self.counts_off + 32].view(torch.int64).cpu())
        check(rc, 'mvsdf_step_wait_counts_seq')
        return tuple(self._counts)

    def partition_done(self, seq):
        rc = lib().mvsdf_step_wait_counts_seq(self._h, seq, self._counts)
        if rc != -4:
            check(rc, 'mvsdf_step_wait_counts_seq')

    def saved_offsets(self):
        out = (C.c_size_t * 6)()
        check(lib().mvsdf_step_saved_offsets(self._h, out), 'mvsdf_step_saved_offsets')
        return dict(zip(('x_eval', 'y_eval', 'n_eval', 'view_sorted', 'render_ctx', 'rgb_sorted'), (int(v) for v in out)))

    def hint_N(self):
        return int(self._counts_peek[0]) if lib().mvsdf_step_done_seq(self._h, self._counts_peek) > 0 else -1


    def bwd_block(self):
        if self._bwd is None:
            self._bwd = torch.empty(self.layout.bwd_bytes, dtype=torch.uint8, device=self.device)
        return self._bwd

    def backward(self, prm, N, n_true, d_mask, e_mask, use_geo, ups, fwd, targets, accumulate):
        p = [None if t is None else C.c_void_p(t if isinstance(t, int) else t.data_ptr()) for t in ups]
        dv, dg, db = targets
        check(lib().mvsdf_step_backward(self._h, C.byref(prm), N, n_true, d_mask, e_mask, 1 if use_geo else 0, p[0], p[1], p[2], p[3], p[4],
                                        fwd.data_ptr(), self.bwd_block().data_ptr(), dv, dg, db, 1 if accumulate else 0, _stream(self.device)),
              'mvsdf_step_backward')

    def set_timing(self, on):
        check(lib().mvsdf_step_set_timing(self._h, 1 if on else 0), 'mvsdf_step_set_timing')
        self.timing = bool(on)

    def trace_times(self):
        ms = (C.c_float * 3)()
        check(lib().mvsdf_step_trace_times(self._h, ms), 'mvsdf_step_trace_times')
        return tuple(ms)

    def times(self):
        ms = (C.c_float * 6)()
        check(lib().mvsdf_step_times(self._h, ms), 'mvsdf_step_times')
        return tuple(ms)


class StepRecord:
    __slots__ = ('step', 'fwd', 'prm', 'params', 'N', 'n_true', 'counts', 'd_mask', 'e_mask', 'use_geo', 'n_layers', 'vs', 'gs', 'bs', 'keep', 'done', 'versions',
                 'seq', 'inputs_keep', 'live', 'eager_unhit', 'unhit_pending', '__weakref__')

    def __init__(self):
        self.fwd = self.N = self.n_true = self.counts = self.seq = None
        self.done = False
        self.eager_unhit = True
        self.unhit_pending = False

    def resolve_unhit(self):
        if self.unhit_pending:
            self.unhit_pending = False
            self.step.resolve_unhit(self.fwd)

    def resolve(self):
        if self.N is None:
            self.counts = self.step.wait_counts_seq(self.seq, self.fwd)
# ... 276 lines not shown
```

Before: 1.516 million.

## Cut long-tail sphere tracing rounds and resume spilled rays on a side stream

Adds a sphere-trace cut mode. After a capped number of rounds, rays still needing evaluation are spilled with their full per-ray state to a workspace buffer, and a resume pass continues them on a separate non-blocking stream. This overlaps the straggler tail with the later sampler and secant stages on the main stream. It is enabled automatically through a heuristic when the sphere grid occupies between half and all of the CUs with the x3 engine. The cost is a larger workspace, extra counters, a spill/resume round trip and cross-stream event synchronisation.

```diff
diff --git a/include/mvsdf_hip.h b/include/mvsdf_hip.h
--- a/include/mvsdf_hip.h
+++ b/include/mvsdf_hip.h
@@ -48,7 +48,10 @@
     MVSDF_CNT_TAIL_NEXT = 9,
     MVSDF_CNT_TAIL_READY = 10,
     MVSDF_CNT_TAIL_WGS = 11,
-    MVSDF_CNT_TAIL_ROWS = 12
+    MVSDF_CNT_TAIL_ROWS = 12,
+    MVSDF_CNT_N_SPILL = 13,
+    MVSDF_CNT_N_SAMPLER_LATE = 14,
+    MVSDF_CNT_LATE_ROUNDS = 15
 };
 
 int mvsdf_version(void);
@@ -88,6 +91,11 @@
                       const uint8_t* object_mask, int B, int P, int training, const float* intervals, const float* minsdf_steps,
                       float* points, uint8_t* mask, float* dists, unsigned long long* counters, void* workspace,
                       size_t workspace_bytes, int mt, int mt_samples, void* stream);
+
+size_t mvsdf_trace_cut_workspace_bytes(int R, int n_steps);
+int mvsdf_trace_cut_stage(int stage, int max_rounds, const MvsdfNetDesc* net, const MvsdfTraceParams* tp, const float* cam_loc, const float* ray_dirs,
+                          const uint8_t* object_mask, int B, int P, int training, const float* intervals, const float* minsdf_steps, float* points, uint8_t* mask,
+                          float* dists, unsigned long long* counters, void* workspace, size_t workspace_bytes, int mt, int mt_samples, void* stream);
 
 size_t mvsdf_tracegen_state_bytes(int R);
 int mvsdf_tracegen_init(const MvsdfTraceParams* tp, const float* cam_loc, const float* ray_dirs, const uint8_t* object_mask, int B, int P,
@@ -227,6 +235,7 @@
 int mvsdf_step_forward(void* step, const MvsdfStepParams* prm, const MvsdfStepInputs* in, int d_mask, int e_mask, int mode, void* fwd, void* stream);
 int mvsdf_step_resolve_unhit(void* step, void* fwd, void* stream);
 int mvsdf_step_can_defer_unhit(void* step);
+int mvsdf_step_set_sphere_cut(void* step, int enable, int max_rounds);
 int mvsdf_step_last_tracer_grid(void* step, int out[2]);
 int mvsdf_step_wait_counts(void* step, long long counts[4]);
 #define MVSDF_STEP_COUNT_RING 64
diff --git a/mvsdf_amd/_lib.py b/mvsdf_amd/_lib.py
--- a/mvsdf_amd/_lib.py
+++ b/mvsdf_amd/_lib.py
@@ -38,6 +38,8 @@
         L.mvsdf_trace_workspace_bytes.argtypes = [C.c_int]
         L.mvsdf_trace_workspace_bytes_n.restype = C.c_size_t
         L.mvsdf_trace_workspace_bytes_n.argtypes = [C.c_int, C.c_int]
+        L.mvsdf_trace_cut_workspace_bytes.restype = C.c_size_t
+        L.mvsdf_trace_cut_workspace_bytes.argtypes = [C.c_int, C.c_int]
         for fn in ('mvsdf_sdf_ctx_floats', 'mvsdf_sdf_bwd_ws_floats', 'mvsdf_render_ctx_floats', 'mvsdf_render_bwd_ws_floats'):
             getattr(L, fn).restype = C.c_size_t
         L.mvsdf_adam_ws_floats.restype = C.c_size_t
@@ -162,14 +164,14 @@
 
 EXPORTS = [
     'mvsdf_version', 'mvsdf_abi_struct_sizes', 'mvsdf_last_error', 'mvsdf_packed_floats', 'mvsdf_fold_pack', 'mvsdf_fold_backward', 'mvsdf_fold_pack_net', 'mvsdf_fold_backward_net', 'mvsdf_packed_bf16_bytes', 'mvsdf_pack_bf16w_net', 'mvsdf_pack_bf16s_net', 'mvsdf_pack_bf16x3_net', 'mvsdf_pack_bf16x3t_net',
-    'mvsdf_sdf_col0', 'mvsdf_camera_rays', 'mvsdf_sphere_intersection', 'mvsdf_trace_workspace_bytes', 'mvsdf_trace_workspace_bytes_n', 'mvsdf_trace', 'mvsdf_trace_stage', 'mvsdf_det_math',
+    'mvsdf_sdf_col0', 'mvsdf_camera_rays', 'mvsdf_sphere_intersection', 'mvsdf_trace_workspace_bytes', 'mvsdf_trace_workspace_bytes_n', 'mvsdf_trace', 'mvsdf_trace_stage', 'mvsdf_trace_cut_workspace_bytes', 'mvsdf_trace_cut_stage', 'mvsdf_det_math',
     'mvsdf_tracegen_state_bytes', 'mvsdf_tracegen_init', 'mvsdf_tracegen_step', 'mvsdf_tracegen_finish', 'mvsdf_tracegen_rows', 'mvsdf_tracegen_reduce',
     'mvsdf_tracegen_secant',
     'mvsdf_sdf_ctx_floats', 'mvsdf_sdf_forward', 'mvsdf_sdf_bwd_ws_floats', 'mvsdf_sdf_backward', 'mvsdf_sdf_backward_pair', 'mvsdf_sdf_backward_finish',
     'mvsdf_feat_corr', 'mvsdf_depth_carve', 'mvsdf_loss_terms', 'mvsdf_loss_prep', 'mvsdf_loss_scale', 'mvsdf_adam_ws_floats', 'mvsdf_adam_step', 'mvsdf_adam_step_scaled', 'mvsdf_adam_step_fused',
     'mvsdf_partition_rays', 'mvsdf_step_outputs', 'mvsdf_step_backward_inputs', 'mvsdf_step_backward_fbar', 'mvsdf_dsurf_select', 'mvsdf_dsurf_points',
     'mvsdf_render_ctx_floats', 'mvsdf_render_bwd_ws_floats', 'mvsdf_render_forward', 'mvsdf_render_backward',
-    'mvsdf_step_create', 'mvsdf_step_destroy', 'mvsdf_step_forward', 'mvsdf_step_resolve_unhit', 'mvsdf_step_can_defer_unhit', 'mvsdf_step_last_tracer_grid', 'mvsdf_step_wait_counts', 'mvsdf_step_backward', 'mvsdf_step_set_timing', 'mvsdf_step_trace_times', 'mvsdf_step_times',
+    'mvsdf_step_create', 'mvsdf_step_destroy', 'mvsdf_step_forward', 'mvsdf_step_resolve_unhit', 'mvsdf_step_can_defer_unhit', 'mvsdf_step_set_sphere_cut', 'mvsdf_step_last_tracer_grid', 'mvsdf_step_wait_counts', 'mvsdf_step_backward', 'mvsdf_step_set_timing', 'mvsdf_step_trace_times', 'mvsdf_step_times',
     'mvsdf_step_seq', 'mvsdf_step_counts_offset', 'mvsdf_step_wait_counts_seq', 'mvsdf_step_done_seq', 'mvsdf_step_can_defer', 'mvsdf_step_saved_offsets',
     'mvsdf_loss_layout', 'mvsdf_loss_forward', 'mvsdf_loss_backward',
     'mvsdf_mc_workspace_bytes', 'mvsdf_mc_count', 'mvsdf_mc_emit', 'mvsdf_mesh_cc_workspace_bytes', 'mvsdf_mesh_components', 'mvsdf_mesh_select',
diff --git a/mvsdf_amd/csrc/step_driver.hip b/mvsdf_amd/csrc/step_driver.hip
--- a/mvsdf_amd/csrc/step_driver.hip
+++ b/mvsdf_amd/csrc/step_driver.hip
@@ -48,6 +48,9 @@
     int split_rows;
     int can_lazy;
     int last_grid[2];
+    int cut_enable, cut_rounds, cut_on;
+    hipStream_t late;
+    hipEvent_t ev_cut, ev_late;
 };
 
 void make_descs(const Step& st, const MvsdfStepParams* prm, const char* fwd, MvsdfNetDesc* sdf, MvsdfNetDesc* sdfT, MvsdfNetDesc* rnd, MvsdfNetDesc* rndT) {
@@ -127,6 +130,7 @@
     st->R = d.B * d.P; st->E = d.n_eik + 2 * d.n_ds; st->M = st->R + st->E; st->nl = nl;
     st->Nout = d.N[d.n_sdf - 1]; st->K0r = d.K[d.n_sdf];
     st->split_rows = -1;
+    st->cut_enable = -1; st->cut_on = -1;
     const int R = st->R, M = st->M;
     MvsdfNetDesc sdf, sdfT, rnd, rndT;
     MvsdfStepParams fake;
@@ -140,7 +144,7 @@
     L.ray_dirs = take((size_t)R * 12); L.cam_loc = take((size_t)d.B * 12);
     L.points = take((size_t)R * 12); L.mask = take((size_t)R); L.dists = take((size_t)R * 4); L.counters = take(16 * 8);
     L.object_mask_out = take((size_t)R);
-    fo.trace_ws_bytes = mvsdf_trace_workspace_bytes_n(R, d.tp.n_steps);
+    fo.trace_ws_bytes = mvsdf_trace_cut_workspace_bytes(R, d.tp.n_steps);
     fo.trace_ws = take(fo.trace_ws_bytes);
     fo.chain_x3 = mv_dev_switches().chain_x3;
     for (int l = 0; l < nl; ++l) {
@@ -212,6 +216,7 @@
     if (st->timing) for (int i = 0; i < 9; ++i) hipEventDestroy(st->ev_t[i]);
     if (st->counts_host) { hipEventDestroy(st->ev_counts); hipHostFree(st->counts_host); }
     if (st->side) { hipStreamSynchronize(st->side); hipEventDestroy(st->ev_fork); hipEventDestroy(st->ev_join); hipStreamDestroy(st->side); }
+    if (st->late) { hipStreamSynchronize(st->late); hipEventDestroy(st->ev_cut); hipEventDestroy(st->ev_late); hipStreamDestroy(st->late); }
     delete st;
 }
 
@@ -226,6 +231,15 @@
         st->timing = 0;
     }
     st->timed = false; st->timed_bwd = false;
+    return 0;
+}
+
+int mvsdf_step_set_sphere_cut(void* step, int enable, int max_rounds) {
+    Step* st = (Step*)step;
+    if (!st) return mv_fail(-1, "mvsdf_step_set_sphere_cut: null step");
+    st->cut_enable = enable < 0 ? -1 : (enable ? 1 : 0);
+    st->cut_rounds = max_rounds > 0 ? max_rounds : 0;
+    st->cut_on = -1;
     return 0;
 }
 
@@ -334,6 +348,21 @@
         ~SideGuard() { if (armed && side) (void)hipStreamSynchronize(side); }
     } side_guard{st->side, false};
     if (split) ST_HIP(hipEventRecord(st->ev_fork, s));
+    if (st->cut_on < 0) {
+        st->cut_on = st->cut_enable > 0 || (st->cut_enable < 0 && mv_trace_cut_pays(&sdf, R, d.mt));
+        if (st->cut_on && !st->late) {
+            if (hipStreamCreateWithFlags(&st->late, hipStreamNonBlocking) != hipSuccess) { (void)hipGetLastError(); st->late = nullptr; st->cut_on = 0; }
+            else if (hipEventCreateWithFlags(&st->ev_cut, hipEventDisableTiming) != hipSuccess || hipEventCreateWithFlags(&st->ev_late, hipEventDisableTiming) != hipSuccess) {
+                (void)hipGetLastError();
+                if (st->ev_cut) { (void)hipEventDestroy(st->ev_cut); st->ev_cut = nullptr; }
+                if (st->ev_late) { (void)hipEventDestroy(st->ev_late); st->ev_late = nullptr; }
+                (void)hipStreamDestroy(st->late);
+                st->late = nullptr; st->cut_on = 0;
+            }
+        }
+    }
+    const bool cut = lazy && st->cut_on == 1;
+    SideGuard late_guard{st->late, false};
     float* points = (float*)(fwd + L.points); uint8_t* mask = (uint8_t*)(fwd + L.mask); float* dists = (float*)(fwd + L.dists);
     unsigned long long* counters = (unsigned long long*)(fwd + L.counters);
     auto stage = [&](int which) {
@@ -344,7 +373,19 @@
                                  counters, fwd + fo.trace_ws, fo.trace_ws_bytes, d.mt, d.mt_samples, stream);
     };
     if (st->timing) ST_HIP(hipEventRecord(st->ev_t[0], s));
-    if (lazy) ST_TRY(stage(1));
+    auto cut_stage = [&](int which, void* strm) {
+        return mv_trace_cut_stage(which, st->cut_rounds, 1, &sdf, &d.tp, cam_loc, ray_dirs, in->object_mask, d.B, d.P, 1, in->intervals, in->minsdf_steps, points, mask, dists,
+                                  counters, fwd + fo.trace_ws, fo.trace_ws_bytes, d.mt, d.mt_samples, strm);
+    };
+    if (cut) {
+        ST_TRY(cut_stage(1, stream));
+        ST_HIP(hipEventRecord(st->ev_cut, s));
+        ST_HIP(hipStreamWaitEvent(st->late, st->ev_cut, 0));
+        late_guard.armed = true;
+        ST_TRY(cut_stage(2, (void*)st->late));
+        ST_TRY(cut_stage(3, (void*)st->late));
+        ST_HIP(hipEventRecord(st->ev_late, st->late));
+    } else if (lazy) ST_TRY(stage(1));
     else ST_TRY(mv_trace_stage1_prezeroed(&sdf, &d.tp, cam_loc, ray_dirs, in->object_mask, d.B, d.P, 1, in->intervals, in->minsdf_steps, points, mask, dists,
                                      counters, fwd + fo.trace_ws, fo.trace_ws_bytes, d.mt, d.mt_samples, stream));
     if (st->timing) ST_HIP(hipEventRecord(st->ev_t[1], s));
@@ -357,6 +398,7 @@
         else ST_HIP(hipEventRecord(st->ev_join, st->side));
     }
     ST_TRY(stage(3));
+    if (cut) { ST_HIP(hipStreamWaitEvent(s, st->ev_late, 0)); late_guard.armed = false; }
     if (st->timing) ST_HIP(hipEventRecord(st->ev_t[2], s));
     long long* perm = (long long*)(fwd + L.perm); long long* inv = (long long*)(fwd + fo.inv); long long* true_rows = (long long*)(fwd + fo.true_rows);
     long long* counts = (long long*)(fwd + fo.counts); float* view_sorted = (float*)(fwd + fo.view_sorted);
diff --git a/mvsdf_amd/csrc/step_internal.h b/mvsdf_amd/csrc/step_internal.h
--- a/mvsdf_amd/csrc/step_internal.h
+++ b/mvsdf_amd/csrc/step_internal.h
@@ -52,4 +52,8 @@
 extern "C" int mv_trace_stage_notail(int stage, const MvsdfNetDesc* desc, const MvsdfTraceParams* tp, const float* cam_loc, const float* ray_dirs, const uint8_t* object_mask,
                               int B, int P, int training, const float* intervals, const float* minsdf_steps, float* points, uint8_t* mask, float* dists,
                               unsigned long long* counters, void* workspace, size_t workspace_bytes, int mt, int mt_samples, void* stream);
+extern "C" int mv_trace_cut_stage(int stage, int max_rounds, int prezeroed, const MvsdfNetDesc* desc, const MvsdfTraceParams* tp, const float* cam_loc, const float* ray_dirs,
+                              const uint8_t* object_mask, int B, int P, int training, const float* intervals, const float* minsdf_steps, float* points, uint8_t* mask,
+                              float* dists, unsigned long long* counters, void* workspace, size_t workspace_bytes, int mt, int mt_samples, void* stream);
+extern "C" int mv_trace_cut_pays(const MvsdfNetDesc* desc, int R, int mt);
 void mv_trace_last_grid(int out[2]);
diff --git a/mvsdf_amd/csrc/trace.hip b/mvsdf_amd/csrc/trace.hip
--- a/mvsdf_amd/csrc/trace.hip
+++ b/mvsdf_amd/csrc/trace.hip
@@ -74,9 +74,14 @@
     int stop_left;
     unsigned* probe;
 };
+struct CutCtx {
+    float4* spill;
+    int max_rounds, resume;
+};
+#define MV_SPILL_F4 4
 #define MV_SPHERE_FINALIZE \
     if (tid == 0 && nrows_total) atomicAdd(&counters[MV_CNT_ROWS_SPHERE], nrows_total); \
-    if (valid) { \
+    if (valid && !spilled) { \
         bool net_mask = acc_s < acc_e; \
         const bool sampler = unf_s; \
         float dist = acc_s; \
@@ -107,7 +112,7 @@
             const bool smp = kind & MV_ITEM_SAMPLER; \
             w_zmin[gid] = zmin; \
             w_zmax[gid] = zmax; \
-            const unsigned long long idx = atomicAdd(&counters[smp ? MV_CNT_N_SAMPLER : MV_CNT_N_MINSDF], 1ull); \
+            const unsigned long long idx = atomicAdd(&counters[smp ? cnt_smp : MV_CNT_N_MINSDF], 1ull); \
             (smp ? w_list : w_list_min)[idx] = gid | (kind << 28); \
             if (!smp) n_pub = 1; \
         } \
@@ -119,7 +124,7 @@
                                                             int R, int P, int training, float* __restrict__ o_points,
                                                             uint8_t* __restrict__ o_mask, float* __restrict__ o_dists,
                                                             float* __restrict__ w_zmin, float* __restrict__ w_zmax, int* __restrict__ w_list,
-                                                            int* __restrict__ w_list_min, unsigned long long* __restrict__ counters, TailCtx tail) {
+                                                            int* __restrict__ w_list_min, unsigned long long* __restrict__ counters, TailCtx tail, CutCtx cut) {
     extern __shared__ __attribute__((aligned(16))) float smem[];
     constexpr int ROWS = 16 * MT, NR = 8 * MT;
     const long long clk0 = tail.probe ? (long long)wall_clock64() : 0;
@@ -128,12 +133,21 @@
     TraceLds lds = mv_carve<NET, (NTW < 4)>(smem, ROWS, net.S, 3 + 6 * net.multires, 0);
     int* s_n = lds.misc;
 
-    const int gid = blockIdx.x * NR + tid;
-    const bool valid = (tid < NR) && (gid < R);
+    const int n_spill = cut.resume ? (int)counters[MV_CNT_N_SPILL] : 0;
+    if (cut.resume && (int)blockIdx.x * NR >= n_spill) return;
+    const int cnt_smp = cut.resume ? (int)MV_CNT_N_SAMPLER_LATE : (int)MV_CNT_N_SAMPLER;
+    const int slot0 = blockIdx.x * NR + tid;
+    const bool valid = (tid < NR) && (slot0 < (cut.resume ? n_spill : R));
+    float4 sp2 = {0.f, 0.f, 0.f, 0.f};
+    if (cut.resume && valid) sp2 = cut.spill[MV_SPILL_F4 * (size_t)slot0 + 2];
+    const int gid = (cut.resume && valid) ? __float_as_int(sp2.z) : slot0;
     float c[3] = {0, 0, 0}, d[3] = {0, 0, 0};
     float t0 = 0.f, t1 = 0.f;
     bool isect = false, om = false;
-    if (valid) {
+    if (valid && cut.resume) {
+        const int b = gid / P;
+        for (int i = 0; i < 3; ++i) { c[i] = cam_loc[3 * b + i]; d[i] = dirs[3 * (size_t)gid + i]; }
+    } else if (valid) {
         const int b = gid / P;
         for (int i = 0; i < 3; ++i) { c[i] = cam_loc[3 * b + i]; d[i] = dirs[3 * (size_t)gid + i]; }
         isect = mv_sphere_isect(c, d, tp.r, t0, t1);
@@ -149,6 +163,15 @@
 
     bool hard_s = false, hard_e = false, bo_s = false, bo_e = false;
     const float lss1 = 1.0f - tp.line_search_step;
+    if (cut.resume && valid) {
+        const float4 a = cut.spill[MV_SPILL_F4 * (size_t)slot0], b = cut.spill[MV_SPILL_F4 * (size_t)slot0 + 1];
+        const int f = __float_as_int(cut.spill[MV_SPILL_F4 * (size_t)slot0 + 3].x);
+        acc_s = a.x; acc_e = a.y; next_s = a.z; next_e = a.w; curr_s = b.x; curr_e = b.y; t0 = b.z; t1 = b.w; ts = sp2.x; te = sp2.y;
+        iters = __float_as_int(sp2.w); k = f & 0xff; phase = (f >> 8) & 3;
+        unf_s = (f >> 16) & 1; unf_e = (f >> 17) & 1; req_s = (f >> 18) & 1; req_e = (f >> 19) & 1; hard_s = (f >> 20) & 1; hard_e = (f >> 21) & 1;
+        bo_s = (f >> 22) & 1; bo_e = (f >> 23) & 1; isect = (f >> 24) & 1; om = (f >> 25) & 1;
+    }
+    bool spilled = false;
     bool helping = false;
     int n_pub = 0;
     int h_chunk = 0, h_left = 0, h_items = 0, h_nr = 0;
@@ -200,7 +223,9 @@
                     if (sr_e[dd] >= 0) { float* p = lds.pts + sr_e[dd] * 3; p[0] = c[0] + z * d[0]; p[1] = c[1] + z * d[1]; p[2] = c[2] + z * d[2]; }
                 }
             }
-            if (lane == 0) { s_n[0] = base; s_n[1] = n; }
+            const bool cut_now = cut.max_rounds > 0 && n_rounds >= (unsigned)cut.max_rounds && n > 0;
+            if (cut_now) spilled = req_s || req_e;
+            if (lane == 0) { s_n[0] = cut_now ? 0 : base; s_n[1] = n; }
         }
         int n = 0;
         if (!helping) {
@@ -354,6 +379,24 @@
         }
     }
 
+    if (cut.resume && tid == 0) atomicMax(&counters[MV_CNT_LATE_ROUNDS], (unsigned long long)n_rounds);
+    if (cut.max_rounds > 0 && w == 0) {
+        const unsigned long long ml = __ballot(spilled);
+        if (ml) {
+            int base = 0;
+            if (lane == 0) base = (int)atomicAdd(&counters[MV_CNT_N_SPILL], (unsigned long long)__popcll(ml));
+            base = __shfl(base, 0);
+            if (spilled) {
+                float4* o = cut.spill + MV_SPILL_F4 * (size_t)(base + __popcll(ml & ((1ull << lane) - 1ull)));
+                const int f = k | (phase << 8) | ((int)unf_s << 16) | ((int)unf_e << 17) | ((int)req_s << 18) | ((int)req_e << 19) | ((int)hard_s << 20) | ((int)hard_e << 21) |
+                              ((int)bo_s << 22) | ((int)bo_e << 23) | ((int)isect << 24) | ((int)om << 25);
+                o[0] = make_float4(acc_s, acc_e, next_s, next_e);
+                o[1] = make_float4(curr_s, curr_e, t0, t1);
+                o[2] = make_float4(ts, te, __int_as_float(gid), __int_as_float(iters));
+                o[3] = make_float4(__int_as_float(f), 0.f, 0.f, 0.f);
+            }
+        }
+    }
     if (tail.enable) {
         if (tid == 0 && h_units) atomicAdd(&counters[MV_CNT_TAIL_ROWS], (unsigned long long)h_units * (unsigned long long)ROWS);
         if (tail.probe && tid == 0) {
@@ -619,6 +662,7 @@
 struct TraceCall {
     int engine, R, P, training;
     bool tail, no_tail;
+    int cut_rounds; bool resume;
     const MvTraceParams* tp;
     const float *cam_loc, *dirs, *intervals, *steps;
     const uint8_t* om;
@@ -642,9 +686,13 @@
         if (e != hipSuccess) return e;
         set1 = lds1;
     }
+    const MvTraceCutWs cw = mv_trace_cut_ws(t.R, t.tp->n_steps);
+    if ((t.cut_rounds > 0 || t.resume) && t.tail) return hipErrorInvalidValue;
+    const bool cutting = t.cut_rounds > 0 || t.resume;
+    const CutCtx cut = {cutting ? mv_ws_at<float4>(t.ws, cw.spill) : nullptr, t.resume ? 0 : t.cut_rounds, t.resume ? 1 : 0};
     hipLaunchKernelGGL((k_sphere_trace<MT, NTW, NW, NET>), dim3(mv_sphere_grid(t.R, MT)), dim3(64 * NW), lds1, t.stream, net, *t.tp, t.cam_loc, t.dirs, t.om, t.R, t.P,
-                       t.training, t.points, t.mask, t.dists, mv_ws_at<float>(t.ws, w.w_zmin), mv_ws_at<float>(t.ws, w.w_zmax), mv_ws_at<int>(t.ws, w.w_list),
-                       mv_ws_at<int>(t.ws, w.w_list_min), t.counters, tail);
+                       t.training, t.points, t.mask, t.dists, mv_ws_at<float>(t.ws, w.w_zmin), mv_ws_at<float>(t.ws, w.w_zmax),
+                       mv_ws_at<int>(t.ws, t.resume ? cw.list_late : w.w_list), mv_ws_at<int>(t.ws, w.w_list_min), t.counters, tail, cut);
     return hipGetLastError();
 }
 
@@ -678,6 +726,14 @@
             hipLaunchKernelGGL((k_ray_samples<MT, NTW, NW, NET>), dim3(g.rest), wg, lds2, t.stream, net, tp, c, rest, none, 0);
             hipLaunchKernelGGL(k_reduce_items, dim3(g.red), red_wg, 0, t.stream, tp, c, c.list_rest, c.src_rest, (int)MV_CNT_N_SAMPLER_REST, 1);
         }
+    } else if (part == 32) {
+        const MvTraceCutWs cw = mv_trace_cut_ws(t.R, n);
+        int* list_late = mv_ws_at<int>(t.ws, cw.list_late);
+        c.sv = mv_ws_at<float>(t.ws, cw.sv_late); c.n_first = n;
+        const int blocks = mv_row_blocks(t.R, n, MT);
+        const RowSeg all = {list_late, nullptr, (int)MV_CNT_N_SAMPLER_LATE, 0, n, blocks, 0};
+        hipLaunchKernelGGL((k_ray_samples<MT, NTW, NW, NET>), dim3(blocks), wg, lds2, t.stream, net, tp, c, all, none, 0);
+        hipLaunchKernelGGL(k_reduce_items, dim3(g.red), red_wg, 0, t.stream, tp, c, list_late, (const int*)nullptr, (int)MV_CNT_N_SAMPLER_LATE, 0);
     } else if (part == 8) {
         hipLaunchKernelGGL((k_ray_samples<MT, NTW, NW, NET>), dim3(g.sec), wg, lds2, t.stream, net, tp, c, none, none, g.sec);
         g_last_grid[0] = g.sec; g_last_grid[1] = 0;
@@ -744,9 +800,10 @@
     if (s1.rc) return hipErrorInvalidValue;
     t.tail = !t.no_tail && mv_tail_on(t.engine, t.training, t.steps != nullptr, t.R, s1.mt, mv_cu_count(), sw);
     hipError_t e = (stages & 1) ? mv_launch_inst(s1, net, t, 0) : hipSuccess;
-    for (int part = 1; part <= 16 && e == hipSuccess; part <<= 1)
+    for (int part = 1; part <= 32 && e == hipSuccess; part <<= 1)
         if ((stages >> 1) & part)
-            e = mv_launch_inst(part == 16 ? mv_route_secant(t.engine, maxnt, mt_samples, t.R, sw) : mv_route_samples(t.engine, maxnt, mt_samples, t.R, part, sw), net, t, part);
+            e = mv_launch_inst(part == 16 ? mv_route_secant(t.engine, maxnt, mt_samples, t.R, sw) : mv_route_samples(t.engine, maxnt, mt_samples, t.R, part == 32 ? 1 : part, sw),
+                               net, t, part);
     return e;
 }
 
@@ -966,12 +1023,13 @@
 extern "C" {
 
 size_t mvsdf_trace_workspace_bytes_n(int R, int n_steps) { return mv_trace_ws(R, n_steps).total; }
+size_t mvsdf_trace_cut_workspace_bytes(int R, int n_steps) { return mv_trace_cut_ws(R, n_steps).total; }
 size_t mvsdf_trace_workspace_bytes(int R) { return mvsdf_trace_workspace_bytes_n(R, 128); }
 
 static int trace_impl(int stages, const MvsdfNetDesc* desc, const MvsdfTraceParams* tp, const float* cam_loc, const float* ray_dirs,
                       const uint8_t* object_mask, int B, int P, int training, const float* intervals, const float* minsdf_steps,
                       float* points, uint8_t* mask, float* dists, unsigned long long* counters, void* workspace,
-                      size_t workspace_bytes, int mt, int mt_samples, void* stream) {
+                      size_t workspace_bytes, int mt, int mt_samples, void* stream, int cut_rounds = 0) {
     const MvEngineClass ec = mv_trace_engine(desc ? desc->trace_dtype : 0, false);
     if (ec.rc) return mv_fail(ec.rc, ec.why);
     return mv_with_trace_net(desc, ec.engine, [&](const auto& net) {
@@ -983,11 +1041,13 @@
             return mv_fail(-1, "mvsdf_trace: tracer parameters out of range");
         const int R = B * P;
         if (workspace_bytes < mvsdf_trace_workspace_bytes_n(R, tp->n_steps)) return mv_fail(-1, "mvsdf_trace: workspace too small");
+        if ((cut_rounds > 0 || (stages & (0x400 | 64))) && workspace_bytes < mvsdf_trace_cut_workspace_bytes(R, tp->n_steps))
+            return mv_fail(-1, "mvsdf_trace_cut_stage: workspace too small (mvsdf_trace_cut_workspace_bytes)");
         hipStream_t s = (hipStream_t)stream;
         hipError_t e = hipSuccess;
-        if ((stages & 1) && !(stages & 0x100)) e = hipMemsetAsync(counters, 0, 16 * sizeof(unsigned long long), s);
+        if ((stages & 1) && !(stages & 0x500)) e = hipMemsetAsync(counters, 0, 16 * sizeof(unsigned long long), s);
         if (e != hipSuccess) return mv_check(e, "mvsdf_trace: memset");
-        const TraceCall t = {ec.engine, R, P, training, false, (stages & 0x200) != 0, tp, cam_loc, ray_dirs, intervals, minsdf_steps ? minsdf_steps : intervals, object_mask,
+        const TraceCall t = {ec.engine, R, P, training, false, (stages & 0x200) != 0, cut_rounds, (stages & 0x400) != 0, tp, cam_loc, ray_dirs, intervals, minsdf_steps ? minsdf_steps : intervals, object_mask,
                              points, dists, mask, workspace, counters, s};
         return mv_check(mv_trace_launch(stages, net, t, mt, mt_samples), "mvsdf_trace");
     });
@@ -1024,6 +1084,29 @@
     if (stage < 1 || stage > 7 || !bits[stage]) return mv_fail(-1, "mv_trace_stage_notail: stage must be 1, 5, 6 or 7");
     return trace_impl(bits[stage] | 0x200, desc, tp, cam_loc, ray_dirs, object_mask, B, P, training, intervals, minsdf_steps, points, mask, dists, counters,
                       workspace, workspace_bytes, mt, mt_samples, stream);
+}
+
+int mv_trace_cut_stage(int stage, int max_rounds, int prezeroed, const MvsdfNetDesc* desc, const MvsdfTraceParams* tp, const float* cam_loc, const float* ray_dirs,
+                       const uint8_t* object_mask, int B, int P, int training, const float* intervals, const float* minsdf_steps, float* points, uint8_t* mask, float* dists,
+                       unsigned long long* counters, void* workspace, size_t workspace_bytes, int mt, int mt_samples, void* stream) {
+    if (stage < 1 || stage > 3 || !tp) return mv_fail(-1, "mvsdf_trace_cut_stage: stage must be 1..3");
+    const int bits[4] = {0, 1 | (prezeroed ? 0x100 : 0), 1 | 0x400, 64};
+    return trace_impl(bits[stage] | 0x200, desc, tp, cam_loc, ray_dirs, object_mask, B, P, training, intervals, minsdf_steps, points, mask, dists, counters,
+                      workspace, workspace_bytes, mt, mt_samples, stream, stage == 1 ? (max_rounds > 0 ? max_rounds : tp->st_iters + 1) : 0);
+}
+int mvsdf_trace_cut_stage(int stage, int max_rounds, const MvsdfNetDesc* desc, const MvsdfTraceParams* tp, const float* cam_loc, const float* ray_dirs,
+                          const uint8_t* object_mask, int B, int P, int training, const float* intervals, const float* minsdf_steps, float* points, uint8_t* mask,
+                          float* dists, unsigned long long* counters, void* workspace, size_t workspace_bytes, int mt, int mt_samples, void* stream) {
+    return mv_trace_cut_stage(stage, max_rounds, 0, desc, tp, cam_loc, ray_dirs, object_mask, B, P, training, intervals, minsdf_steps, points, mask, dists, counters,
+                              workspace, workspace_bytes, mt, mt_samples, stream);
+}
+int mv_trace_cut_pays(const MvsdfNetDesc* desc, int R, int mt) {
+    const MvEngineClass ec = mv_trace_engine(desc ? desc->trace_dtype : 0, false);
+    if (ec.rc || !desc) return 0;
+    int maxnt = 0;
+    for (int l = 0; l + 1 < desc->n_layers && l < MVSDF_MAX_LAYERS; ++l) { const int nt = (desc->N[l] + 15) / 16; maxnt = nt > maxnt ? nt : maxnt; }
+    const MvInst s1 = mv_route_sphere(ec.engine, maxnt, mt);
+    return (s1.rc == 0 && mv_sphere_cut_on(ec.engine, R, s1.mt, mv_cu_count())) ? 1 : 0;
 }
 
 size_t mvsdf_tracegen_state_bytes(int R) { return (size_t)(R > 0 ? R : 0) * sizeof(GenRay); }
diff --git a/mvsdf_amd/csrc/trace_params.h b/mvsdf_amd/csrc/trace_params.h
--- a/mvsdf_amd/csrc/trace_params.h
+++ b/mvsdf_amd/csrc/trace_params.h
@@ -14,6 +14,9 @@
 #define MV_CNT_TAIL_READY MVSDF_CNT_TAIL_READY
 #define MV_CNT_TAIL_WGS MVSDF_CNT_TAIL_WGS
 #define MV_CNT_TAIL_ROWS MVSDF_CNT_TAIL_ROWS
+#define MV_CNT_N_SPILL MVSDF_CNT_N_SPILL
+#define MV_CNT_N_SAMPLER_LATE MVSDF_CNT_N_SAMPLER_LATE
+#define MV_CNT_LATE_ROUNDS MVSDF_CNT_LATE_ROUNDS
 #define MV_ITEM_SAMPLER 1
 #define MV_ITEM_MINSDF 2
 #define MV_ITEM_OM 4
diff --git a/mvsdf_amd/csrc/trace_route.h b/mvsdf_amd/csrc/trace_route.h
--- a/mvsdf_amd/csrc/trace_route.h
+++ b/mvsdf_amd/csrc/trace_route.h
@@ -115,4 +115,18 @@
     const size_t r = 4 * (size_t)(R > 0 ? R : 0), n = n_steps > 0 ? n_steps : 0;
     return {0, r, 2 * r, 6 * r, 7 * r, 8 * r, 9 * r, (9 + n) * r, (10 + n) * r, (11 + n) * r, (11 + 2 * n) * r + 256};
 }
+inline bool mv_sphere_cut_on(int engine, int R, int mt1, int cus) {
+    const int grid = mv_sphere_grid(R, mt1);
+    return engine == MV_ENG_X3 && mt1 == 1 && grid <= cus && 2 * grid > cus;
+}
+struct MvTraceCutWs {
+    size_t spill;
+    size_t list_late;
+    size_t sv_late;
+    size_t total;
+};
+inline MvTraceCutWs mv_trace_cut_ws(int R, int n_steps) {
+    const size_t r = 4 * (size_t)(R > 0 ? R : 0), n = n_steps > 0 ? n_steps : 0, b = (mv_trace_ws(R, n_steps).total + 255) & ~(size_t)255;
+    return {b, b + 16 * r, b + 17 * r, b + (17 + n) * r + 256};
+}
 template <class T> inline T* mv_ws_at(void* ws, size_t offset) { return (T*)((char*)ws + offset); }
diff --git a/mvsdf_amd/model/implicit_differentiable_renderer.py b/mvsdf_amd/model/implicit_differentiable_renderer.py
--- a/mvsdf_amd/model/implicit_differentiable_renderer.py
+++ b/mvsdf_amd/model/implicit_differentiable_renderer.py
@@ -314,6 +314,8 @@
         self.host_stage = type(self).HOST_STAGE
         self.deferred_step = type(self).DEFERRED_STEP
         self.eager_unhit_rows = os.environ.get('MVSDF_EAGER_UNHIT', '0') not in ('', '0')
+        self.sphere_cut = {'0': False, '': False, '2': 2}.get(os.environ.get('MVSDF_SPHERE_CUT', '1'), True)
+        self.sphere_cut_rounds = 0
         self._steps = {}
         self._ones = None
 
@@ -569,6 +571,7 @@
         rec.use_geo = not bool(train_progress < conf.phase[0] or conf.disable_rgb_grad)
         rec.inputs_keep = keep
         rec.eager_unhit = bool(self.eager_unhit_rows) or not st.can_defer_unhit
+        st.set_sphere_cut(self.sphere_cut, self.sphere_cut_rounds)
         NS.enqueue_forward(rec)
         if stage_slot is not None:
             stage_slot[2] = (st, rec.seq)
diff --git a/mvsdf_amd/native_step.py b/mvsdf_amd/native_step.py
--- a/mvsdf_amd/native_step.py
+++ b/mvsdf_amd/native_step.py
@@ -64,6 +64,7 @@
         L.mvsdf_step_forward.argtypes = [C.c_void_p, C.c_void_p, C.c_void_p, C.c_int, C.c_int, C.c_int, C.c_void_p, C.c_void_p]
         L.mvsdf_step_resolve_unhit.argtypes = [C.c_void_p, C.c_void_p, C.c_void_p]
         L.mvsdf_step_can_defer_unhit.argtypes = [C.c_void_p]
+        L.mvsdf_step_set_sphere_cut.argtypes = [C.c_void_p, C.c_int, C.c_int]
         L.mvsdf_step_last_tracer_grid.argtypes = [C.c_void_p, C.c_void_p]
         L.mvsdf_step_wait_counts.argtypes = [C.c_void_p, C.c_void_p]
         L.mvsdf_step_seq.argtypes = [C.c_void_p]
@@ -155,6 +156,7 @@
         self.can_defer = bool(L.mvsdf_step_can_defer(h))
         self.counts_off = int(L.mvsdf_step_counts_offset(h))
         self.can_defer_unhit = bool(L.mvsdf_step_can_defer_unhit(h))
+        self._cut = (1, 0)
 
     def __del__(self):
         h, self._h = getattr(self, '_h', None), None
@@ -206,6 +208,12 @@
         check(lib().mvsdf_step_forward(self._h, C.byref(prm), C.byref(self.inputs), d_mask, e_mask, 1 if eager_unhit else 0, fwd.data_ptr(),
                                        _stream(self.device)), 'mvsdf_step_forward')
         return fwd
+
+    def set_sphere_cut(self, mode, max_rounds=0):
+        key = (int(mode), int(max_rounds))
+        if key != self._cut:
+            check(lib().mvsdf_step_set_sphere_cut(self._h, {0: 0, 1: -1}.get(key[0], 1), key[1]), 'mvsdf_step_set_sphere_cut')
+            self._cut = key
 
     def resolve_unhit(self, fwd):
         check(lib().mvsdf_step_resolve_unhit(self._h, fwd.data_ptr(), _stream(self.device)), 'mvsdf_step_resolve_unhit')
```

New measurement: 1.542 million, median of 6. 1.7% higher.
